# jiny2001/dcscn-super-resolution

Measured on AMD Instinct MI355X. Metric: LR Mpixels/sec at 48x48 patches, L12_F196to48 x2, higher is better.
Workload: dtype f32-equivalent (3x3 stack, wide 1x1 convs and folded tail: f16 hi/lo split, 3 products per MAC, f32 accumulate -- error at the f32 kernels' level, same parity bars; everything else f32)

## Files before the change

dcscn-super-resolution_amd/build.py:

```python

import os
import shutil
import subprocess
import sys
from concurrent.futures import ThreadPoolExecutor

PKG_DIR = os.path.dirname(os.path.abspath(__file__))
CSRC = os.path.join(PKG_DIR, "csrc")
INCLUDE = os.path.join(os.path.dirname(PKG_DIR), "include")
LIB_NAME = "libdcscn_hip.so"
LIB_PATH = os.path.join(PKG_DIR, LIB_NAME)
HEADERS = [os.path.join(CSRC, h) for h in sorted(os.listdir(CSRC)) if h.endswith((".h", ".hpp"))] + [os.path.join(INCLUDE, "dcscn.h")]
ARCH = "gfx950"
NO_PK_F32 = ["-Xclang", "-target-feature", "-Xclang", "-packed-fp32-ops"]
FLAGS = ["--offload-arch=" + ARCH, "-O3", "-std=c++17", "-fPIC", "-Wall", "-Wno-unused-function"] + NO_PK_F32
NO_SLP = ["-fno-slp-vectorize"]
KERNEL = NO_SLP + ["-Rpass-analysis=kernel-resource-usage"]
NO_CONTRACT = ["-ffp-contract=off"]
SOURCE_TABLE = {
    "api.hip": ([], False), "graph.hip": ([], False), "pack.hip": ([], False), "exec.hip": ([], False), "kernels.hip": ([], False),
    "resample.hip": ([], False), "ensemble.hip": ([], False), "color.hip": (NO_CONTRACT, False), "metrics.hip": (NO_CONTRACT, False),
    "conv_k1.hip": ([], False), "conv_k3.hip": ([], False), "conv_k5.hip": ([], False), "conv_k7.hip": ([], False),
    "conv_wino2.hip": (KERNEL, True), "conv_nin.hip": (KERNEL, True), "feat_stream.hip": (KERNEL, True),
    "conv_nin_h.hip": (KERNEL, True), "conv_nin_h_w8.hip": (KERNEL, True), "conv3_h.hip": (KERNEL, True), "conv3_h8.hip": (KERNEL, True),
    "conv5_h.hip": (KERNEL, True), "conv3_h_p16.hip": (KERNEL, True), "conv3_h8_p16.hip": (KERNEL, True),
    "conv3_h_fast16.hip": (KERNEL, True), "conv3_h8_fast16.hip": (KERNEL, True), "conv_nin_h_fast16.hip": (KERNEL, True),
    "conv5_h_fast16.hip": (KERNEL, True), "feat_stream_redo.hip": (NO_SLP, False), "feat3_stream.hip": (KERNEL, True),
    "feat3_stream_fast16.hip": (KERNEL, True),
    "train.hip": ([], False), "train_data.hip": ([], False), "train_h.hip": (KERNEL, True),
    "train_wgrad_h.hip": (KERNEL, True),
}
SOURCES = list(SOURCE_TABLE)
EXTRA_FLAGS = {src: flags for src, (flags, _) in SOURCE_TABLE.items()}
NO_SCRATCH = tuple(src for src, (_, no_spill) in SOURCE_TABLE.items() if no_spill)


def hipcc_path():
    for cand in (shutil.which("hipcc"), "/opt/rocm/bin/hipcc"):
        if cand and os.path.isfile(cand):
            return cand
    raise RuntimeError("hipcc not found; the DCSCN HIP extension cannot be built")


def _stale(target, deps):
    if not os.path.isfile(target):
        return True
    t = os.path.getmtime(target)
    return any(os.path.getmtime(d) > t for d in deps)


def _run(cmd):
    proc = subprocess.run(cmd, stdout=subprocess.PIPE, stderr=subprocess.STDOUT, text=True)
    proc.stdout = "\n".join(ln for ln in proc.stdout.splitlines() if "'-packed-fp32-ops' is not a recognized feature" not in ln)
    if proc.returncode != 0:
        raise RuntimeError("command failed (%d): %s\n%s" % (proc.returncode, " ".join(cmd), proc.stdout))
    if any(cmd[-3].endswith(n) for n in NO_SCRATCH if len(cmd) >= 3):
        import re
        bad = [ln for ln in proc.stdout.splitlines() if re.search(r"(ScratchSize \[bytes/lane\]|VGPRs Spill): [1-9]", ln)]
        if bad:
            os.remove(cmd[-1])
            raise RuntimeError("register spill in a kernel that must not spill (%s):\n%s" % (cmd[-3], "\n".join(bad[:6])))
        return ""
    return proc.stdout


def build(force=False, verbose=False):
    hipcc = hipcc_path()
    obj_dir = os.path.join(PKG_DIR, "build")
    os.makedirs(obj_dir, exist_ok=True)
    jobs = []
    objs = []
    for src in SOURCES:
        src_path = os.path.join(CSRC, src)
        obj = os.path.join(obj_dir, os.path.splitext(src)[0] + ".o")
        objs.append(obj)
        if force or _stale(obj, [src_path, os.path.abspath(__file__)] + HEADERS):
            jobs.append([hipcc] + FLAGS + EXTRA_FLAGS.get(src, []) + ["-I", INCLUDE, "-c", src_path, "-o", obj])
    if jobs:
        with ThreadPoolExecutor(max_workers=len(jobs)) as pool:
            for out in pool.map(_run, jobs):
                if verbose and out.strip():
                    print(out, file=sys.stderr)
    if jobs or force or _stale(LIB_PATH, objs):
        out = _run([hipcc, "--offload-arch=" + ARCH, "-shared", "-fPIC"] + objs + ["-o", LIB_PATH])
        if verbose and out.strip():
            print(out, file=sys.stderr)
    return LIB_PATH


if __name__ == "__main__":
    print(build(force="--force" in sys.argv, verbose=True))
```

dcscn-super-resolution_amd/csrc/api.hip:

```cpp
#include "plan.h"

#pragma clang fp contract(off)

namespace dcscn_impl {

thread_local std::string g_global_error;

void set_global_error(const char* fmt, ...) {
    char buf[512];
    va_list ap;
    va_start(ap, fmt);
    vsnprintf(buf, sizeof buf, fmt, ap);
    va_end(ap);
    g_global_error = buf;
}

int fail(dcscn_ctx* h, int code, const char* fmt, ...) {
    char buf[512];
    va_list ap;
    va_start(ap, fmt);
    vsnprintf(buf, sizeof buf, fmt, ap);
    va_end(ap);
    if (h) h->error = buf;
    g_global_error = buf;
    return code;
}

}

extern "C" {

int dcscn_abi_version(void) { return DCSCN_ABI_VERSION; }

const char* dcscn_last_global_error(void) { return g_global_error.c_str(); }

int dcscn_device_count(void) {
    int n = 0;
    hipError_t e = hipGetDeviceCount(&n);
    if (e != hipSuccess) {
        set_global_error("hipGetDeviceCount: %s", hipGetErrorString(e));
        return -DCSCN_ERR_HIP;
    }
    return n;
}

int dcscn_filter_schedule(int layers, int filters, int min_filters, double gamma, int32_t* out) {
    if (!out || layers <= 0 || gamma <= 0.0) {
        set_global_error("dcscn_filter_schedule: bad arguments");
        return DCSCN_ERR_INVALID_ARG;
    }
    std::vector<int> s;
    filter_schedule(layers, filters, std::min(filters, min_filters), gamma, s);
    for (int i = 0; i < layers; ++i) out[i] = s[i];
    return DCSCN_OK;
}

int dcscn_create(const dcscn_config* cfg, int device, dcscn_handle* out) {
    if (!cfg || !out) return fail(nullptr, DCSCN_ERR_INVALID_ARG, "dcscn_create: null argument");
    *out = nullptr;
    if (cfg->struct_size != (int32_t)sizeof(dcscn_config))
        return fail(nullptr, DCSCN_ERR_INVALID_ARG, "dcscn_create: struct_size %d != %zu", cfg->struct_size, sizeof(dcscn_config));
    dcscn_config c = *cfg;
    c.min_filters = std::min(c.filters, c.min_filters);
    c.reconstruct_layers = std::max(c.reconstruct_layers, 1);
    if (c.scale < 2 || c.scale > 4) return fail(nullptr, DCSCN_ERR_UNSUPPORTED, "scale %d (supported: 2, 3, 4)", c.scale);
    if (c.layers < 1 || c.layers > 256 || c.filters < 1) return fail(nullptr, DCSCN_ERR_INVALID_ARG, "bad layers/filters");
    if (c.layers > 1 && !(c.filters_decay_gamma > 0.0)) return fail(nullptr, DCSCN_ERR_INVALID_ARG, "filters_decay_gamma must be > 0");
    if (c.cnn_size != 1 && c.cnn_size != 3 && c.cnn_size != 5 && c.cnn_size != 7)
        return fail(nullptr, DCSCN_ERR_UNSUPPORTED, "cnn_size %d (supported: 1, 3, 5, 7)", c.cnn_size);
    if (c.channels != 1) return fail(nullptr, DCSCN_ERR_UNSUPPORTED, "channels %d (the reference itself only supports 1)", c.channels);
    if (c.batch_norm) return fail(nullptr, DCSCN_ERR_UNSUPPORTED, "batch_norm is not implemented");
    float dummy;
    if (kernel_act(c.activator, &dummy) < 0) return fail(nullptr, DCSCN_ERR_INVALID_ARG, "Not implemented activator:%d", c.activator);
    if (c.legacy_no_c && c.use_nin) return fail(nullptr, DCSCN_ERR_INVALID_ARG, "legacy_no_c requires use_nin = 0");
    if (c.reconstruct_layers > 1 && c.reconstruct_filters < 1) return fail(nullptr, DCSCN_ERR_INVALID_ARG, "reconstruct_filters must be positive");

    int ndev = 0;
    hipError_t e = hipGetDeviceCount(&ndev);
    if (e != hipSuccess || ndev <= 0)
        return fail(nullptr, DCSCN_ERR_HIP, "no HIP device available (%s); this library has no CPU fallback",
                    e != hipSuccess ? hipGetErrorString(e) : "device count 0");
    if (device < 0 || device >= ndev) return fail(nullptr, DCSCN_ERR_INVALID_ARG, "device %d out of range [0, %d)", device, ndev);

    dcscn_ctx* h = new (std::nothrow) dcscn_ctx();
    if (!h) return fail(nullptr, DCSCN_ERR_NOMEM, "out of host memory");
    h->cfg = c;
    h->device = device;
    int rc = DCSCN_OK;
    do {
        if ((e = hipSetDevice(device)) != hipSuccess) { rc = fail(h, DCSCN_ERR_HIP, "hipSetDevice: %s", hipGetErrorString(e)); break; }
        hipDeviceProp_t prop;
        if ((e = hipGetDeviceProperties(&prop, device)) != hipSuccess) { rc = fail(h, DCSCN_ERR_HIP, "hipGetDeviceProperties: %s", hipGetErrorString(e)); break; }
        if (strncmp(prop.gcnArchName, "gfx950", 6) != 0) {
            rc = fail(h, DCSCN_ERR_HIP, "device %d is %s; this library is built for gfx950 (MI355X) only", device, prop.gcnArchName);
            break;
        }
        h->n_cus = prop.multiProcessorCount > 0 ? prop.multiProcessorCount : 256;
        if ((e = hipStreamCreateWithFlags(&h->stream, hipStreamNonBlocking)) != hipSuccess) { rc = fail(h, DCSCN_ERR_HIP, "hipStreamCreate: %s", hipGetErrorString(e)); break; }
        if ((e = hipEventCreateWithFlags(&h->done_ev, hipEventDisableTiming)) != hipSuccess) { rc = fail(h, DCSCN_ERR_HIP, "hipEventCreate: %s", hipGetErrorString(e)); break; }
        if ((e = conv_init_kernels()) != hipSuccess) { rc = fail(h, DCSCN_ERR_HIP, "kernel attribute setup: %s", hipGetErrorString(e)); break; }
        {
            size_t free_b = 0, total_b = 0;
            if (hipMemGetInfo(&free_b, &total_b) == hipSuccess && free_b > 0)
                h->workspace_budget = std::min<int64_t>(h->workspace_budget, std::max<int64_t>((int64_t)(free_b / 10 * 6), (int64_t)256 << 20));
        }
        rc = build_graph(h);
    } while (0);
    if (rc != DCSCN_OK) {
        g_global_error = h->error;
        dcscn_destroy(h);
        return rc;
    }
    *out = h;
    return DCSCN_OK;
}

int dcscn_num_tensors(dcscn_handle h) { return h ? (int)h->tensors.size() : -DCSCN_ERR_INVALID_ARG; }

int dcscn_tensor_info(dcscn_handle h, int index, char* name, int name_capacity, int64_t* shape, int* rank) {
    if (!h) return DCSCN_ERR_INVALID_ARG;
    if (index < 0 || index >= (int)h->tensors.size() || !name || name_capacity <= 0 || !shape || !rank)
        return fail(h, DCSCN_ERR_INVALID_ARG, "dcscn_tensor_info: bad argument");
    const TensorSpec& t = h->tensors[index];
    snprintf(name, (size_t)name_capacity, "%s", t.name.c_str());
    *rank = (int)t.shape.size();
    for (int i = 0; i < 4; ++i) shape[i] = i < *rank ? t.shape[i] : 1;
    return DCSCN_OK;
}

int dcscn_set_tensor(dcscn_handle h, const char* name, const float* data, const int64_t* shape, int rank) {
    if (!h) return DCSCN_ERR_INVALID_ARG;
    if (!name || !data || !shape) return fail(h, DCSCN_ERR_INVALID_ARG, "dcscn_set_tensor: null argument");
    if (h->finalized) return fail(h, DCSCN_ERR_STATE, "dcscn_set_tensor after dcscn_finalize");
    auto it = h->tensor_index.find(name);
    if (it == h->tensor_index.end()) return fail(h, DCSCN_ERR_SHAPE, "variable '%s' is not part of this graph", name);
    TensorSpec& t = h->tensors[it->second];
    bool same = rank == (int)t.shape.size();
    for (int i = 0; same && i < rank; ++i) same = shape[i] == t.shape[i];
    if (!same) {
        std::string want, got;
        for (int64_t d : t.shape) want += std::to_string(d) + ",";
        for (int i = 0; i < rank && i < 8; ++i) got += std::to_string(shape[i]) + ",";
        return fail(h, DCSCN_ERR_SHAPE, "variable '%s': shape [%s] does not match graph shape [%s]", name, got.c_str(), want.c_str());
    }
    size_t count = 1;
    for (int64_t d : t.shape) count *= (size_t)d;
    for (size_t i = 0; i < count; ++i)
        if (!std::isfinite(data[i])) return fail(h, DCSCN_ERR_INVALID_ARG, "variable '%s' holds a non-finite value", name);
    t.data.assign(data, data + count);
    t.set = true;
    return DCSCN_OK;
}

static int pack_ops(dcscn_ctx* h) {
    const size_t first = h->device_allocs.size();
    int rc = DCSCN_OK;
    for (Op& op : h->ops) {
        rc = finalize_op(h, op);
        if (rc) break;
    }
    h->pack_allocs.insert(h->pack_allocs.end(), h->device_allocs.begin() + first, h->device_allocs.end());
    h->device_allocs.resize(first);
    return rc;
}

}

namespace dcscn_impl {
int repack_weights(dcscn_ctx* h) {
    HIP_TRY(h, hipDeviceSynchronize());
    if (h->graph_exec) {
        (void)hipGraphExecDestroy(h->graph_exec);
        h->graph_exec = nullptr;
        h->graph_key = dcscn_ctx::GraphKey();
    }
    h->graph_seen = dcscn_ctx::GraphKey();
    for (void* p : h->pack_allocs) (void)hipFree(p);
    h->pack_allocs.clear();
    return pack_ops(h);
}
}

extern "C" {

int dcscn_finalize(dcscn_handle h) {
    if (!h) return DCSCN_ERR_INVALID_ARG;
    if (h->finalized) return DCSCN_OK;
    for (const TensorSpec& t : h->tensors)
        if (!t.set) return fail(h, DCSCN_ERR_MISSING_TENSOR, "variable '%s' was never set", t.name.c_str());
    HIP_TRY(h, hipSetDevice(h->device));
    if (h->fold_tail) fold_linear_tail(h);
    fuse_tail_stream(h);
    fuse_feat_stream(h);
    densify_features(h);
    fuse_feat3_stream(h);
    fold_whole_tail(h);
    int rc0 = pack_ops(h);
    if (rc0) return rc0;
    plan_p16(h);
    for (Op& op : h->ops) {
        int rc = DCSCN_OK;
        if (op.kind == OP_CONV && op.shape.nin && op.h16.on && op.h16.in16_ok) {
            op.h16.h_tab16.assign((size_t)4 * op.h16.n_chunks, NinSrcQuad{0, 0, 0});
            rc = upload_vec(h, op.h16.h_tab16, &op.h16.d_tab16);
            if (rc) return rc;
        }
        auto alloc_srctab = [&](Op& o) {
            if (o.multi.empty()) return (int)DCSCN_OK;
            o.h_srctab.assign(std::max<size_t>((size_t)4 * o.n_chunks, (size_t)8 * ((o.cin_phys + kNinHKC - 1) / kNinHKC)), NinSrcQuad{0, 0, 0});
            return upload_vec(h, o.h_srctab, &o.d_srctab);
        };
        rc = alloc_srctab(op);
        if (rc) return rc;
        for (Op& sub : op.fused) {
            rc = alloc_srctab(sub);
            if (rc) return rc;
        }
    }
    h->finalized = true;
    return DCSCN_OK;
}

int dcscn_num_layers(dcscn_handle h) { return h ? (int)h->layers.size() : -DCSCN_ERR_INVALID_ARG; }

int dcscn_layer_info_get(dcscn_handle h, int index, dcscn_layer_info* out) {
    if (!h) return DCSCN_ERR_INVALID_ARG;
    if (!out || index < 0 || index >= (int)h->layers.size()) return fail(h, DCSCN_ERR_INVALID_ARG, "dcscn_layer_info_get: bad argument");
    *out = h->layers[index];
    return DCSCN_OK;
}

int dcscn_num_ops(dcscn_handle h) { return h ? (int)h->ops.size() : -DCSCN_ERR_INVALID_ARG; }

int dcscn_op_info_get(dcscn_handle h, int index, dcscn_op_info* out) {
    if (!h) return DCSCN_ERR_INVALID_ARG;
    if (!out || index < 0 || index >= (int)h->ops.size()) return fail(h, DCSCN_ERR_INVALID_ARG, "dcscn_op_info_get: bad argument");
    const Op& op = h->ops[index];
    memset(out, 0, sizeof *out);
    snprintf(out->name, sizeof out->name, "%s", op.name.c_str());
    const bool s16 = op_on_split16(h, op);
    snprintf(out->kernel, sizeof out->kernel, "%s", kernel_name(op_kernel(h, op)));
    out->kernel_size = op.ks;
    out->in_channels = op.cin;
    out->out_channels = op.cout;
    out->resolution = op.res;
    out->macs_per_lr_pixel = op.macs;
    out->bytes_per_lr_pixel = op.bytes;
    out->executed_macs_per_lr_pixel = op.macs;
    if (op.kind == OP_FOLDX && h->finalized && s16) {
        out->nt = 1; out->kc = 32; out->n_tiles = 1;
        out->executed_macs_per_lr_pixel = (h->fast16 ? 1 : 3) * 25 * (int64_t)op.h16.n_chunks * 32 * 16;
    }
    if (op.kind == OP_CONV && h->finalized) {
        out->mt = op.shape.mt; out->nt = op.shape.nt; out->kc = op.shape.kc; out->n_tiles = op.n_tiles;
        const int64_t r2 = (int64_t)op.res * op.res;
        const int64_t k_exec = (int64_t)op.n_chunks * op.shape.kc;
        if (s16) {
            const int64_t tiles = (int64_t)op.h16.n_tiles * (op.h16.nt - 1) + op.h16.n_full;
            out->nt = op.h16.nt; out->kc = 32; out->n_tiles = op.h16.n_tiles;
            const int64_t ksteps = op.shape.nin ? op.h16.n_chunks : op.fold_s > 0 ? 25 * (int64_t)op.h16.n_chunks
                                                : 9 * (int64_t)(op.h16.n_chunks - (op.h16.tail_octs ? 1 : 0)) + (op.h16.tail_octs ? c3h_tail_steps(op.h16.tail_octs) : 0);
            out->executed_macs_per_lr_pixel = r2 * (h->fast16 ? 1 : 3) * ksteps * 32 * tiles * 16;
        } else if (op.shape.nin) {
            const int64_t tiles = (int64_t)op.n_tiles * (op.shape.nt - 1) + op.n_full;
            out->executed_macs_per_lr_pixel = r2 * k_exec * tiles * 16;
        } else if (op.shape.wino) {
            const int64_t tiles = (int64_t)op.n_tiles * (op.shape.nt - 1) + op.n_full;
            out->executed_macs_per_lr_pixel = r2 * 4 * k_exec * tiles * 16;
        } else {
            out->executed_macs_per_lr_pixel = r2 * op.ks * op.ks * k_exec * (int64_t)op.n_tiles * op.shape.nt * 16;
        }
    }
    return DCSCN_OK;
}

int dcscn_set_option(dcscn_handle h, const char* key, int64_t value) {
    if (!h) return DCSCN_ERR_INVALID_ARG;
    if (!key) return fail(h, DCSCN_ERR_INVALID_ARG, "dcscn_set_option: null key");
    if (!strcmp(key, "sub_batch_pixels")) {
        if (value < 1) return fail(h, DCSCN_ERR_INVALID_ARG, "sub_batch_pixels must be >= 1");
        h->sub_batch_pixels = value;
        return DCSCN_OK;
    }
    if (!strcmp(key, "workspace_budget_bytes")) {
        if (value < 1) return fail(h, DCSCN_ERR_INVALID_ARG, "workspace_budget_bytes must be >= 1");
        h->workspace_budget = value;
        return DCSCN_OK;
    }
    if (!strcmp(key, "spatial_tiling")) {
        h->spatial_tiling = value != 0;
        return DCSCN_OK;
    }
    if (!strcmp(key, "fold_whole_tail")) {
        if (h->finalized) return fail(h, DCSCN_ERR_STATE, "the fold_whole_tail option must be set before dcscn_finalize");
        h->fold_whole = value != 0;
        return DCSCN_OK;
    }
    if (!strcmp(key, "fold_linear_tail")) {
        if (h->finalized) return fail(h, DCSCN_ERR_STATE, "the fold_linear_tail option must be set before dcscn_finalize");
        h->fold_tail = value != 0;
        h->fold_force = value == 2;
        return DCSCN_OK;
    }
    if (!strcmp(key, "stream_tail")) {
        if (h->finalized) return fail(h, DCSCN_ERR_STATE, "the stream_tail option must be set before dcscn_finalize");
        h->stream_tail = value != 0;
        return DCSCN_OK;
    }
    if (!strcmp(key, "stream_features")) {
        if (h->finalized) return fail(h, DCSCN_ERR_STATE, "the stream_features option must be set before dcscn_finalize");
        h->stream_features = value != 0;
        return DCSCN_OK;
    }
    if (!strcmp(key, "stream_nin")) {
        if (h->finalized) return fail(h, DCSCN_ERR_STATE, "the stream_nin option must be set before dcscn_finalize");
        h->stream_nin = value != 0;
        return DCSCN_OK;
    }
    if (!strcmp(key, "stream_dense")) {
        if (h->finalized) return fail(h, DCSCN_ERR_STATE, "the stream_dense option must be set before dcscn_finalize");
        h->stream_dense = value != 0;
        return DCSCN_OK;
    }
    if (!strcmp(key, "dense_features")) {
        if (h->finalized) return fail(h, DCSCN_ERR_STATE, "the dense_features option must be set before dcscn_finalize");
        h->dense_features = value != 0;
        return DCSCN_OK;
    }
    if (!strcmp(key, "nin_gemm")) {
        if (h->finalized) return fail(h, DCSCN_ERR_STATE, "the nin_gemm option must be set before dcscn_finalize");
        h->nin = value != 0;
        return DCSCN_OK;
    }
    if (!strcmp(key, "winograd")) {
        if (h->finalized) return fail(h, DCSCN_ERR_STATE, "the winograd option must be set before dcscn_finalize");
        h->winograd = value != 0;
        return DCSCN_OK;
    }
    if (!strcmp(key, "split16")) {
        h->split16 = value != 0;
        h->split16_mask = value == 2 ? 1 : value == 3 ? 2 : 3;
        return DCSCN_OK;
    }
    if (!strcmp(key, "fast16")) {
        h->fast16 = value != 0;
        return DCSCN_OK;
    }
    if (!strcmp(key, "fast16_stream")) {
        h->fast16_stream = value != 0;
        return DCSCN_OK;
    }
    if (!strcmp(key, "train_split16")) {
        h->train_split16 = value != 0;
        return DCSCN_OK;
    }
    if (!strcmp(key, "train_split16_wgrad")) {
        h->train_split16_wgrad = value != 0;
        return DCSCN_OK;
    }
    if (!strcmp(key, "p16")) {
        h->p16 = value != 0;
        return DCSCN_OK;
    }
    if (!strcmp(key, "conv3_h8")) {
        h->conv3_h8 = value != 0;
        return DCSCN_OK;
    }
    if (!strcmp(key, "nin_h8")) {
        h->nin_h8 = value != 0;
        return DCSCN_OK;
    }
    if (!strcmp(key, "debug_digest")) {
        if ((int)h->ops.size() + 1 > 1024) return fail(h, DCSCN_ERR_UNSUPPORTED, "debug_digest: more than 1023 launches");
        h->debug_digest = value != 0;
        return DCSCN_OK;
    }
    if (!strcmp(key, "debug_poison")) {
        h->debug_poison = (int)value;
        return DCSCN_OK;
    }
    if (!strcmp(key, "profile")) {
        h->profile = value != 0;
        return DCSCN_OK;
    }
    if (!strcmp(key, "graph_replay")) {
        h->graph_replay = value != 0;
        if (!h->graph_replay && h->graph_exec) {
            (void)hipGraphExecDestroy(h->graph_exec);
            h->graph_exec = nullptr;
        }
        h->graph_seen = dcscn_ctx::GraphKey{};
        return DCSCN_OK;
    }
    return fail(h, DCSCN_ERR_INVALID_ARG, "unknown option '%s'", key);
}

int dcscn_forward_device(dcscn_handle h, const float* x, const float* x2, float* y, int n, int height, int width, void* stream) {
    if (!h) return DCSCN_ERR_INVALID_ARG;
    if (h->finalized)
        if (int rc_ = train_sync_inference(h)) return rc_;
    return run_forward(h, x, x2, y, n, height, width, stream ? (hipStream_t)stream : h->stream);
}

static int ensure_io(dcscn_ctx* h, size_t lr_floats, size_t hr_floats) {
    int rc = grow(h, &h->io_x, &h->io_x_cap, lr_floats, h->stream, DCSCN_ERR_HIP);
    if (!rc) rc = grow(h, &h->io_x2, &h->io_x2_cap, hr_floats, h->stream, DCSCN_ERR_HIP);
    if (!rc) rc = grow(h, &h->io_y, &h->io_y_cap, hr_floats, h->stream, DCSCN_ERR_HIP);
    return rc;
}

static int forward_host_chunked(dcscn_ctx* h, const float* x, const float* x2, float* y, int n, int height, int width) {
    const int s = h->cfg.scale;
    const size_t lr1 = (size_t)height * width, hr1 = lr1 * s * s;
    int rc = ensure_io(h, lr1 * n, hr1 * n);
    if (rc) return rc;
    const int chunks = (hr1 * n * sizeof(float) >= ((size_t)8 << 20) && n >= 8) ? 4 : 1;
    while ((int)h->host_ev.size() < chunks) {
        hipEvent_t e;
        HIP_TRY(h, hipEventCreateWithFlags(&e, hipEventDisableTiming));
        h->host_ev.push_back(e);
    }
    int begin[5];
    for (int i = 0; i <= chunks; ++i) begin[i] = (int)((int64_t)n * i / chunks);
    auto span = [&](int i, int* b, int* cnt) { *b = begin[chunks - 1 - i] ; *cnt = begin[chunks - i] - begin[chunks - 1 - i]; };
    auto download = [&](int i) -> int {
        int b, cnt;
        span(i, &b, &cnt);
        HIP_TRY(h, hipEventSynchronize(h->host_ev[i]));
        HIP_TRY(h, hipMemcpy(y + (size_t)b * hr1, h->io_y + (size_t)b * hr1, (size_t)cnt * hr1 * sizeof(float), hipMemcpyDeviceToHost));
        return DCSCN_OK;
    };
    for (int i = 0; i < chunks; ++i) {
        int b, cnt;
        span(i, &b, &cnt);
        if (cnt > 0) {
            HIP_TRY(h, hipMemcpy(h->io_x + (size_t)b * lr1, x + (size_t)b * lr1, (size_t)cnt * lr1 * sizeof(float), hipMemcpyHostToDevice));
            if (x2) HIP_TRY(h, hipMemcpy(h->io_x2 + (size_t)b * hr1, x2 + (size_t)b * hr1, (size_t)cnt * hr1 * sizeof(float), hipMemcpyHostToDevice));
            else rc = resize_device(h, h->io_x + (size_t)b * lr1, h->io_x2 + (size_t)b * hr1, cnt, height, width, height * s, width * s, h->stream);
            if (!rc) rc = run_forward(h, h->io_x + (size_t)b * lr1, h->io_x2 + (size_t)b * hr1, h->io_y + (size_t)b * hr1, cnt, height, width, h->stream);
            if (rc) return rc;
        }
        HIP_TRY(h, hipEventRecord(h->host_ev[i], h->stream));
        if (i > 0 && (rc = download(i - 1))) return rc;
    }
    if ((rc = download(chunks - 1))) return rc;
    return DCSCN_OK;
}

int dcscn_forward(dcscn_handle h, const float* x, const float* x2, float* y, int n, int height, int width) {
    if (!h) return DCSCN_ERR_INVALID_ARG;
    if (!h->finalized) return fail(h, DCSCN_ERR_STATE, "dcscn_forward before dcscn_finalize");
    if (int rc_ = train_sync_inference(h)) return rc_;
    if (n < 0 || height <= 0 || width <= 0) return fail(h, DCSCN_ERR_INVALID_ARG, "bad shape n=%d h=%d w=%d", n, height, width);
    if (n == 0) return DCSCN_OK;
    if (!x || !x2 || !y) return fail(h, DCSCN_ERR_INVALID_ARG, "null image pointer");
    HIP_TRY(h, hipSetDevice(h->device));
    return forward_host_chunked(h, x, x2, y, n, height, width);
}

int dcscn_resample_table(int in_size, int out_size, int* ksize, int* bounds, double* weights, int capacity) {
    if (in_size <= 0 || out_size <= 0 || !ksize) return DCSCN_ERR_INVALID_ARG;
    std::vector<int> b;
    std::vector<double> k;
    *ksize = resample_coeffs(in_size, out_size, &b, &k);
    if (!bounds && !weights) return DCSCN_OK;
    if (!bounds || !weights || capacity < (int)k.size()) return DCSCN_ERR_INVALID_ARG;
    std::copy(b.begin(), b.end(), bounds);
    std::copy(k.begin(), k.end(), weights);
    return DCSCN_OK;
}

int dcscn_resize_bicubic(dcscn_handle h, const float* in, float* out, int n, int height, int width, int out_height, int out_width) {
    if (!h) return DCSCN_ERR_INVALID_ARG;
    if (n < 0 || height <= 0 || width <= 0 || out_height <= 0 || out_width <= 0)
        return fail(h, DCSCN_ERR_INVALID_ARG, "bad shape n=%d %dx%d -> %dx%d", n, height, width, out_height, out_width);
    if (n == 0) return DCSCN_OK;
    if (!in || !out) return fail(h, DCSCN_ERR_INVALID_ARG, "null image pointer");
    HIP_TRY(h, hipSetDevice(h->device));
    const size_t ni = (size_t)n * height * width, no = (size_t)n * out_height * out_width;
    int rc = grow(h, &h->rs_in, &h->rs_in_cap, ni, h->stream);
    if (!rc) rc = grow(h, &h->rs_out, &h->rs_out_cap, no, h->stream);
    if (rc) return rc;
    HIP_TRY(h, hipMemcpy(h->rs_in, in, ni * sizeof(float), hipMemcpyHostToDevice));
    rc = resize_device(h, h->rs_in, h->rs_out, n, height, width, out_height, out_width, h->stream);
    if (rc) return rc;
    HIP_TRY(h, hipStreamSynchronize(h->stream));
    HIP_TRY(h, hipMemcpy(out, h->rs_out, no * sizeof(float), hipMemcpyDeviceToHost));
    return DCSCN_OK;
}

int dcscn_resize_bicubic_device(dcscn_handle h, const float* in, float* out, int n, int height, int width, int out_height,
                                int out_width, void* stream) {
    if (!h) return DCSCN_ERR_INVALID_ARG;
    if (n < 0 || height <= 0 || width <= 0 || out_height <= 0 || out_width <= 0)
        return fail(h, DCSCN_ERR_INVALID_ARG, "bad shape n=%d %dx%d -> %dx%d", n, height, width, out_height, out_width);
    if (n == 0) return DCSCN_OK;
    if (!in || !out) return fail(h, DCSCN_ERR_INVALID_ARG, "null image pointer");
    HIP_TRY(h, hipSetDevice(h->device));
    hipStream_t st = stream ? (hipStream_t)stream : h->stream;
    if (h->has_last && h->last_stream != st) HIP_TRY(h, hipStreamWaitEvent(st, h->done_ev, 0));
    const int rc = resize_device(h, in, out, n, height, width, out_height, out_width, st);
    if (rc) return rc;
    return forward_done(h, st);
}

int dcscn_resample_table_bytes(int in_size, int out_size, int* ksize, int* bounds, int32_t* coeffs, int capacity) {
    if (in_size <= 0 || out_size <= 0 || !ksize) return DCSCN_ERR_INVALID_ARG;
    std::vector<int> b, k;
    *ksize = resample_coeffs8(in_size, out_size, &b, &k);
    if (!bounds && !coeffs) return DCSCN_OK;
    if (!bounds || !coeffs || capacity < (int)k.size()) return DCSCN_ERR_INVALID_ARG;
    std::copy(b.begin(), b.end(), bounds);
    std::copy(k.begin(), k.end(), coeffs);
    return DCSCN_OK;
}

static int resize_bytes_args(dcscn_handle h, const uint8_t* in, uint8_t* out, int n, int height, int width, int channels, int out_height,
                             int out_width, bool* run) {
    *run = false;
    if (n < 0 || height <= 0 || width <= 0 || out_height <= 0 || out_width <= 0)
        return fail(h, DCSCN_ERR_INVALID_ARG, "bad shape n=%d %dx%d -> %dx%d", n, height, width, out_height, out_width);
    if (channels != 1 && channels != 3)
        return fail(h, DCSCN_ERR_INVALID_ARG, "%d channels (uint8 images have 1 (mode L) or 3 (RGB))", channels);
    if (n == 0) return DCSCN_OK;
    if (!in || !out) return fail(h, DCSCN_ERR_INVALID_ARG, "null image pointer");
    *run = true;
    return DCSCN_OK;
}

int dcscn_resize_bicubic_bytes(dcscn_handle h, const uint8_t* in, uint8_t* out, int n, int height, int width, int channels, int out_height,
                               int out_width) {
    if (!h) return DCSCN_ERR_INVALID_ARG;
    bool run;
    int rc = resize_bytes_args(h, in, out, n, height, width, channels, out_height, out_width, &run);
    if (rc || !run) return rc;
    HIP_TRY(h, hipSetDevice(h->device));
    const size_t ni = (size_t)n * height * width * channels, no = (size_t)n * out_height * out_width * channels;
    rc = grow(h, &h->rs_in, &h->rs_in_cap, (ni + 3) / 4, h->stream);
    if (!rc) rc = grow(h, &h->rs_out, &h->rs_out_cap, (no + 3) / 4, h->stream);
    if (rc) return rc;
    HIP_TRY(h, hipMemcpy(h->rs_in, in, ni, hipMemcpyHostToDevice));
    rc = resize_device_bytes(h, reinterpret_cast<const uint8_t*>(h->rs_in), reinterpret_cast<uint8_t*>(h->rs_out), n, height, width, channels,
                             out_height, out_width, h->stream);
    if (rc) return rc;
    HIP_TRY(h, hipStreamSynchronize(h->stream));
    HIP_TRY(h, hipMemcpy(out, h->rs_out, no, hipMemcpyDeviceToHost));
    return DCSCN_OK;
}

int dcscn_resize_bicubic_bytes_device(dcscn_handle h, const uint8_t* in, uint8_t* out, int n, int height, int width, int channels,
                                      int out_height, int out_width, void* stream) {
    if (!h) return DCSCN_ERR_INVALID_ARG;
    bool run;
    int rc = resize_bytes_args(h, in, out, n, height, width, channels, out_height, out_width, &run);
    if (rc || !run) return rc;
    HIP_TRY(h, hipSetDevice(h->device));
    hipStream_t st = stream ? (hipStream_t)stream : h->stream;
    if (h->has_last && h->last_stream != st) HIP_TRY(h, hipStreamWaitEvent(st, h->done_ev, 0));
    rc = resize_device_bytes(h, in, out, n, height, width, channels, out_height, out_width, st);
    if (rc) return rc;
    return forward_done(h, st);
}

int dcscn_forward_lr(dcscn_handle h, const float* x, float* y, int n, int height, int width) {
    if (!h) return DCSCN_ERR_INVALID_ARG;
    if (!h->finalized) return fail(h, DCSCN_ERR_STATE, "dcscn_forward_lr before dcscn_finalize");
    if (int rc_ = train_sync_inference(h)) return rc_;
    if (n < 0 || height <= 0 || width <= 0) return fail(h, DCSCN_ERR_INVALID_ARG, "bad shape n=%d h=%d w=%d", n, height, width);
    if (n == 0) return DCSCN_OK;
    if (!x || !y) return fail(h, DCSCN_ERR_INVALID_ARG, "null image pointer");
    HIP_TRY(h, hipSetDevice(h->device));
    return forward_host_chunked(h, x, nullptr, y, n, height, width);
}

static int ensemble_on_device(dcscn_ctx* h, int height, int width, int n) {
    const int s = h->cfg.scale;
    const size_t lr = (size_t)height * width, hr = lr * s * s;
    const int na = std::min(n, 4), nb = n - na;
    int rc = grow(h, &h->ens_x, &h->ens_x_cap, n * lr, h->stream);
    if (!rc) rc = grow(h, &h->ens_x2, &h->ens_x2_cap, n * hr, h->stream);
    if (!rc) rc = grow(h, &h->ens_y, &h->ens_y_cap, n * hr, h->stream);
    if (!rc) rc = grow(h, &h->ens_out, &h->ens_out_cap, 2 * hr, h->stream);
    if (rc) return rc;
    HIP_TRY(h, ensemble_gather_launch(h->io_x, h->ens_x, height, width, n, h->stream));
    HIP_TRY(h, ensemble_gather_launch(h->io_x2, h->ens_x2, height * s, width * s, n, h->stream));
    rc = run_forward(h, h->ens_x, h->ens_x2, h->ens_y, na, height, width, h->stream);
    if (!rc && nb > 0)
        rc = run_forward(h, h->ens_x + (size_t)na * lr, h->ens_x2 + (size_t)na * hr, h->ens_y + (size_t)na * hr, nb, width, height, h->stream);
    if (rc) return rc;
    HIP_TRY(h, ensemble_reduce_launch(h->ens_y, reinterpret_cast<double*>(h->ens_out), height * s, width * s, n, h->stream));
    return DCSCN_OK;
}

int dcscn_forward_ensemble(dcscn_handle h, const float* x, const float* x2, double* y, int height, int width, int n_ensemble) {
    if (!h) return DCSCN_ERR_INVALID_ARG;
    if (!h->finalized) return fail(h, DCSCN_ERR_STATE, "dcscn_forward_ensemble before dcscn_finalize");
    if (int rc_ = train_sync_inference(h)) return rc_;
    if (!x || !x2 || !y) return fail(h, DCSCN_ERR_INVALID_ARG, "null image pointer");
    if (n_ensemble < 1 || n_ensemble > 8) return fail(h, DCSCN_ERR_INVALID_ARG, "n_ensemble %d outside [1, 8]", n_ensemble);
    if (height <= 0 || width <= 0) return fail(h, DCSCN_ERR_INVALID_ARG, "bad shape h=%d w=%d", height, width);
    HIP_TRY(h, hipSetDevice(h->device));
    const int s = h->cfg.scale;
    const size_t lr = (size_t)height * width, hr = lr * s * s;
    int rc = ensure_io(h, lr, hr);
    if (rc) return rc;
    HIP_TRY(h, hipMemcpy(h->io_x, x, lr * sizeof(float), hipMemcpyHostToDevice));
    HIP_TRY(h, hipMemcpy(h->io_x2, x2, hr * sizeof(float), hipMemcpyHostToDevice));
    rc = ensemble_on_device(h, height, width, n_ensemble);
    if (rc) return rc;
    HIP_TRY(h, hipStreamSynchronize(h->stream));
    HIP_TRY(h, hipMemcpy(y, h->ens_out, hr * sizeof(double), hipMemcpyDeviceToHost));
    return DCSCN_OK;
}


static int color_args(dcscn_handle h, const void* a, const void* b, int64_t n, const char* what) {
    if (!a || !b) return fail(h, DCSCN_ERR_INVALID_ARG, "%s: null pointer", what);
    if (n < 0) return fail(h, DCSCN_ERR_INVALID_ARG, "%s: negative pixel count", what);
    return DCSCN_OK;
}

int dcscn_convert_rgb_to_y(dcscn_handle h, const uint8_t* rgb, double* y, int64_t n_pixels) {
    if (!h) return DCSCN_ERR_INVALID_ARG;
    int rc = color_args(h, rgb, y, n_pixels, "dcscn_convert_rgb_to_y");
    if (rc || n_pixels == 0) return rc;
    HIP_TRY(h, hipSetDevice(h->device));
    rc = grow(h, &h->col_rgb, &h->col_rgb_cap, (size_t)(3 * n_pixels + 3) / 4, h->stream);
    if (!rc) rc = grow(h, &h->col_d, &h->col_d_cap, (size_t)2 * n_pixels, h->stream);
    if (rc) return rc;
    HIP_TRY(h, hipMemcpy(h->col_rgb, rgb, (size_t)3 * n_pixels, hipMemcpyHostToDevice));
    HIP_TRY(h, rgb_to_y_launch(reinterpret_cast<const uint8_t*>(h->col_rgb), reinterpret_cast<double*>(h->col_d), nullptr, n_pixels, h->stream));
    HIP_TRY(h, hipStreamSynchronize(h->stream));
    HIP_TRY(h, hipMemcpy(y, h->col_d, (size_t)n_pixels * sizeof(double), hipMemcpyDeviceToHost));
    return DCSCN_OK;
}

int dcscn_convert_rgb_to_ycbcr(dcscn_handle h, const uint8_t* rgb, double* ycbcr, int64_t n_pixels) {
    if (!h) return DCSCN_ERR_INVALID_ARG;
    int rc = color_args(h, rgb, ycbcr, n_pixels, "dcscn_convert_rgb_to_ycbcr");
    if (rc || n_pixels == 0) return rc;
    HIP_TRY(h, hipSetDevice(h->device));
    rc = grow(h, &h->col_rgb, &h->col_rgb_cap, (size_t)(3 * n_pixels + 3) / 4, h->stream);
    if (!rc) rc = grow(h, &h->col_d, &h->col_d_cap, (size_t)6 * n_pixels, h->stream);
    if (rc) return rc;
    HIP_TRY(h, hipMemcpy(h->col_rgb, rgb, (size_t)3 * n_pixels, hipMemcpyHostToDevice));
    HIP_TRY(h, rgb_to_ycbcr_launch(reinterpret_cast<const uint8_t*>(h->col_rgb), reinterpret_cast<double*>(h->col_d), n_pixels, h->stream));
    HIP_TRY(h, hipStreamSynchronize(h->stream));
    HIP_TRY(h, hipMemcpy(ycbcr, h->col_d, (size_t)3 * n_pixels * sizeof(double), hipMemcpyDeviceToHost));
    return DCSCN_OK;
}

int dcscn_convert_y_and_cbcr_to_rgb(dcscn_handle h, const double* y, const double* cbcr, double* rgb, int64_t n_pixels) {
    if (!h) return DCSCN_ERR_INVALID_ARG;
    int rc = color_args(h, y, cbcr, n_pixels, "dcscn_convert_y_and_cbcr_to_rgb");
    if (!rc && !rgb) rc = fail(h, DCSCN_ERR_INVALID_ARG, "dcscn_convert_y_and_cbcr_to_rgb: null pointer");
    if (rc || n_pixels == 0) return rc;
    HIP_TRY(h, hipSetDevice(h->device));
    rc = grow(h, &h->col_d, &h->col_d_cap, (size_t)6 * n_pixels, h->stream);
    if (!rc) rc = grow(h, &h->col_d2, &h->col_d2_cap, (size_t)6 * n_pixels, h->stream);
    if (rc) return rc;
    double* dy = reinterpret_cast<double*>(h->col_d);
    double* dc = dy + n_pixels;
    HIP_TRY(h, hipMemcpy(dy, y, (size_t)n_pixels * sizeof(double), hipMemcpyHostToDevice));
    HIP_TRY(h, hipMemcpy(dc, cbcr, (size_t)2 * n_pixels * sizeof(double), hipMemcpyHostToDevice));
    HIP_TRY(h, y_cbcr_to_rgb_launch(dy, nullptr, dc, nullptr, reinterpret_cast<double*>(h->col_d2), n_pixels, h->stream));
    HIP_TRY(h, hipStreamSynchronize(h->stream));
    HIP_TRY(h, hipMemcpy(rgb, h->col_d2, (size_t)3 * n_pixels * sizeof(double), hipMemcpyDeviceToHost));
    return DCSCN_OK;
}

static int sr_from_lr_on_device(dcscn_ctx* h, int lh, int lw, int n_ensemble) {
    const int s = h->cfg.scale;
    int rc = resize_device(h, h->io_x, h->io_x2, 1, lh, lw, lh * s, lw * s, h->stream);
    if (rc) return rc;
    if (n_ensemble > 1) return ensemble_on_device(h, lh, lw, n_ensemble);
    return run_forward(h, h->io_x, h->io_x2, h->io_y, 1, lh, lw, h->stream);
}

static int download_sr(dcscn_ctx* h, size_t hr, int n_ensemble, double* y) {
    HIP_TRY(h, hipStreamSynchronize(h->stream));
    if (n_ensemble > 1) {
        HIP_TRY(h, hipMemcpy(y, h->ens_out, hr * sizeof(double), hipMemcpyDeviceToHost));
    } else {
        std::vector<float> tmp(hr);
        HIP_TRY(h, hipMemcpy(tmp.data(), h->io_y, hr * sizeof(float), hipMemcpyDeviceToHost));
        for (size_t i = 0; i < hr; ++i) y[i] = (double)tmp[i];
    }
    return DCSCN_OK;
}

static int evaluate_rgb_on_device(dcscn_ctx* h, const uint8_t* rgb, int height, int width, int n_ensemble, const char* what) {
    if (!h->finalized) return fail(h, DCSCN_ERR_STATE, "%s before dcscn_finalize", what);
    if (int rc_ = train_sync_inference(h)) return rc_;
    if (!rgb) return fail(h, DCSCN_ERR_INVALID_ARG, "%s: null pointer", what);
    if (n_ensemble < 1 || n_ensemble > 8) return fail(h, DCSCN_ERR_INVALID_ARG, "n_ensemble %d outside [1, 8]", n_ensemble);
    const int s = h->cfg.scale;
    if (height <= 0 || width <= 0 || height % s || width % s)
        return fail(h, DCSCN_ERR_INVALID_ARG, "image %dx%d is not aligned to the scale %d (set_image_alignment, utilty.py:196-208)", height, width, s);
    HIP_TRY(h, hipSetDevice(h->device));
    const int lh = height / s, lw = width / s;
    const size_t hr = (size_t)height * width, lrn = (size_t)lh * lw;
    int rc = ensure_io(h, lrn, hr);
    if (!rc) rc = grow(h, &h->col_rgb, &h->col_rgb_cap, (3 * hr + 3) / 4, h->stream);
    if (!rc) rc = grow(h, &h->col_d, &h->col_d_cap, 2 * hr, h->stream);
    if (!rc) rc = grow(h, &h->col_y32, &h->col_y32_cap, hr, h->stream);
    if (rc) return rc;
    HIP_TRY(h, hipMemcpy(h->col_rgb, rgb, 3 * hr, hipMemcpyHostToDevice));
    HIP_TRY(h, rgb_to_y_launch(reinterpret_cast<const uint8_t*>(h->col_rgb), reinterpret_cast<double*>(h->col_d), h->col_y32, (long long)hr, h->stream));
    rc = resize_device(h, h->col_y32, h->io_x, 1, height, width, lh, lw, h->stream);
    if (!rc) rc = sr_from_lr_on_device(h, lh, lw, n_ensemble);
    return rc;
}

int dcscn_evaluate_rgb(dcscn_handle h, const uint8_t* rgb, int height, int width, int n_ensemble, double* true_y, float* lr, double* y) {
    if (!h) return DCSCN_ERR_INVALID_ARG;
    int rc = evaluate_rgb_on_device(h, y ? rgb : nullptr, height, width, n_ensemble, "dcscn_evaluate_rgb");
    const size_t hr = (size_t)height * width, lrn = hr / ((size_t)h->cfg.scale * h->cfg.scale);
    if (!rc) rc = download_sr(h, hr, n_ensemble, y);
    if (rc) return rc;
    if (true_y) HIP_TRY(h, hipMemcpy(true_y, h->col_d, hr * sizeof(double), hipMemcpyDeviceToHost));
    if (lr) HIP_TRY(h, hipMemcpy(lr, h->io_x, lrn * sizeof(float), hipMemcpyDeviceToHost));
    return DCSCN_OK;
}


static const MetricWeights& metric_weights() {
    static const MetricWeights wt = [] {
        MetricWeights m;
        const double sigma2 = 1.5 * 1.5;
        for (int k = 0; k < kMetricTaps; ++k) {
            const double x = (double)(k - kMetricTaps / 2);
            m.w[k] = exp(-0.5 / sigma2 * (x * x));
        }
        double sum = ((m.w[0] + m.w[1]) + (m.w[2] + m.w[3])) + ((m.w[4] + m.w[5]) + (m.w[6] + m.w[7]));
        for (int k = 8; k < kMetricTaps; ++k) sum += m.w[k];
        for (int k = 0; k < kMetricTaps; ++k) m.w[k] = m.w[k] / sum;
        return m;
    }();
    return wt;
}

static int metric_shape(dcscn_ctx* h, int height, int width, int border, const char* what, int* sh, int* sw) {
    if (height <= 0 || width <= 0) return fail(h, DCSCN_ERR_INVALID_ARG, "%s: bad shape h=%d w=%d", what, height, width);
    if (border < 0) return fail(h, DCSCN_ERR_INVALID_ARG, "%s: negative border_size %d (win_size cannot be placed)", what, border);
    *sh = height - 2 * border;
    *sw = width - 2 * border;
    if (*sh < kMetricTaps || *sw < 1)
        return fail(h, DCSCN_ERR_INVALID_ARG, "%s: win_size exceeds image extent (%d x %d after shaving %d: needs %d rows and 1 column)", what,
                    *sh, *sw, border, kMetricTaps);
    return DCSCN_OK;
}

static int metric_buffers(dcscn_ctx* h, int sh, int sw) {
    return grow(h, &h->met_buf, &h->met_buf_cap, (size_t)8 + 2 * (size_t)metric_segments(sh) * sw, h->stream);
}

static int metric_enqueue(dcscn_ctx* h, int slot, const double* a64, const float* a32, const double* b64, const float* b32, int width, int border,
                          int sh, int sw) {
    double* part_s = h->met_buf + 8;
    long long* part_e = reinterpret_cast<long long*>(part_s + (size_t)metric_segments(sh) * sw);
    HIP_TRY(h, metrics_launch(a64, a32, b64, b32, width, border, sh, sw, metric_weights(), part_s, part_e,
                              reinterpret_cast<long long*>(h->met_buf) + 4 * slot, h->stream));
    return DCSCN_OK;
}

static int metric_download(dcscn_ctx* h, dcscn_metrics* first, dcscn_metrics* second) {
    long long words[8];
    HIP_TRY(h, hipStreamSynchronize(h->stream));
    HIP_TRY(h, hipMemcpy(words, h->met_buf, sizeof words, hipMemcpyDeviceToHost));
    dcscn_metrics* outs[2] = {first, second};
    for (int i = 0; i < 2; ++i) {
        if (!outs[i]) continue;
        dcscn_metrics& m = *outs[i];
        m.sq_err_sum = words[4 * i];
        m.n_pixels = words[4 * i + 1];
        memcpy(&m.ssim, &words[4 * i + 2], sizeof(double));
        const double err = (double)m.sq_err_sum / (double)m.n_pixels;
        m.psnr = m.sq_err_sum == 0 ? (double)INFINITY : 10.0 * log10((255.0 * 255.0) / err);
    }
    return DCSCN_OK;
}

int dcscn_psnr_ssim(dcscn_handle h, const double* a, const double* b, int height, int width, int border_size, dcscn_metrics* out) {
    if (!h) return DCSCN_ERR_INVALID_ARG;
    if (!a || !b || !out) return fail(h, DCSCN_ERR_INVALID_ARG, "dcscn_psnr_ssim: null pointer");
    int sh, sw;
    int rc = metric_shape(h, height, width, border_size, "dcscn_psnr_ssim", &sh, &sw);
    if (rc) return rc;
    HIP_TRY(h, hipSetDevice(h->device));
    const size_t n = (size_t)height * width;
    rc = grow(h, &h->col_d, &h->col_d_cap, 2 * n, h->stream);
    if (!rc) rc = grow(h, &h->col_d2, &h->col_d2_cap, 2 * n, h->stream);
    if (!rc) rc = metric_buffers(h, sh, sw);
    if (rc) return rc;
    const double* da = reinterpret_cast<const double*>(h->col_d);
    const double* db = reinterpret_cast<const double*>(h->col_d2);
    HIP_TRY(h, hipMemcpy(h->col_d, a, n * sizeof(double), hipMemcpyHostToDevice));
    HIP_TRY(h, hipMemcpy(h->col_d2, b, n * sizeof(double), hipMemcpyHostToDevice));
    rc = metric_enqueue(h, 0, da, nullptr, db, nullptr, width, border_size, sh, sw);
    if (!rc) rc = metric_download(h, out, nullptr);
    return rc;
}

int dcscn_evaluate_rgb_metrics(dcscn_handle h, const uint8_t* rgb, int height, int width, int n_ensemble, int border_size, dcscn_metrics* model,
                               dcscn_metrics* bicubic, double* y) {
    if (!h) return DCSCN_ERR_INVALID_ARG;
    if (!h->finalized) return fail(h, DCSCN_ERR_STATE, "dcscn_evaluate_rgb_metrics before dcscn_finalize");
    if (!rgb || !model) return fail(h, DCSCN_ERR_INVALID_ARG, "dcscn_evaluate_rgb_metrics: null pointer");
    int sh, sw;
    int rc = metric_shape(h, height, width, border_size, "dcscn_evaluate_rgb_metrics", &sh, &sw);
    if (!rc) rc = evaluate_rgb_on_device(h, rgb, height, width, n_ensemble, "dcscn_evaluate_rgb_metrics");
    if (!rc) rc = metric_buffers(h, sh, sw);
    if (rc) return rc;
    const double* true_y = reinterpret_cast<const double*>(h->col_d);
    rc = metric_enqueue(h, 0, true_y, nullptr, n_ensemble > 1 ? reinterpret_cast<const double*>(h->ens_out) : nullptr,
                        n_ensemble > 1 ? nullptr : h->io_y, width, border_size, sh, sw);
    if (!rc && bicubic) rc = metric_enqueue(h, 1, true_y, nullptr, nullptr, h->io_x2, width, border_size, sh, sw);
    if (!rc) rc = metric_download(h, model, bicubic);
    if (!rc && y) rc = download_sr(h, (size_t)height * width, n_ensemble, y);
    return rc;
}

int dcscn_sr_rgb(dcscn_handle h, const uint8_t* rgb, const uint8_t* rgb_upscaled, int height, int width, int n_ensemble, double* y, double* rgb_out) {
    if (!h) return DCSCN_ERR_INVALID_ARG;
    if (!h->finalized) return fail(h, DCSCN_ERR_STATE, "dcscn_sr_rgb before dcscn_finalize");
    if (int rc_ = train_sync_inference(h)) return rc_;
    if (!rgb || !rgb_upscaled || !rgb_out) return fail(h, DCSCN_ERR_INVALID_ARG, "dcscn_sr_rgb: null pointer");
    if (n_ensemble < 1 || n_ensemble > 8) return fail(h, DCSCN_ERR_INVALID_ARG, "n_ensemble %d outside [1, 8]", n_ensemble);
    if (height <= 0 || width <= 0) return fail(h, DCSCN_ERR_INVALID_ARG, "bad shape h=%d w=%d", height, width);
    HIP_TRY(h, hipSetDevice(h->device));
    const int s = h->cfg.scale;
    const size_t lrn = (size_t)height * width, hr = lrn * s * s;
    int rc = ensure_io(h, lrn, hr);
    if (!rc) rc = grow(h, &h->col_rgb, &h->col_rgb_cap, (3 * hr + 3) / 4 + (3 * lrn + 3) / 4 + 4, h->stream);
    if (!rc) rc = grow(h, &h->col_d2, &h->col_d2_cap, 6 * hr, h->stream);
    if (rc) return rc;
    uint8_t* d_up = reinterpret_cast<uint8_t*>(h->col_rgb);
    uint8_t* d_lr = d_up + ((3 * hr + 15) & ~(size_t)15);
    HIP_TRY(h, hipMemcpy(d_lr, rgb, 3 * lrn, hipMemcpyHostToDevice));
    HIP_TRY(h, hipMemcpy(d_up, rgb_upscaled, 3 * hr, hipMemcpyHostToDevice));
    HIP_TRY(h, rgb_to_y_launch(d_lr, nullptr, h->io_x, (long long)lrn, h->stream));
    rc = sr_from_lr_on_device(h, height, width, n_ensemble);
    if (rc) return rc;
    HIP_TRY(h, y_cbcr_to_rgb_launch(n_ensemble > 1 ? reinterpret_cast<const double*>(h->ens_out) : nullptr, n_ensemble > 1 ? nullptr : h->io_y,
                                    nullptr, d_up, reinterpret_cast<double*>(h->col_d2), (long long)hr, h->stream));
    if (y) rc = download_sr(h, hr, n_ensemble, y);
    else HIP_TRY(h, hipStreamSynchronize(h->stream));
    if (rc) return rc;
    HIP_TRY(h, hipMemcpy(rgb_out, h->col_d2, 3 * hr * sizeof(double), hipMemcpyDeviceToHost));
    return DCSCN_OK;
}

int dcscn_sr_rgb_bytes(dcscn_handle h, const uint8_t* rgb, int height, int width, int n_ensemble, uint8_t* rgb_bicubic, uint8_t* y_bicubic,
                       uint8_t* y_out, uint8_t* rgb_out) {
    if (!h) return DCSCN_ERR_INVALID_ARG;
    if (!h->finalized) return fail(h, DCSCN_ERR_STATE, "dcscn_sr_rgb_bytes before dcscn_finalize");
    if (int rc_ = train_sync_inference(h)) return rc_;
    if (!rgb || (!rgb_bicubic && !y_bicubic && !y_out && !rgb_out)) return fail(h, DCSCN_ERR_INVALID_ARG, "dcscn_sr_rgb_bytes: null pointer");
    if (n_ensemble < 1 || n_ensemble > 8) return fail(h, DCSCN_ERR_INVALID_ARG, "n_ensemble %d outside [1, 8]", n_ensemble);
    if (height <= 0 || width <= 0) return fail(h, DCSCN_ERR_INVALID_ARG, "bad shape h=%d w=%d", height, width);
    HIP_TRY(h, hipSetDevice(h->device));
    const int s = h->cfg.scale;
    const size_t lrn = (size_t)height * width, hr = lrn * s * s;
    const bool net = y_out || rgb_out, luma = net || y_bicubic, colour = rgb_bicubic || rgb_out;
    const size_t plane = (hr + 15) & ~(size_t)15;
    int rc = ensure_io(h, lrn, hr);
    if (!rc) rc = grow(h, &h->col_rgb, &h->col_rgb_cap, (3 * hr + 3) / 4 + (3 * lrn + 3) / 4 + 4, h->stream);
    if (!rc) rc = grow(h, &h->col_d2, &h->col_d2_cap, (2 * plane + 3 * hr + 3) / 4, h->stream);
    if (rc) return rc;
    uint8_t* d_up = reinterpret_cast<uint8_t*>(h->col_rgb);
    uint8_t* d_lr = d_up + ((3 * hr + 15) & ~(size_t)15);
    uint8_t* d_yb = reinterpret_cast<uint8_t*>(h->col_d2);
    uint8_t *d_yo = d_yb + plane, *d_ro = d_yo + plane;
    HIP_TRY(h, hipMemcpy(d_lr, rgb, 3 * lrn, hipMemcpyHostToDevice));
    if (colour && (rc = resize_device_bytes(h, d_lr, d_up, 1, height, width, 3, height * s, width * s, h->stream))) return rc;
    if (luma) {
        HIP_TRY(h, rgb_to_y_launch(d_lr, nullptr, h->io_x, (long long)lrn, h->stream));
        rc = net ? sr_from_lr_on_device(h, height, width, n_ensemble)
                 : resize_device(h, h->io_x, h->io_x2, 1, height, width, height * s, width * s, h->stream);
        if (rc) return rc;
    }
    const double* y64 = n_ensemble > 1 ? reinterpret_cast<const double*>(h->ens_out) : nullptr;
    const float* y32 = n_ensemble > 1 ? nullptr : h->io_y;
    if (y_bicubic) HIP_TRY(h, cast_bytes_launch(nullptr, h->io_x2, d_yb, (long long)hr, h->stream));
    if (y_out) HIP_TRY(h, cast_bytes_launch(y64, y32, d_yo, (long long)hr, h->stream));
    if (rgb_out) HIP_TRY(h, y_cbcr_to_rgb_bytes_launch(y64, y32, d_up, d_ro, (long long)hr, h->stream));
    HIP_TRY(h, hipStreamSynchronize(h->stream));
    if (rgb_bicubic) HIP_TRY(h, hipMemcpy(rgb_bicubic, d_up, 3 * hr, hipMemcpyDeviceToHost));
    if (y_bicubic) HIP_TRY(h, hipMemcpy(y_bicubic, d_yb, hr, hipMemcpyDeviceToHost));
    if (y_out) HIP_TRY(h, hipMemcpy(y_out, d_yo, hr, hipMemcpyDeviceToHost));
    if (rgb_out) HIP_TRY(h, hipMemcpy(rgb_out, d_ro, 3 * hr, hipMemcpyDeviceToHost));
    return DCSCN_OK;
}

int dcscn_get_profile(dcscn_handle h, double* ms, int capacity) {
    if (!h) return DCSCN_ERR_INVALID_ARG;
    if (!ms || capacity < 0) return fail(h, DCSCN_ERR_INVALID_ARG, "dcscn_get_profile: bad argument");
    const int nops = (int)h->ops.size();
    std::vector<double> acc(nops + 1, 0.0);
    const int forwards = h->ev_forwards;
    if (h->ev_used > 0) {
        HIP_TRY(h, hipDeviceSynchronize());
        const size_t launches = h->ev_used / 2;
        for (size_t l = 0; l < launches && l < h->ev_op.size(); ++l) {
            float t = 0.0f;
            HIP_TRY(h, hipEventElapsedTime(&t, h->ev[2 * l], h->ev[2 * l + 1]));
            acc[std::min(std::max(h->ev_op[l], 0), nops)] += t;
        }
    }
    h->ev_used = 0;
    h->ev_forwards = 0;
    h->ev_op.clear();
    if (forwards > 1)
        for (double& v : acc) v /= forwards;
    for (int i = 0; i < std::min(capacity, nops + 1); ++i) ms[i] = acc[i];
    return DCSCN_OK;
}

int dcscn_debug_digests(dcscn_handle h, uint64_t* out, int capacity) {
    if (!h) return DCSCN_ERR_INVALID_ARG;
    if (!out || capacity < 0) return fail(h, DCSCN_ERR_INVALID_ARG, "dcscn_debug_digests: bad argument");
    if (!h->d_digest) return fail(h, DCSCN_ERR_STATE, "dcscn_debug_digests: no forward has run with the debug_digest option on");
    HIP_TRY(h, hipDeviceSynchronize());
    const int n = std::min(capacity, (int)h->ops.size() + 1);
    HIP_TRY(h, hipMemcpy(out, h->d_digest, (size_t)n * sizeof(uint64_t), hipMemcpyDeviceToHost));
    return DCSCN_OK;
}

int64_t dcscn_workspace_bytes(dcscn_handle h) { return h ? (int64_t)h->arena_bytes : -1; }

int dcscn_num_presplit_tensors(dcscn_handle h) {
    if (!h) return -DCSCN_ERR_INVALID_ARG;
    if (!h->finalized || !p16_active(h)) return 0;
    int n = 0;
    for (const WsBuf& b : h->bufs) n += b.p16_ok && b.stride > 0;
    return n;
}

const char* dcscn_last_error(dcscn_handle h) { return h ? h->error.c_str() : g_global_error.c_str(); }

int dcscn_get_stream(dcscn_handle h, void** stream) {
    if (!h) return DCSCN_ERR_INVALID_ARG;
    if (!stream) return fail(h, DCSCN_ERR_INVALID_ARG, "dcscn_get_stream: null pointer");
    *stream = (void*)h->stream;
    return DCSCN_OK;
}

int dcscn_synchronize(dcscn_handle h) {
    if (!h) return DCSCN_ERR_INVALID_ARG;
    HIP_TRY(h, hipSetDevice(h->device));
    if (h->has_last) HIP_TRY(h, hipStreamSynchronize(h->last_stream));
    HIP_TRY(h, hipStreamSynchronize(h->stream));
    return DCSCN_OK;
}

int dcscn_destroy(dcscn_handle h) {
    if (!h) return DCSCN_OK;
    (void)hipSetDevice(h->device);
    if (h->has_last) (void)hipStreamSynchronize(h->last_stream);
    if (h->stream) (void)hipStreamSynchronize(h->stream);
    if (h->graph_exec) (void)hipGraphExecDestroy(h->graph_exec);
    if (h->done_ev) (void)hipEventDestroy(h->done_ev);
    for (hipEvent_t e : h->host_ev) (void)hipEventDestroy(e);
    for (hipEvent_t e : h->ev) (void)hipEventDestroy(e);
    train_free(h);
    train_batches_free(h);
    for (void* p : h->device_allocs) (void)hipFree(p);
    for (void* p : h->pack_allocs) (void)hipFree(p);
    if (h->arena) (void)hipFree(h->arena);
    if (h->d_zrec) (void)hipFree(h->d_zrec);
    if (h->d_digest) (void)hipFree(h->d_digest);
    for (float* p : {h->io_x, h->io_x2, h->io_y, h->tile_x, h->tile_x2, h->tile_y, h->rs_tmp, h->rs_in, h->rs_out, h->ens_x, h->ens_x2, h->ens_y, h->ens_out, h->col_rgb, h->col_d,
                     h->col_d2, h->col_y32})
        if (p) (void)hipFree(p);
    if (h->met_buf) (void)hipFree(h->met_buf);
    if (h->stream) (void)hipStreamDestroy(h->stream);
    delete h;
    return DCSCN_OK;
}

}
```

dcscn-super-resolution_amd/csrc/conv3_h8.hip:

```cpp
#include "conv3_h8.hpp"

namespace dcscn {

using List = C3EVariants<false, 3>;

hipError_t c3e_init_kernels() {
    hipError_t e = c3e16_init_kernels();
    if (e == hipSuccess) e = c3e1_init_kernels();
    return e != hipSuccess ? e : List::set_attrs();
}

bool c3e_eligible(int nt, const ConvArgs& a, int n_groups) {
    return n_groups == 2 && nt >= 4 && nt <= 6 && a.n_full >= 1 && a.n_full <= 2 && a.ps == 1 && a.res == nullptr && (a.act == ACT_ALPHA || a.act == ACT_NONE) &&
           a.n_chunks >= 3;
}

hipError_t c3e_launch(int nt, const ConvArgs& args, int n_groups, int n_cus, hipStream_t stream, bool fast16) {
    if (!c3e_eligible(nt, args, n_groups) || !args.wpack16 || args.tiles_x != (args.W + 15) / 16 || args.tiles_y != (args.H + 15) / 16) return hipErrorInvalidValue;
    ConvArgs a = args;
    a.n_groups = n_groups;
    a.nt_pack = nt;
    const long long units = (long long)a.N * a.tiles_y * a.tiles_x;
    if (units > 0x7fffffffLL) return hipErrorInvalidValue;
    const int wgs = (int)(units < n_cus ? units : n_cus);
    const bool out16 = a.out0.p16.base != nullptr && (a.split >= (1 << 29) || a.out1.p16.base != nullptr);
    const bool p16 = a.in16.base && out16;
    if (!p16 && (a.in16.base || a.out0.p16.base || a.out1.p16.base)) return hipErrorInvalidValue;
    const int key = c3e_key(nt, a.n_full == 2 ? nt : nt - 1, p16);
    if (fast16) return c3e1_launch(key, a, wgs, stream);
    if (p16) return c3e16_launch(key, a, wgs, stream);
    return List::launch(key, a, wgs, stream);
}

}
```

dcscn-super-resolution_amd/csrc/conv3_h8.hpp:

```cpp
#pragma once
#include "conv3_h.hpp"
#include "p16.hpp"

namespace dcscn {

template <int N>
__device__ __forceinline__ void c3p_wait_vm() { asm volatile("s_waitcnt vmcnt(%0)" ::"n"(N) : "memory"); }
__device__ __forceinline__ void c3p_barrier() { asm volatile("s_waitcnt lgkmcnt(0)\n\ts_barrier" ::: "memory"); }

__device__ __forceinline__ void glds16c(const void* sbase, unsigned voff, unsigned lds_dst) {
    asm volatile("s_mov_b32 m0, %2\n\ts_nop 0\n\tglobal_load_lds_dwordx4 %0, %1" : : "v"(voff), "s"(sbase), "s"(lds_dst) : "memory", "m0");
}

template <int NT>
struct C3EGeom {
    static constexpr int THREADS = 512;
    static constexpr int KC = 32, TH = 16, TW = 16, HT = 18, HP = HT * HT;
    static constexpr int PIX_BYTES = 128, ROW_BYTES = HT * PIX_BYTES, IN_BYTES = HP * PIX_BYTES;
    static constexpr int IN_BUF = 41 * 1024;
    static constexpr int IN_ITEMS = HP * 8;
    static constexpr int IN_ROUNDS = (IN_ITEMS + THREADS - 1) / THREADS;
    static constexpr int F_TAP_BYTES = NT * 2048;
    static constexpr int F_ROUNDS = (2 * NT + 3) / 4;
    static constexpr int IMG = 0;
    static constexpr int F_BASE = 2 * IN_BUF;
    static constexpr int BA_BASE = F_BASE + 2 * 3 * F_TAP_BYTES;
    static constexpr int LDS_BYTES = BA_BASE + 4 * NT * 128;
};

template <int NT, int C1, int NTP = NT, bool P16 = false, int NP = 3>
__global__ __launch_bounds__(512, 2) void conv3_h8(const ConvArgs a) {
    static_assert(C1 == NT || C1 == NT - 1, "half 1 takes as many tiles as half 0 or one fewer");
    static_assert(NP == 1 || NP == 3, "one product (fast16) or three (split16)");
    constexpr int PFD = 2 < NT ? 2 : (NT > 1 ? NT - 1 : 1), NB = PFD + 1;
    using G = C3EGeom<NT>;
    extern __shared__ __attribute__((aligned(16))) char smem_c3e[];
    char* const smem = smem_c3e;
    constexpr int F = G::F_ROUNDS, L = G::IN_ROUNDS;

    const int tid = threadIdx.x;
    const int lane = tid & 63;
    const int wave = __builtin_amdgcn_readfirstlane(tid >> 6);
    const int half = wave >> 2, w4 = wave & 3;
    const int H = a.H, W = a.W;
    const int n_groups = a.n_groups, ntp = NTP ? NTP : a.nt_pack;
    const int n_pairs = (n_groups + 1) >> 1;
    const int n_units = a.N * a.tiles_y * a.tiles_x * n_pairs;
    const int n_chunks = a.n_chunks;
    const int octs = a.tail_octs;
    const int n_main = octs ? n_chunks - 1 : n_chunks;
    const int n_tail = (9 * octs + 3) >> 2;
    const int t_total = n_main * 9 + n_tail;
    const bool fastable = a.ps == 1 && a.res == nullptr && (a.act == ACT_ALPHA || a.act == ACT_NONE) && (a.split & 15) == 0;
    const unsigned lds0 = (unsigned)(uintptr_t)(__attribute__((address_space(3))) char*)smem;
    const unsigned f_off = (unsigned)(lane * 16);
    const int cq = tid & 7;
    const int tap_stride = ntp * 2048;

    struct Unit {
        int valid, tile_id, img, y0, x0, g, o;
        int pix0;
        bool all_in, full;
        const char* a_base;
        const char* f_base;
        unsigned ok_mask;
    };
    auto decode = [&](int id, Unit& u) DCSCN_INL {
        u.valid = id < n_units;
        const int idc = u.valid ? id : 0;
        const int tile_id = idc / n_pairs, p = idc - tile_id * n_pairs;
        const int g0 = 2 * p;
        if (g0 + 1 < n_groups) {
            u.g = g0 + half; u.o = 0;
        } else {
            u.g = g0; u.o = half ? NT : 0;
        }
        int bid = tile_id;
        const int tx = bid % a.tiles_x;
        bid /= a.tiles_x;
        const int ty = bid % a.tiles_y;
        u.tile_id = tile_id;
        u.img = bid / a.tiles_y;
        u.y0 = ty * G::TH; u.x0 = tx * G::TW;
        u.all_in = u.y0 >= 1 && u.x0 >= 1 && u.y0 + G::TH + 1 <= H && u.x0 + G::TW + 1 <= W;
        u.full = u.y0 + G::TH <= H && u.x0 + G::TW <= W;
        if constexpr (P16) { u.a_base = nullptr; u.pix0 = (u.img * H + u.y0 - 1) * W + u.x0 - 1; }
        else { u.pix0 = 0; u.a_base = reinterpret_cast<const char*>(a.in + (size_t)u.img * H * W * a.in_stride + a.in_off + ((ptrdiff_t)(u.y0 - 1) * W + (u.x0 - 1)) * a.in_stride); }
        u.f_base = reinterpret_cast<const char*>(a.wpack16) + (size_t)u.g * n_chunks * 9 * tap_stride + (size_t)u.o * 2048;
        unsigned m = 0;
        int hp0 = tid >> 3;
        asm volatile("" : "+v"(hp0));
        int hrow = hp0 / G::HT, hcol = hp0 - G::HT * hrow;
        static_for<0, L>([&](auto r_) DCSCN_INL {
            constexpr int r = decltype(r_)::value;
            const int gy = u.y0 - 1 + hrow, gx = u.x0 - 1 + hcol;
            bool ok = r * 64 + hp0 < G::HP && gy >= 0 && gy < H && gx >= 0 && gx < W;
            if constexpr (P16 && r == L - 1) {
                const int hp = 320 + (hp0 & 7), hr = hp / G::HT, hc = hp - G::HT * hr;
                const int qy = u.y0 - 1 + hr, qx = u.x0 - 1 + hc;
                ok = hp < G::HP && qy >= 0 && qy < H && qx >= 0 && qx < W;
            }
            m |= ok ? (1u << r) : 0u;
            hcol += 64 - 3 * G::HT; hrow += 3;
            if (hcol >= G::HT) { hcol -= G::HT; hrow += 1; }
        });
        u.ok_mask = m;
    };

    f32x4 gin[L];
    auto load_in = [&](const char* base, unsigned mask, int chunk) DCSCN_INL {
        const int c0 = chunk * G::KC + cq * 4;
        const unsigned coff = (unsigned)((c0 < a.cin_phys ? c0 : 0) * 4);
        int hp0 = tid >> 3;
        asm volatile("" : "+v"(hp0));
        int hrow = hp0 / G::HT, hcol = hp0 - G::HT * hrow;
        const int stride4 = a.in_stride * 4;
        static_for<0, L>([&](auto r_) DCSCN_INL {
            constexpr int r = decltype(r_)::value;
            const int pix = ((mask >> r) & 1u) ? hrow * W + hcol : W + 1;
            asm volatile("global_load_dwordx4 %0, %1, %2" : "=v"(gin[r]) : "v"((unsigned)(pix * stride4) + coff), "s"(base) : "memory");
            hcol += 64 - 3 * G::HT; hrow += 3;
            if (hcol >= G::HT) { hcol -= G::HT; hrow += 1; }
        });
    };
    const float m1 = opaque_minus_one();
    auto convert_store = [&](auto r_, bool all_in, unsigned mask, int chunk, int buf) DCSCN_INL {
        constexpr int r = decltype(r_)::value;
        asm volatile("" : "+v"(gin[r]));
        f32x4 x = gin[r];
        const bool whole = all_in && (chunk + 1) * G::KC <= a.cin_phys;
        if (!whole) {
            const bool ok = chunk * G::KC + cq * 4 < a.cin_phys && ((mask >> r) & 1u);
            x.x = ok ? x.x : 0.0f; x.y = ok ? x.y : 0.0f; x.z = ok ? x.z : 0.0f; x.w = ok ? x.w : 0.0f;
        }
        h4 hi, lo;
        split4(x, m1, hi, lo);
        const u32x2 hu = __builtin_bit_cast(u32x2, hi), lu = __builtin_bit_cast(u32x2, lo);
        int hp0 = tid >> 3;
        asm volatile("" : "+v"(hp0));
        const int hp = r * 64 + hp0;
        const int hcol = hp % G::HT;
        const int kq = cq >> 1;
        const int off = buf * G::IN_BUF + hp * G::PIX_BYTES + c3h_unit(hcol, kq, 0) * 16 + (cq & 1) * 8;
        if (r < L - 1 || hp < G::HP) {
            *reinterpret_cast<u32x2*>(smem + off) = hu;
            *reinterpret_cast<u32x2*>(smem + (off ^ 16)) = lu;
        }
    };
    auto img_piece = [&](auto r_, int pix0, unsigned mask, int chunk, int buf) DCSCN_INL {
        constexpr int r = decltype(r_)::value;
        const int rem = a.in16.octs - 4 * chunk;
        const int rec = rem >= 4 ? 128 : 32 * rem;
        const char* base = a.in16.base + (long long)chunk * a.in16.plane;
        int t8 = tid >> 3;
        asm volatile("" : "+v"(t8));
        const int hp = r < L - 1 ? r * 64 + t8 : 320 + (t8 & 7);
        const int hrow = hp / G::HT, hcol = hp - G::HT * hrow;
        const int s = lane & 7;
        const int kq = ((s >> 1) - (hcol >> 1)) & 3;
        const int part = (s ^ kq ^ hcol) & 1;
        const bool ok = ((mask >> r) & 1u) && kq < rem;
        const unsigned voff = ok ? 128u + (unsigned)(pix0 + hrow * W + hcol) * (unsigned)rec + (unsigned)((2 * kq + part) * 16) : (unsigned)(s * 16);
        const int piece = r < L - 1 ? wave + 8 * r : 40;
        glds16c(base, voff, lds0 + (unsigned)(buf * G::IN_BUF + piece * 1024));
    };
    auto dma_f = [&](const char* src, int slot , int cnt) DCSCN_INL {
        const int pieces = cnt > 0 ? 2 * cnt : 1;
        static_for<0, F>([&](auto r_) DCSCN_INL {
            constexpr int r = decltype(r_)::value;
            const int piece = (w4 + 4 * r) % pieces;
            glds16c(src + piece * 1024, f_off, lds0 + (unsigned)slot + (unsigned)piece * 1024u);
        });
    };
    auto tap_src = [&](const Unit& u, const Unit& un, int tt) DCSCN_INL -> const char* {
        const Unit& w = tt < t_total ? u : un;
        const int t = tt < t_total ? tt : tt - t_total;
        int idx;
        if (t < n_main * 9) { const int c = t / 9, s = t - 9 * c; idx = c * 9 + (s % 3) * 3 + s / 3; }
        else idx = t;
        return w.f_base + (size_t)idx * tap_stride;
    };

    auto run = [&](auto cnt_c, auto half_c) DCSCN_INL {
    constexpr int CNT = decltype(cnt_c)::value;
    constexpr int HALF = decltype(half_c)::value;
    constexpr bool BAR_L = HALF == 1, BAR_C = HALF == 0;
    constexpr bool DMA_LATE = HALF == 1;
    Unit cur, nxt;
    int id = blockIdx.x;
    decode(id, cur);
    if (!cur.valid) return;
    decode(id + (int)gridDim.x, nxt);
    int ibuf = 0;
    int sl0 = G::F_BASE + (half * 3 + 0) * G::F_TAP_BYTES, sl1 = G::F_BASE + (half * 3 + 1) * G::F_TAP_BYTES, sl2 = G::F_BASE + (half * 3 + 2) * G::F_TAP_BYTES;
    dma_f(tap_src(cur, nxt, 0), sl0, CNT);
    dma_f(tap_src(cur, nxt, 1), sl1, CNT);
    if constexpr (P16) {
        static_for<0, L>([&](auto r_) DCSCN_INL { img_piece(r_, cur.pix0, cur.ok_mask, 0, 0); });
        asm volatile("s_waitcnt vmcnt(0)" ::: "memory");
    } else {
        load_in(cur.a_base, cur.ok_mask, 0);
        asm volatile("s_waitcnt vmcnt(0)" ::: "memory");
        static_for<0, L>([&](auto r_) DCSCN_INL { convert_store(r_, cur.all_in, cur.ok_mask, 0, 0); });
    }
    c3p_barrier();
    if (half == 1) asm volatile("s_setprio 1");

    f32x4 acc[4][NT];
    [[maybe_unused]] h8 xh[4], xl[4], wa[NB], wb[NB];
    bool pending = false;
    int parity = 0;
    int e_tile = 0, e_img = 0, e_y0 = 0, e_x0 = 0, e_g = 0, e_o = 0;
    bool e_full = false;

    auto epilogue = [&]() DCSCN_INL {
        const int ba = G::BA_BASE + ((parity ^ 1) * 2 + half) * NT * 128;
        const int cb16 = e_g * ntp * 16 - 16 * (e_g > a.n_full ? e_g - a.n_full : 0) + e_o * 16;
        const float inv = a.inv_scale;
        const float zero = opaque_zero();
        float chk = 0.0f;
        int le = lane;
        asm volatile("" : "+v"(le));
        const int lje = le & 15, lke = le >> 4;
        if constexpr (P16) {
            const h2 zero2 = p16_opaque_zero2();
            auto finish = [&](auto act_c, auto mask_c) DCSCN_INL {
                constexpr int ACT_C = decltype(act_c)::value;
                constexpr bool MASK = decltype(mask_c)::value;
                const bool col_ok = !MASK || e_x0 + lje < W;
                static_for<0, CNT>([&](auto n_) DCSCN_INL {
                    constexpr int n = decltype(n_)::value;
                    const int c0 = cb16 + n * 16;
                    const bool first = c0 < a.split;
                    const P16Desc& od = first ? a.out0.p16 : a.out1.p16;
                    const int oct0 = ((first ? a.out0.off : a.out1.off) + (first ? c0 : c0 - a.split)) >> 3;
                    const int chunk = oct0 >> 2, rem = od.octs - 4 * chunk;
                    const int rec = rem >= 4 ? 128 : 32 * rem;
                    char* base = od.base + (long long)chunk * od.plane + 128 + (long long)((e_img * H + e_y0) * W + e_x0) * rec + (oct0 & 3) * 32;
                    const unsigned voff = (unsigned)((4 * w4 * W + lje) * rec + lke * 16);
                    const unsigned rowb = (unsigned)(W * rec);
                    const bool chan_ok = col_ok && oct0 + (lke >> 1) < od.octs;
                    const f32x4 bv = *reinterpret_cast<const f32x4*>(smem + ba + (n * 4 + lke) * 16);
                    f32x4 av = {0.0f, 0.0f, 0.0f, 0.0f};
                    if (ACT_C == ACT_ALPHA || (ACT_C < 0 && a.act == ACT_ALPHA)) av = *reinterpret_cast<const f32x4*>(smem + ba + NT * 64 + (n * 4 + lke) * 16);
                    static_for<0, 4>([&](auto m_) DCSCN_INL {
                        constexpr int m = decltype(m_)::value;
                        f32x4 v = acc[m][n] * inv + bv;
                        if constexpr (ACT_C == ACT_ALPHA) {
                            v.x = v.x > 0.0f ? v.x : av.x * v.x;
                            v.y = v.y > 0.0f ? v.y : av.y * v.y;
                            v.z = v.z > 0.0f ? v.z : av.z * v.z;
                            v.w = v.w > 0.0f ? v.w : av.w * v.w;
                        } else if constexpr (ACT_C < 0) {
                            if (chan_ok && (!MASK || e_y0 + 4 * w4 + m < H)) chk = nonfinite_acc(chk, acc[m][n], zero);
                            v.x = activate1(v.x, av.x, a.act);
                            v.y = activate1(v.y, av.y, a.act);
                            v.z = activate1(v.z, av.z, a.act);
                            v.w = activate1(v.w, av.w, a.act);
                        }
                        const u32x4 unit = p16_unit(v, m1, chk, zero2, chan_ok && (!MASK || e_y0 + 4 * w4 + m < H));
                        if (chan_ok && (!MASK || e_y0 + 4 * w4 + m < H)) *reinterpret_cast<u32x4*>(base + (size_t)(voff + m * rowb)) = unit;
                    });
                });
            };
            if (e_full) {
                if (a.act == ACT_ALPHA) finish(std::integral_constant<int, ACT_ALPHA>{}, std::false_type{});
                else if (a.act == ACT_NONE) finish(std::integral_constant<int, ACT_NONE>{}, std::false_type{});
                else finish(std::integral_constant<int, -1>{}, std::false_type{});
            } else {
                if (a.act == ACT_ALPHA) finish(std::integral_constant<int, ACT_ALPHA>{}, std::true_type{});
                else finish(std::integral_constant<int, -1>{}, std::true_type{});
            }
            if (chk != chk && a.redo) { a.redo[0] = 1; a.redo[1 + e_img] = 1; }
            pending = false;
            return;
        }
        if (fastable && e_full) {
            auto finish = [&](auto act_c) DCSCN_INL {
                constexpr int ACT_C = decltype(act_c)::value;
                static_for<0, CNT>([&](auto n_) DCSCN_INL {
                    constexpr int n = decltype(n_)::value;
                    const int c0 = cb16 + n * 16;
                    const bool first = c0 < a.split;
                    float* optr = first ? a.out0.ptr : a.out1.ptr;
                    const int ostride = first ? a.out0.stride : a.out1.stride;
                    const int ooff = first ? a.out0.off : a.out1.off;
                    const int owidth = first ? a.out0.width : a.out1.width;
                    const int cc0 = first ? c0 : c0 - a.split;
                    char* base = reinterpret_cast<char*>(optr + ((size_t)(e_img * H + e_y0) * W + e_x0) * ostride + ooff + cc0);
                    const unsigned voff = (unsigned)(((4 * w4 * W + lje) * ostride + 4 * lke) * 4);
                    const unsigned rowb = (unsigned)(W * ostride * 4);
                    const bool chan_ok = cc0 + 4 * lke < owidth;
                    const f32x4 bv = *reinterpret_cast<const f32x4*>(smem + ba + (n * 4 + lke) * 16);
                    f32x4 av = {0.0f, 0.0f, 0.0f, 0.0f};
                    if constexpr (ACT_C == ACT_ALPHA) av = *reinterpret_cast<const f32x4*>(smem + ba + NT * 64 + (n * 4 + lke) * 16);
                    static_for<0, 4>([&](auto m_) DCSCN_INL {
                        constexpr int m = decltype(m_)::value;
                        f32x4 v = acc[m][n] * inv + bv;
                        if constexpr (ACT_C == ACT_ALPHA) {
                            v.x = v.x > 0.0f ? v.x : av.x * v.x;
                            v.y = v.y > 0.0f ? v.y : av.y * v.y;
                            v.z = v.z > 0.0f ? v.z : av.z * v.z;
                            v.w = v.w > 0.0f ? v.w : av.w * v.w;
                        }
                        if (chan_ok) chk = nonfinite_acc(chk, acc[m][n], zero);
                        if (chan_ok) *reinterpret_cast<f32x4*>(base + (size_t)(voff + m * rowb)) = v;
                    });
                });
            };
            if (a.act == ACT_ALPHA) finish(std::integral_constant<int, ACT_ALPHA>{});
            else finish(std::integral_constant<int, ACT_NONE>{});
        } else {
            const int obase = cb16 + 4 * lke;
            const int act = a.act, ps = a.ps, orow = W * ps;
            const int gx = e_x0 + lje;
            static_for<0, CNT>([&](auto n_) DCSCN_INL {
                constexpr int n = decltype(n_)::value;
                const int c = obase + n * 16;
                const f32x4 bv = *reinterpret_cast<const f32x4*>(smem + ba + (n * 4 + lke) * 16);
                f32x4 av = {0.0f, 0.0f, 0.0f, 0.0f};
                if (act == ACT_ALPHA) av = *reinterpret_cast<const f32x4*>(smem + ba + NT * 64 + (n * 4 + lke) * 16);
                const bool first = c < a.split;
                float* optr = first ? a.out0.ptr : a.out1.ptr;
                const int ostride = first ? a.out0.stride : a.out1.stride;
                const int ooff = first ? a.out0.off : a.out1.off;
                const int owidth = first ? a.out0.width : a.out1.width;
                const int cc = first ? c : c - a.split;
                int ch = cc, ay = 0, bx = 0;
                if (ps != 1) {
                    const int sub = cc / a.ps_c;
                    ch = cc - sub * a.ps_c;
                    ay = sub / ps;
                    bx = sub - ay * ps;
                }
                const bool live = gx < W && cc < owidth;
                static_for<0, 4>([&](auto m_) DCSCN_INL {
                    constexpr int m = decltype(m_)::value;
                    const int gy = e_y0 + 4 * w4 + m;
                    f32x4 v = acc[m][n] * inv + bv;
                    v.x = activate1(v.x, av.x, act);
                    v.y = activate1(v.y, av.y, act);
                    v.z = activate1(v.z, av.z, act);
                    v.w = activate1(v.w, av.w, act);
                    if (live && gy < H) {
                        chk = nonfinite_acc(chk, acc[m][n], zero);
                        const size_t pix = (size_t)((e_img * H + gy) * ps + ay) * orow + (size_t)(gx * ps + bx);
                        if (a.res) v += *reinterpret_cast<const f32x4*>(a.res + pix * a.res_stride + ch);
                        *reinterpret_cast<f32x4*>(optr + pix * ostride + ooff + ch) = v;
                    }
                });
            });
        }
        if (chk != chk && a.redo) { a.redo[0] = 1; a.redo[1 + e_img] = 1; }
        pending = false;
    };
    auto phase_barrier = [&](auto on_c) DCSCN_INL {
        __builtin_amdgcn_sched_barrier(0);
        if constexpr (decltype(on_c)::value) {
            c3p_barrier();
            __builtin_amdgcn_sched_barrier(0);
        }
    };
    constexpr std::integral_constant<bool, BAR_L> bar_l{};
    constexpr std::integral_constant<bool, BAR_C> bar_c{};

    while (true) {
        {
            const int ba = G::BA_BASE + (parity * 2 + half) * NT * 128;
            const int t4 = tid & 255;
            const int boff = cur.g * ntp * 16 + cur.o * 16;
            if (t4 < NT * 4) {
                if (t4 < CNT * 4) *reinterpret_cast<f32x4*>(smem + ba + t4 * 16) = reinterpret_cast<const f32x4*>(a.bias + boff)[t4];
            } else if (t4 >= 64 && t4 < 64 + NT * 4 && a.act == ACT_ALPHA) {
                if (t4 - 64 < CNT * 4) *reinterpret_cast<f32x4*>(smem + ba + NT * 64 + (t4 - 64) * 16) = reinterpret_cast<const f32x4*>(a.alpha + boff)[t4 - 64];
            }
        }
        int b_hi = 0;
        const int a_lane = lane * 16;
        int tt = 0;
        for (int chunk = 0; chunk < n_main; ++chunk) {
            const bool last_main = chunk + 1 == n_main;
            const bool ends = last_main && octs == 0;
            const char* li_base = ends ? nxt.a_base : cur.a_base;
            const unsigned li_ok = ends ? nxt.ok_mask : cur.ok_mask;
            const bool li_all_in = ends ? nxt.all_in : cur.all_in;
            const int li_pix0 = ends ? nxt.pix0 : cur.pix0;
            const int lchunk = ends ? 0 : chunk + 1;
            const int img_off = ibuf * G::IN_BUF;
            static_for<0, 9>([&](auto s_) DCSCN_INL {
                constexpr int step = decltype(s_)::value;
                constexpr int kx = step / 3, ky = step % 3;
                if constexpr (ky == 0) {
                    int l = lane;
                    asm volatile("" : "+v"(l));
                    const int hx = (l & 15) + kx;
                    b_hi = img_off + (4 * w4 * G::HT + hx) * G::PIX_BYTES + c3h_unit(hx, l >> 4, 0) * 16;
                }
                static_for<(ky == 0 ? 0 : 3), 4>([&](auto m_) DCSCN_INL {
                    constexpr int row = ky + decltype(m_)::value;
                    xh[row & 3] = *reinterpret_cast<const h8*>(smem + b_hi + row * G::ROW_BYTES);
                    if constexpr (NP == 3) xl[row & 3] = *reinterpret_cast<const h8*>(smem + (b_hi ^ 16) + row * G::ROW_BYTES);
                });
                const char* fs = smem + (step % 3 == 0 ? sl0 : step % 3 == 1 ? sl1 : sl2) + a_lane;
                static_for<0, PFD>([&](auto p_) DCSCN_INL {
                    constexpr int p = decltype(p_)::value;
                    wb[p] = *reinterpret_cast<const h8*>(fs + (2 * p) * 1024);
                    if constexpr (NP == 3) wa[p] = *reinterpret_cast<const h8*>(fs + (2 * p + 1) * 1024);
                });
                auto dma_ahead = [&]() DCSCN_INL {
                    constexpr int step2 = (step + 2) % 9;
                    constexpr int ptap2 = (step2 % 3) * 3 + step2 / 3;
                    const char* src;
                    if constexpr (step + 2 < 9) src = cur.f_base + (size_t)(chunk * 9 + ptap2) * tap_stride;
                    else src = !last_main ? cur.f_base + (size_t)((chunk + 1) * 9 + ptap2) * tap_stride
                             : octs      ? cur.f_base + (size_t)(n_main * 9 + step2) * tap_stride
                                         : nxt.f_base + (size_t)ptap2 * tap_stride;
                    dma_f(src, (step + 2) % 3 == 0 ? sl0 : (step + 2) % 3 == 1 ? sl1 : sl2, CNT);
                };
                if constexpr (!DMA_LATE) dma_ahead();
                constexpr int IMG = P16 && step >= 1 && step <= L ? 1 : 0, IMG_PREV = P16 && step >= 2 && step <= L + 1 ? 1 : 0;
                if constexpr (P16) { if constexpr (IMG) img_piece(std::integral_constant<int, step - 1>{}, li_pix0, li_ok, lchunk, ibuf ^ 1); }
                else {
                    if constexpr (step == 0) load_in(li_base, li_ok, lchunk);
                    if constexpr (step >= 3) convert_store(std::integral_constant<int, step - 3>{}, li_all_in, li_ok, lchunk, ibuf ^ 1);
                }
                if constexpr (step == 0) { if (chunk == 0 && pending) epilogue(); }
                if constexpr (DMA_LATE) { if constexpr (P16) c3p_wait_vm<IMG>(); else if constexpr (step == 0) c3p_wait_vm<L>(); else c3p_wait_vm<0>(); }
                phase_barrier(bar_l);
                if constexpr (DMA_LATE) { dma_ahead(); __builtin_amdgcn_sched_barrier(0); }
                if constexpr (step == 0) {
                    if (chunk == 0)
                        static_for<0, 4>([&](auto m_) DCSCN_INL {
                            static_for<0, NT>([&](auto n_) DCSCN_INL { acc[decltype(m_)::value][decltype(n_)::value] = f32x4{0.0f, 0.0f, 0.0f, 0.0f}; });
                        });
                }
                auto mfmas = [&](auto cnt_c) DCSCN_INL {
                    constexpr int CNT = decltype(cnt_c)::value;
                    static_for<0, CNT>([&](auto n_) DCSCN_INL {
                        constexpr int n = decltype(n_)::value;
                        if constexpr (n + PFD < CNT) {
                            wb[(n + PFD) % NB] = *reinterpret_cast<const h8*>(fs + (2 * (n + PFD)) * 1024);
                            if constexpr (NP == 3) wa[(n + PFD) % NB] = *reinterpret_cast<const h8*>(fs + (2 * (n + PFD) + 1) * 1024);
                        }
                        if constexpr (NP == 3) {
                        static_for<0, 4>([&](auto m_) DCSCN_INL { constexpr int m = decltype(m_)::value; acc[m][n] = __builtin_amdgcn_mfma_f32_16x16x32_f16(wa[n % NB], xh[(ky + m) & 3], acc[m][n], 0, 0, 0); });
                        static_for<0, 4>([&](auto m_) DCSCN_INL { constexpr int m = decltype(m_)::value; acc[m][n] = __builtin_amdgcn_mfma_f32_16x16x32_f16(wb[n % NB], xl[(ky + m) & 3], acc[m][n], 0, 0, 0); });
                        }
                        static_for<0, 4>([&](auto m_) DCSCN_INL { constexpr int m = decltype(m_)::value; acc[m][n] = __builtin_amdgcn_mfma_f32_16x16x32_f16(wb[n % NB], xh[(ky + m) & 3], acc[m][n], 0, 0, 0); });
                        __builtin_amdgcn_sched_barrier(0);
                    });
                };
                mfmas(std::integral_constant<int, CNT>{});
                if constexpr (HALF == 0) { if constexpr (P16) c3p_wait_vm<F + IMG + IMG_PREV>(); else if constexpr (step <= 1) c3p_wait_vm<F + L>(); else c3p_wait_vm<F>(); }
                phase_barrier(bar_c);
                ++tt;
            });
            ibuf ^= 1;
        }
        if (octs) {
            const int img_off = ibuf * G::IN_BUF;
            int l = lane;
            asm volatile("" : "+v"(l));
            auto tail_step = [&](int step, auto first_c) DCSCN_INL {
                constexpr bool FIRST = decltype(first_c)::value;
                if constexpr (!P16)
                if (!FIRST && step == 2) {
                    if constexpr (HALF == 0) c3p_wait_vm<F>();
                    static_for<0, L>([&](auto r_) DCSCN_INL { convert_store(r_, nxt.all_in, nxt.ok_mask, 0, ibuf ^ 1); });
                }
                if constexpr (!DMA_LATE) dma_f(tap_src(cur, nxt, tt + 2), sl2, CNT);
                if constexpr (P16) {
                    if constexpr (!FIRST) { if (step == 1) static_for<0, L>([&](auto r_) DCSCN_INL { img_piece(r_, nxt.pix0, nxt.ok_mask, 0, ibuf ^ 1); }); }
                } else if constexpr (FIRST) load_in(nxt.a_base, nxt.ok_mask, 0);
                const int pair = 4 * step + (l >> 4);
                int tap = octs == 1 ? pair : octs == 2 ? pair >> 1 : (pair * 11) >> 5;
                const int oct = pair - tap * octs;
                tap = tap < 8 ? tap : 8;
                const int ky = (tap * 11) >> 5, kx = tap - 3 * ky;
                const int hx = (l & 15) + kx;
                const int b = img_off + ((4 * w4 + ky) * G::HT + hx) * G::PIX_BYTES + c3h_unit(hx, oct, 0) * 16;
                static_for<0, 4>([&](auto m_) DCSCN_INL {
                    constexpr int m = decltype(m_)::value;
                    xh[m] = *reinterpret_cast<const h8*>(smem + b + m * G::ROW_BYTES);
                    if constexpr (NP == 3) xl[m] = *reinterpret_cast<const h8*>(smem + (b ^ 16) + m * G::ROW_BYTES);
                });
                const char* fs = smem + sl0 + a_lane;
                static_for<0, PFD>([&](auto p_) DCSCN_INL {
                    constexpr int p = decltype(p_)::value;
                    wb[p] = *reinterpret_cast<const h8*>(fs + (2 * p) * 1024);
                    if constexpr (NP == 3) wa[p] = *reinterpret_cast<const h8*>(fs + (2 * p + 1) * 1024);
                });
                if constexpr (DMA_LATE) {
                    if constexpr (P16) { if (!FIRST && step == 1) c3p_wait_vm<L>(); else c3p_wait_vm<0>(); }
                    else if constexpr (FIRST) c3p_wait_vm<L>(); else c3p_wait_vm<0>();
                }
                phase_barrier(bar_l);
                if constexpr (DMA_LATE) { dma_f(tap_src(cur, nxt, tt + 2), sl2, CNT); __builtin_amdgcn_sched_barrier(0); }
                auto mfmas = [&](auto cnt_c) DCSCN_INL {
                    constexpr int CNT = decltype(cnt_c)::value;
                    static_for<0, CNT>([&](auto n_) DCSCN_INL {
                        constexpr int n = decltype(n_)::value;
                        if constexpr (n + PFD < CNT) {
                            wb[(n + PFD) % NB] = *reinterpret_cast<const h8*>(fs + (2 * (n + PFD)) * 1024);
                            if constexpr (NP == 3) wa[(n + PFD) % NB] = *reinterpret_cast<const h8*>(fs + (2 * (n + PFD) + 1) * 1024);
                        }
                        if constexpr (NP == 3) {
                        static_for<0, 4>([&](auto m_) DCSCN_INL { constexpr int m = decltype(m_)::value; acc[m][n] = __builtin_amdgcn_mfma_f32_16x16x32_f16(wa[n % NB], xh[m], acc[m][n], 0, 0, 0); });
                        static_for<0, 4>([&](auto m_) DCSCN_INL { constexpr int m = decltype(m_)::value; acc[m][n] = __builtin_amdgcn_mfma_f32_16x16x32_f16(wb[n % NB], xl[m], acc[m][n], 0, 0, 0); });
                        }
                        static_for<0, 4>([&](auto m_) DCSCN_INL { constexpr int m = decltype(m_)::value; acc[m][n] = __builtin_amdgcn_mfma_f32_16x16x32_f16(wb[n % NB], xh[m], acc[m][n], 0, 0, 0); });
                        __builtin_amdgcn_sched_barrier(0);
                    });
                };
                mfmas(std::integral_constant<int, CNT>{});
                if constexpr (HALF == 0) {
                    if constexpr (P16) { if (!FIRST && step == 1) c3p_wait_vm<F + L>(); else c3p_wait_vm<F>(); }
                    else if (FIRST || step == 1) c3p_wait_vm<F + L>(); else c3p_wait_vm<F>();
                }
                phase_barrier(bar_c);
                ++tt;
                { const int t = sl0; sl0 = sl1; sl1 = sl2; sl2 = t; }
            };
            tail_step(0, std::true_type{});
            for (int step = 1; step < n_tail; ++step) tail_step(step, std::false_type{});
            ibuf ^= 1;
        }
        pending = true;
        e_tile = cur.tile_id; e_img = cur.img; e_y0 = cur.y0; e_x0 = cur.x0; e_g = cur.g; e_o = cur.o; e_full = cur.full;
        parity ^= 1;
        if (!nxt.valid) break;
        id += (int)gridDim.x;
        decode(id, cur);
        decode(id + (int)gridDim.x, nxt);
    }
    epilogue();
    };
    if (half == 0) run(std::integral_constant<int, NT>{}, std::integral_constant<int, 0>{});
    else run(std::integral_constant<int, C1>{}, std::integral_constant<int, 1>{});
    asm volatile("s_waitcnt vmcnt(0)" ::: "memory");
}

constexpr int c3e_key(int nt, int c1, bool p16) { return (8 * nt + c1) * 2 + p16; }

template <int NT, int C1, bool P16, int NP>
struct C3EVariant {
    static constexpr int KEY = c3e_key(NT, C1, P16);
    static constexpr auto kernel = &conv3_h8<NT, C1, NT, P16, NP>;
    static constexpr int THREADS = C3EGeom<NT>::THREADS, LDS = C3EGeom<NT>::LDS_BYTES;
    static hipError_t set_attr() { return allow_lds(kernel, LDS); }
    static hipError_t launch(const ConvArgs& a, int wgs, hipStream_t stream) {
        if (P16 && (long long)a.N * a.H * a.W > kP16MaxPixels) return hipErrorInvalidValue;
        hipLaunchKernelGGL(kernel, dim3((unsigned)wgs), dim3(THREADS), LDS, stream, a);
        return hipGetLastError();
    }
};
template <bool P16, int NP>
using C3EVariants = Variants<C3EVariant<6, 6, P16, NP>, C3EVariant<6, 5, P16, NP>, C3EVariant<5, 5, P16, NP>, C3EVariant<5, 4, P16, NP>, C3EVariant<4, 4, P16, NP>,
                             C3EVariant<4, 3, P16, NP>>;

hipError_t c3e16_init_kernels();
hipError_t c3e16_launch(int key, const ConvArgs& a, int wgs, hipStream_t stream);
hipError_t c3e1_init_kernels();
hipError_t c3e1_launch(int key, const ConvArgs& a, int wgs, hipStream_t stream);

}
```

dcscn-super-resolution_amd/csrc/exec.hip:

```cpp
#include "plan.h"

#pragma clang fp contract(off)

namespace dcscn_impl {


static int ensure_workspace(dcscn_ctx* h, int nb, int H, int W, hipStream_t stream) {
    const bool want16 = p16_active(h);
    if (h->arena && nb <= h->lay_n && H == h->lay_h && W == h->lay_w && want16 == h->p16_now) return DCSCN_OK;
    std::vector<size_t> offsets(h->bufs.size()), sizes(h->bufs.size());
    size_t total = 0;
    for (size_t i = 0; i < h->bufs.size(); ++i) {
        const WsBuf& b = h->bufs[i];
        offsets[i] = total;
        sizes[i] = ws_tensor_bytes(b, (long long)nb * H * b.res * W * b.res, want16);
        total += ws_granules(sizes[i]);
    }
    const size_t redo_ints = 1 + (size_t)nb;
    h->redo_off = total;
    h->redo_ints = redo_ints;
    total += ws_granules(redo_ints * sizeof(int32_t));
    total = std::max<size_t>(total, 256);
    if (total > h->arena_bytes) {
        if (h->has_last) HIP_TRY(h, hipStreamSynchronize(h->last_stream));
        HIP_TRY(h, hipStreamSynchronize(h->stream));
        if (h->arena) HIP_TRY(h, hipFree(h->arena));
        h->arena = nullptr;
        h->arena_bytes = 0;
        h->lay_n = h->lay_h = h->lay_w = 0;
        hipError_t e = hipMalloc(&h->arena, total);
        if (e != hipSuccess) {
            (void)hipGetLastError();
            return fail(h, DCSCN_ERR_NOMEM, "workspace of %zu bytes: %s", total, hipGetErrorString(e));
        }
        h->arena_bytes = total;
    } else if (h->has_last && h->last_stream != stream) {
        HIP_TRY(h, hipStreamWaitEvent(stream, h->done_ev, 0));
    }
    for (size_t i = 0; i < h->bufs.size(); ++i) {
        WsBuf& b = h->bufs[i];
        b.offset = offsets[i];
        b.bytes = sizes[i];
        b.p16 = want16 && b.p16_ok && b.stride > 0;
        b.plane = p16_plane_bytes((long long)nb * H * b.res * W * b.res);
    }
    h->p16_now = want16;
    HIP_TRY(h, hipMemsetAsync(h->arena, 0, total, stream));
    h->carve_gen += 1;
    h->lay_n = nb;
    h->lay_h = H;
    h->lay_w = W;
    return DCSCN_OK;
}

static P16Desc p16_desc(const dcscn_ctx* h, int id) {
    const WsBuf& b = h->bufs[id];
    return P16Desc{static_cast<char*>(h->arena) + b.offset, b.plane, b.octs, 0};
}

bool op_on_split16(const dcscn_ctx* h, const Op& op) {
    if (op.kind == OP_STREAM || op.kind == OP_TAIL || op.kind == OP_STREAM3 || op.kind == OP_FOLDX) return h->split16 && op.h16.on && (h->split16_mask & 1);
    return op.kind == OP_CONV && h->split16 && op.h16.on && (h->split16_mask & (op.shape.nin ? 2 : 1));
}

static bool op_takes_h8(const dcscn_ctx* h, const Op& op) {
    if (!op_on_split16(h, op) || !h->conv3_h8 || op.shape.nin || op.fold_s > 0) return false;
    ConvArgs a{};
    a.n_full = op.h16.n_full; a.ps = op.ps; a.res = op.residual ? reinterpret_cast<const float*>(1) : nullptr; a.act = op.act; a.n_chunks = op.h16.n_chunks;
    if (!c3e_eligible(op.h16.nt, a, op.h16.n_tiles)) return false;
    const bool on16 = p16_active(h);
    const bool in16 = on16 && op.h16.in16_ok;
    bool all16 = true, any16 = false;
    for_each_dst(op, [&](int buf, int) {
        const bool o = on16 && buf >= 0 && h->bufs[buf].p16_ok && h->bufs[buf].stride > 0;
        all16 = all16 && o; any16 = any16 || o;
    });
    return in16 ? all16 : !any16;
}


Kernel op_kernel(const dcscn_ctx* h, const Op& op, bool redo) {
    const bool s16 = !redo && op_on_split16(h, op);
    switch (op.kind) {
        case OP_CONV:
            if (s16) return op.shape.nin ? K_CONV_NIN_H : op.fold_s > 0 ? K_CONV5_H : op_takes_h8(h, op) ? K_CONV3_H8 : K_CONV3_H;
            return op.shape.nin ? K_CONV_NIN : op.shape.wino ? K_CONV_WINO2 : K_CONV_IGEMM;
        case OP_CIN1: return K_CONV_CIN1;
        case OP_COUT1: return K_CONV_COUT1;
        case OP_DW: return K_DEPTHWISE;
        case OP_STREAM: return K_FEAT_STREAM;
        case OP_TAIL: return K_TAIL_STREAM;
        case OP_STREAM3: return s16 ? K_FEAT3_STREAM : K_LAYER_BY_LAYER;
        case OP_FOLDX: return s16 ? K_CONV5_H : K_LAYER_BY_LAYER;
    }
    return K_CONV_IGEMM;
}

const char* kernel_name(Kernel k) {
    static const char* const names[] = {"conv_igemm", "conv_wino2", "conv_nin", "conv_nin_h", "conv5_h", "conv3_h8", "conv3_h", "conv_cin1", "conv_cout1",
                                        "depthwise", "feat_stream", "tail_stream", "feat3_stream", "layer by layer"};
    static_assert(sizeof names / sizeof names[0] == K_LAYER_BY_LAYER + 1, "one name per Kernel");
    return names[k];
}

static bool op_any_split16(const dcscn_ctx* h, const Op& op) {
    if (op_on_split16(h, op)) return true;
    if (op_kernel(h, op, false) != K_LAYER_BY_LAYER) return false;
    for (const Op& sub : op.fused)
        if (op_any_split16(h, sub)) return true;
    return false;
}

struct Pass {
    int nb, H, W;
    const float* x; const float* x2; float* y;
    hipStream_t stream;
    bool redo;
};

static int32_t* redo_flags(const dcscn_ctx* h) { return reinterpret_cast<int32_t*>(static_cast<char*>(h->arena) + h->redo_off); }

template <class Args>
static int stream_geometry(Args& a, const Pass& p, int halo, int workgroups) {
    a.N = p.nb; a.H = p.H; a.W = p.W;
    a.halo = halo;
    if (p.W <= kStreamPX) { a.n_strips = 1; a.useful_w = p.W; }
    else { a.useful_w = kStreamPX - 2 * a.halo; a.n_strips = (p.W + a.useful_w - 1) / a.useful_w; }
    const int64_t cols = (int64_t)p.nb * a.n_strips;
    const int want = (int)std::max<int64_t>(1, (512 + cols - 1) / cols);
    a.useful_h = std::max(32, (p.H + want - 1) / want);
    a.n_blocks = (p.H + a.useful_h - 1) / a.useful_h;
    a.rows_c = a.n_blocks == 1 ? p.H : a.useful_h + 2 * a.halo;
    a.n_jobs = (int)(cols * a.n_blocks);
    a.jobs_per_wg = (a.n_jobs + workgroups - 1) / workgroups;
    return (a.n_jobs + a.jobs_per_wg - 1) / a.jobs_per_wg;
}

static int launch_stream3(dcscn_ctx* h, const Op& op, const Pass& p) {
    Stream3Args a = op.stream3;
    a.x = p.x;
    a.blob = op.d_w;
    const int grid = stream_geometry(a, p, a.L + (a.nin.on ? 1 : 0), h->n_cus);
    auto out_desc = [&](int id, int lo, int hi) {
        S3Out o{};
        o.ptr = buf_ptr(h, id);
        o.stride = h->bufs[id].stride;
        o.width = h->bufs[id].stride;
        o.p16 = h->bufs[id].p16 ? p16_desc(h, id) : P16Desc{nullptr, 0, 0, 0};
        o.lo = lo; o.hi = hi < 0 ? o.width : hi;
        return o;
    };
    if (a.nin.on) {
        for (int i = 0; i < kS3MaxL; ++i) a.out[i] = S3Out{};
        a.out[a.L] = out_desc(op.extra_out[0], 0, 8);
        a.out2 = out_desc(op.extra_out[0], 8, 32);
    } else {
        for (size_t i = 0; i < op.extra_out.size(); ++i) a.out[i] = out_desc(op.extra_out[i], 0, -1);
    }
    a.redo = redo_flags(h);
    HIP_TRY(h, stream3_launch(a, grid, p.stream, h->split16 && h->fast16_stream));
    return DCSCN_OK;
}

static int launch_foldx(dcscn_ctx* h, const Op& op, const Pass& p) {
    ConvArgs b{};
    b.in = buf_ptr(h, op.in_buf);
    b.in_stride = h->bufs[op.in_buf].stride;
    b.in_off = op.in_off;
    b.cin_phys = op.cin_phys;
    if (h->p16_now && op.h16.in16_ok) {
        b.in16 = p16_desc(h, op.in_buf);
        b.in = nullptr;
    }
    b.n_chunks = op.h16.n_chunks;
    b.wpack16 = op.h16.d_w;
    b.bias = op.h16.d_bias;
    b.inv_scale = op.h16.inv_scale;
    b.act = ACT_NONE;
    b.N = p.nb; b.H = p.H; b.W = p.W;
    b.tiles_x = (p.W + 15) / 16;
    b.tiles_y = (p.H + 15) / 16;
    b.out0.ptr = p.y; b.out0.stride = 1; b.out0.width = 1;
    b.out1 = b.out0;
    b.split = kNoSplit;
    b.ps = op.fold_s; b.ps_c = 1;
    b.res = p.x2; b.res_stride = 1;
    b.fold = 2;
    b.redo = redo_flags(h);
    HIP_TRY(h, c5h_launch(1, b, p.stream, h->fast16));
    HIP_TRY(h, c5h_border_launch(b, p.stream, h->fast16));
    return DCSCN_OK;
}

static int launch_tail(dcscn_ctx* h, const Op& op, const Pass& p, bool stream16) {
    TailArgs a = op.tail;
    a.c2 = buf_ptr(h, op.in_buf);
    a.c2_stride = h->bufs[op.in_buf].stride;
    a.x2 = p.x2;
    a.y = p.y;
    a.blob = stream16 ? static_cast<const float*>(op.h16.d_w) : op.d_w;
    a.redo = redo_flags(h); a.redo_check = p.redo ? 1 : 0;
    const int grid = stream_geometry(a, p, 2, 256);
    HIP_TRY(h, tail_launch(a, grid, stream16, p.stream));
    return DCSCN_OK;
}

static int launch_stream(dcscn_ctx* h, const Op& op, const Pass& p, bool stream16) {
    StreamArgs a = op.stream;
    a.x = p.x;
    a.out = buf_ptr(h, op.out_buf[0]);
    a.out_stride = h->bufs[op.out_buf[0]].stride;
    a.blob = stream16 ? static_cast<const float*>(op.h16.d_w) : op.d_w;
    a.redo = redo_flags(h); a.redo_check = p.redo ? 1 : 0;
    const int grid = stream_geometry(a, p, a.L + 1, 256);
    HIP_TRY(h, stream_launch(a, grid, stream16, p.stream));
    return DCSCN_OK;
}

static int launch_dw(dcscn_ctx* h, const Op& op, const Pass& p) {
    DwArgs a{};
    a.in = op.in_buf == EXT_X ? p.x : buf_ptr(h, op.in_buf);
    a.in_stride = op.in_buf == EXT_X ? 1 : h->bufs[op.in_buf].stride;
    a.in_off = op.in_off;
    a.chan_map = op.d_map;
    a.w = op.d_w;
    a.ks = op.ks;
    a.cin = op.cin;
    a.cout_phys = pad4(op.cin);
    a.N = p.nb; a.H = p.H * op.res; a.W = p.W * op.res;
    a.out = buf_ptr(h, op.out_buf[0]);
    a.out_stride = pad4(op.cin);
    a.redo = redo_flags(h); a.redo_check = p.redo ? 1 : 0;
    HIP_TRY(h, depthwise_launch(a, p.stream));
    return DCSCN_OK;
}

static int launch_cout1(dcscn_ctx* h, const Op& op, const Pass& p) {
    Cout1Args a{};
    a.in = buf_ptr(h, op.in_buf);
    a.in_stride = h->bufs[op.in_buf].stride;
    a.in_off = op.in_off;
    a.cin_phys = op.cin_phys;
    a.w = op.d_w;
    a.scale = op.out_scale;
    a.bias = 0.0f;
    a.ks = op.ks;
    a.N = p.nb; a.H = p.H * op.res; a.W = p.W * op.res;
    a.out = p.y;
    a.out_stride = 1;
    a.res = op.residual ? p.x2 : nullptr;
    a.res_stride = 1;
    a.redo = redo_flags(h); a.redo_check = p.redo ? 1 : 0;
    HIP_TRY(h, cout1_launch(a, p.stream));
    return DCSCN_OK;
}

static int launch_cin1(dcscn_ctx* h, const Op& op, const Pass& p) {
    Cin1Args a{};
    a.x = p.x;
    a.w = op.d_w; a.bias = op.d_bias; a.alpha = op.d_alpha;
    a.act = op.act;
    a.ks = op.ks;
    a.N = p.nb; a.H = p.H * op.res; a.W = p.W * op.res;
    a.cs = op.out_width[0];
    a.out.ptr = buf_ptr(h, op.out_buf[0]);
    a.out.stride = h->bufs[op.out_buf[0]].stride;
    a.out.off = op.out_off[0];
    a.out.width = op.out_width[0];
    if (!p.redo && h->bufs[op.out_buf[0]].p16) a.out.p16 = p16_desc(h, op.out_buf[0]);
    a.redo = redo_flags(h); a.redo_check = p.redo ? 1 : 0;
    HIP_TRY(h, cin1_launch(a, p.stream));
    return DCSCN_OK;
}

static int launch_conv(dcscn_ctx* h, const Op& op, const Pass& p, Kernel kernel) {
    const int Hr = p.H * op.res, Wr = p.W * op.res;
    ConvArgs a{};
    a.in = buf_ptr(h, op.in_buf);
    a.in_stride = op.in_stride_override > 0 ? op.in_stride_override : h->bufs[op.in_buf].stride;
    a.in_off = op.in_off;
    a.cin_phys = op.cin_phys;
    a.n_chunks = op.n_chunks;
    a.wpack = op.d_w; a.bias = op.d_bias; a.alpha = op.d_alpha;
    a.act = op.act;
    a.N = p.nb; a.H = Hr; a.W = Wr;
    a.tiles_x = (Wr + 15) / 16;
    a.tiles_y = (Hr + 4 * op.shape.mt - 1) / (4 * op.shape.mt);
    a.n_full = op.n_full;
    for (int i = 0; i < 2; ++i) {
        OutDesc& o = i == 0 ? a.out0 : a.out1;
        const int id = op.out_buf[i];
        o.ptr = id == EXT_Y ? p.y : buf_ptr(h, id);
        o.stride = id == EXT_Y ? 1 : h->bufs[id].stride;
        o.off = op.out_off[i];
        o.width = op.out_width[i];
    }
    a.split = op.split;
    a.ps = op.ps;
    a.ps_c = op.ps == 1 ? 1 : op.ps_c;
    a.vec4 = op.vec4 ? 1 : 0;
    a.res = op.residual ? p.x2 : nullptr;
    a.res_stride = 1;
    a.dww = op.d_dww;
    a.dwk = op.dwk;
    a.fold = op.fold_s > 0 ? 1 : 0;
    a.srctab = op.multi.empty() ? nullptr : op.d_srctab;
    a.redo = redo_flags(h);
    if (kernel == K_CONV_NIN || kernel == K_CONV_WINO2 || kernel == K_CONV_IGEMM) {
        a.redo_check = p.redo ? 1 : 0;
        if (kernel == K_CONV_NIN) HIP_TRY(h, nin_launch(op.shape.nt, a, op.n_tiles, p.stream));
        else if (kernel == K_CONV_WINO2) HIP_TRY(h, wino_launch(op.shape.nt, a, op.n_tiles, p.stream));
        else HIP_TRY(h, conv_launch(op.shape, a, op.n_tiles, p.stream));
        return DCSCN_OK;
    }
    ConvArgs b = a;
    b.wpack16 = op.h16.d_w;
    b.inv_scale = op.h16.inv_scale;
    b.n_chunks = op.h16.n_chunks;
    b.n_full = op.h16.n_full;
    if (h->p16_now && op.h16.in16_ok) {
        b.in16 = p16_desc(h, op.multi.empty() ? op.in_buf : op.multi[0].first);
        b.in = nullptr;
        if (op.shape.nin) b.srctab = op.h16.d_tab16;
    }
    if (op.out_buf[0] >= 0 && h->bufs[op.out_buf[0]].p16) b.out0.p16 = p16_desc(h, op.out_buf[0]);
    if (op.out_buf[1] >= 0 && h->bufs[op.out_buf[1]].p16) b.out1.p16 = p16_desc(h, op.out_buf[1]);
    if (kernel == K_CONV_NIN_H) {
        HIP_TRY(h, nin_h_launch(op.h16.nt, b, op.h16.n_tiles, h->nin_h8, p.stream, h->fast16));
    } else if (kernel == K_CONV5_H) {
        b.bias = op.h16.d_bias;
        HIP_TRY(h, c5h_launch(op.h16.nt, b, p.stream, h->fast16));
    } else {
        b.bias = op.h16.d_bias;
        b.tail_octs = op.h16.tail_octs;
        b.alpha = op.h16.d_alpha;
        b.tiles_y = (Hr + 15) / 16;
        if (kernel == K_CONV3_H8) HIP_TRY(h, c3e_launch(op.h16.nt, b, op.h16.n_tiles, h->n_cus, p.stream, h->fast16));
        else HIP_TRY(h, c3h_launch(op.h16.nt, b, op.h16.n_tiles, p.stream, h->fast16));
    }
    return DCSCN_OK;
}

static int launch_op(dcscn_ctx* h, const Op& op, const Pass& p) {
    const Kernel kernel = op_kernel(h, op, p.redo);
    if (kernel == K_LAYER_BY_LAYER) {
        for (const Op& sub : op.fused) {
            const int rc = launch_op(h, sub, p);
            if (rc) return rc;
        }
        return DCSCN_OK;
    }
    switch (op.kind) {
        case OP_STREAM3: return launch_stream3(h, op, p);
        case OP_FOLDX: return launch_foldx(h, op, p);
        case OP_TAIL: return launch_tail(h, op, p, !p.redo && op_on_split16(h, op));
        case OP_STREAM: return launch_stream(h, op, p, !p.redo && op_on_split16(h, op));
        case OP_DW: return launch_dw(h, op, p);
        case OP_COUT1: return launch_cout1(h, op, p);
        case OP_CIN1: return launch_cin1(h, op, p);
        case OP_CONV: return launch_conv(h, op, p, kernel);
    }
    return DCSCN_OK;
}

static int halo_lr_pixels(const dcscn_ctx* h) {
    double r = 0.0;
    for (const Op& op : h->ops) {
        const int k = op.kind == OP_CONV && op.dwk ? op.dwk : op.ks;
        r += (double)(op.halo >= 0 ? op.halo : k / 2) / op.res;
    }
    return (int)std::ceil(r - 1e-9);
}

static int run_tiled(dcscn_ctx* h, const float* x, const float* x2, float* y, int n, int H, int W, int64_t pass_pixels, hipStream_t stream) {
    const int R = halo_lr_pixels(h), s = h->cfg.scale;
    int Ht = (int)std::min<int64_t>(H, std::max<int64_t>(1, (int64_t)std::sqrt((double)pass_pixels)));
    int Wt = (int)std::min<int64_t>(W, std::max<int64_t>(1, pass_pixels / Ht));
    if (Wt == W) Ht = (int)std::min<int64_t>(H, pass_pixels / Wt);
    if ((Ht < H && Ht <= 2 * R) || (Wt < W && Wt <= 2 * R))
        return fail(h, DCSCN_ERR_NOMEM, "image %dx%d needs spatial tiling, but a pass of %lld LR pixels is too small for windows "
                    "with a %d-pixel halo; raise sub_batch_pixels / workspace_budget_bytes", H, W, (long long)pass_pixels, R);
    auto starts = [&](int full, int win) {
        std::vector<int> v;
        if (win >= full) { v.push_back(0); return v; }
        const int stride = win - 2 * R;
        for (int a = 0; a + win < full; a += stride) v.push_back(a);
        v.push_back(full - win);
        return v;
    };
    const std::vector<int> ys = starts(H, Ht), xs = starts(W, Wt);
    const size_t tiles = (size_t)n * ys.size() * xs.size();
    const size_t lr = tiles * Ht * Wt, hr = lr * s * s;
    if ((lr > h->tile_x_cap || hr > h->tile_x2_cap || hr > h->tile_y_cap) && h->has_last) HIP_TRY(h, hipStreamSynchronize(h->last_stream));
    int rc = grow(h, &h->tile_x, &h->tile_x_cap, lr, stream, DCSCN_ERR_HIP);
    if (!rc) rc = grow(h, &h->tile_x2, &h->tile_x2_cap, hr, stream, DCSCN_ERR_HIP);
    if (!rc) rc = grow(h, &h->tile_y, &h->tile_y_cap, hr, stream, DCSCN_ERR_HIP);
    if (rc) return rc;
    size_t t = 0;
    for (int img = 0; img < n; ++img)
        for (int wy : ys)
            for (int wx : xs) {
                HIP_TRY(h, hipMemcpy2DAsync(h->tile_x + t * Ht * Wt, (size_t)Wt * sizeof(float),
                                            x + ((size_t)img * H + wy) * W + wx, (size_t)W * sizeof(float),
                                            (size_t)Wt * sizeof(float), Ht, hipMemcpyDeviceToDevice, stream));
                HIP_TRY(h, hipMemcpy2DAsync(h->tile_x2 + t * Ht * Wt * s * s, (size_t)Wt * s * sizeof(float),
                                            x2 + ((size_t)img * H * s + (size_t)wy * s) * W * s + (size_t)wx * s, (size_t)W * s * sizeof(float),
                                            (size_t)Wt * s * sizeof(float), (size_t)Ht * s, hipMemcpyDeviceToDevice, stream));
                ++t;
            }
    if ((rc = run_forward(h, h->tile_x, h->tile_x2, h->tile_y, (int)tiles, Ht, Wt, stream))) return rc;
    auto owned = [&](const std::vector<int>& st, size_t i, int full, int* lo, int* hi) {
        *lo = st[i] + (st[i] > 0 ? R : 0);
        *hi = i + 1 < st.size() ? st[i + 1] + R : full;
    };
    t = 0;
    for (int img = 0; img < n; ++img)
        for (size_t iy = 0; iy < ys.size(); ++iy)
            for (size_t ix = 0; ix < xs.size(); ++ix) {
                int y0, y1, x0, x1;
                owned(ys, iy, H, &y0, &y1);
                owned(xs, ix, W, &x0, &x1);
                if (y1 > y0 && x1 > x0) {
                    const float* src = h->tile_y + t * Ht * Wt * s * s + ((size_t)(y0 - ys[iy]) * s) * Wt * s + (size_t)(x0 - xs[ix]) * s;
                    float* dst = y + ((size_t)img * H * s + (size_t)y0 * s) * W * s + (size_t)x0 * s;
                    HIP_TRY(h, hipMemcpy2DAsync(dst, (size_t)W * s * sizeof(float), src, (size_t)Wt * s * sizeof(float),
                                                (size_t)(x1 - x0) * s * sizeof(float), (size_t)(y1 - y0) * s,
                                                hipMemcpyDeviceToDevice, stream));
                }
                ++t;
            }
    return DCSCN_OK;
}


static void pass_pixels(const dcscn_ctx* h, int64_t* pass, int64_t* budget) {
    const bool want16 = p16_active(h);
    constexpr long long kRef = 1 << 20;
    int64_t ws_per_lr_pixel = 0;
    for (const WsBuf& b : h->bufs) ws_per_lr_pixel += (int64_t)b.res * b.res * (int64_t)(ws_tensor_bytes(b, kRef, want16) / kRef);
    ws_per_lr_pixel += (ws_per_lr_pixel + 63) / 64;
    *budget = h->workspace_budget / std::max<int64_t>(ws_per_lr_pixel, 1);
    if (want16) *budget = std::min<int64_t>(*budget, kP16MaxPixels / ((int64_t)h->p16_max_res * h->p16_max_res));
    *pass = std::min(h->sub_batch_pixels, *budget);
}

static int refill_tables(dcscn_ctx* h, hipStream_t stream) {
    std::vector<Op*> with_tables;
    for (Op& op : h->ops) {
        with_tables.push_back(&op);
        for (Op& sub : op.fused) with_tables.push_back(&sub);
    }
    for (Op* opp : with_tables) {
        Op& op = *opp;
        if (op.multi.empty() || !op.d_srctab) continue;
        const unsigned long long pad_ptr = (unsigned long long)(uintptr_t)buf_ptr(h, op.multi[0].first);
        size_t q = 0;
        for (const auto& sg : op.multi) {
            const char* base = reinterpret_cast<const char*>(buf_ptr(h, sg.first));
            const unsigned stride = (unsigned)(h->bufs[sg.first].stride * sizeof(float));
            for (int c4 = 0; c4 < ((sg.second + 7) & ~7) / 4 && q < op.h_srctab.size(); ++c4, ++q)
                op.h_srctab[q] = c4 < sg.second / 4 ? NinSrcQuad{(unsigned long long)(uintptr_t)(base + 16 * c4), stride, 1u} : NinSrcQuad{pad_ptr, 0, 0};
        }
        for (; q < op.h_srctab.size(); ++q) op.h_srctab[q] = NinSrcQuad{pad_ptr, 0, 0};
        HIP_TRY(h, hipMemcpyAsync(op.d_srctab, op.h_srctab.data(), op.h_srctab.size() * sizeof(NinSrcQuad), hipMemcpyHostToDevice, stream));
    }
    for (Op& op : h->ops) {
        if (!op.h16.d_tab16 || !h->p16_now || !op.h16.in16_ok) continue;
        std::vector<std::pair<int, int>> srcs = op.multi;
        if (srcs.empty()) srcs.push_back({op.in_buf, op.cin_phys});
        const unsigned long long zero_rec = (unsigned long long)(uintptr_t)buf_ptr(h, srcs[0].first);
        size_t q = 0;
        for (const auto& sg : srcs) {
            const WsBuf& wb = h->bufs[sg.first];
            const char* base = reinterpret_cast<const char*>(buf_ptr(h, sg.first));
            for (int o = 0; o < wb.octs && q < op.h16.h_tab16.size(); ++o, ++q)
                op.h16.h_tab16[q] = NinSrcQuad{(unsigned long long)(uintptr_t)(base + (long long)(o >> 2) * wb.plane + 128 + (o & 3) * 32),
                                               (unsigned)p16_rec_bytes(wb.octs, o >> 2), 1u};
        }
        for (; q < op.h16.h_tab16.size(); ++q) op.h16.h_tab16[q] = NinSrcQuad{zero_rec, 0, 0};
        HIP_TRY(h, hipMemcpyAsync(op.h16.d_tab16, op.h16.h_tab16.data(), op.h16.h_tab16.size() * sizeof(NinSrcQuad), hipMemcpyHostToDevice, stream));
    }
    h->h_zrec.clear();
    for (const WsBuf& wb : h->bufs)
        if (wb.p16)
            for (int c = 0; c < (wb.octs + 3) / 4; ++c) h->h_zrec.push_back((unsigned long long)(uintptr_t)(static_cast<char*>(h->arena) + wb.offset + (long long)c * wb.plane));
    if (!h->h_zrec.empty()) {
        if (h->h_zrec.size() > h->zrec_cap) {
            const int rc = grow(h, &h->d_zrec, &h->zrec_cap, h->h_zrec.size() * 2, stream, DCSCN_ERR_HIP);
            if (rc) return rc;
        }
        HIP_TRY(h, hipMemcpyAsync(h->d_zrec, h->h_zrec.data(), h->h_zrec.size() * sizeof(unsigned long long), hipMemcpyHostToDevice, stream));
    }
    h->tables_gen = h->carve_gen;
    return DCSCN_OK;
}

static int profile_begin(dcscn_ctx* h, int op_index, const Pass& p, size_t* evi) {
    *evi = h->ev_used;
    h->ev_used += 2;
    h->ev_op.push_back(op_index);
    HIP_TRY(h, hipEventRecord(h->ev[*evi], p.stream));
    return DCSCN_OK;
}

static int run_pass(dcscn_ctx* h, const Pass& p) {
    const int nops = (int)h->ops.size(), s = h->cfg.scale;
    const size_t y_floats = (size_t)p.nb * p.H * s * p.W * s;
    bool any_h16 = false;
    for (const Op& op : h->ops) any_h16 = any_h16 || op_any_split16(h, op);
    if (any_h16)
        HIP_TRY(h, pass_begin_launch(redo_flags(h), (int)h->redo_ints, h->p16_now ? h->d_zrec : nullptr, h->p16_now ? (int)h->h_zrec.size() : 0, p.stream));
    for (int i = 0; i < nops; ++i) {
        const Op& op = h->ops[i];
        size_t evi = 0;
        if (h->profile)
            if (int rc = profile_begin(h, i, p, &evi)) return rc;
        if (h->debug_poison) HIP_TRY(h, debug_poison_launch(h->debug_poison, p.stream));
        if (int rc = launch_op(h, op, p)) return rc;
        if (h->profile) HIP_TRY(h, hipEventRecord(h->ev[evi + 1], p.stream));
        if (h->debug_digest) {
            for (int k = 0; k < 2; ++k) {
                const int idx = op.out_buf[k];
                if (k == 1 && idx == op.out_buf[0]) break;
                if (idx >= 0) {
                    const WsBuf& wb = h->bufs[idx];
                    HIP_TRY(h, debug_digest_launch(static_cast<const char*>(h->arena) + wb.offset, wb.p16 ? wb.bytes / 4 : (size_t)p.nb * p.H * wb.res * p.W * wb.res * wb.stride, h->d_digest + i, p.stream));
                } else if (idx == EXT_Y) {
                    HIP_TRY(h, debug_digest_launch(p.y, y_floats, h->d_digest + i, p.stream));
                }
            }
        }
    }
    if (any_h16) {
        Pass redo = p;
        redo.redo = true;
        size_t evi = 0;
        if (h->profile)
            if (int rc = profile_begin(h, nops, p, &evi)) return rc;
        for (const Op& op : h->ops) {
            if (!op.h16.rerun) continue;
            if (int rc = launch_op(h, op, redo)) return rc;
        }
        if (h->profile) HIP_TRY(h, hipEventRecord(h->ev[evi + 1], p.stream));
    }
    if (h->debug_digest) HIP_TRY(h, debug_digest_launch(p.y, y_floats, h->d_digest + nops, p.stream));
    return DCSCN_OK;
}

struct CaptureGuard {
    hipStream_t stream;
    bool capturing = false;
    ~CaptureGuard() {
        if (!capturing) return;
        hipGraph_t g = nullptr;
        (void)hipStreamEndCapture(stream, &g);
        if (g) (void)hipGraphDestroy(g);
    }
};

int forward_done(dcscn_ctx* h, hipStream_t stream) {
    HIP_TRY(h, hipEventRecord(h->done_ev, stream));
    h->last_stream = stream;
    h->has_last = true;
    return DCSCN_OK;
}

int run_forward(dcscn_ctx* h, const float* x, const float* x2, float* y, int n, int H, int W, hipStream_t stream) {
    if (!h->finalized) return fail(h, DCSCN_ERR_STATE, "dcscn_forward before dcscn_finalize");
    if (n < 0 || H <= 0 || W <= 0) return fail(h, DCSCN_ERR_INVALID_ARG, "bad shape n=%d h=%d w=%d", n, H, W);
    if (n == 0) return DCSCN_OK;
    if (!x || !x2 || !y) return fail(h, DCSCN_ERR_INVALID_ARG, "null image pointer");
    HIP_TRY(h, hipSetDevice(h->device));
    const int64_t per_image = (int64_t)H * W;
    int64_t pass_px, budget_px;
    pass_pixels(h, &pass_px, &budget_px);
    if (h->has_last && h->last_stream != stream) HIP_TRY(h, hipStreamWaitEvent(stream, h->done_ev, 0));
    if (per_image > budget_px && h->spatial_tiling) return run_tiled(h, x, x2, y, n, H, W, budget_px, stream);
    int nb = (int)std::max<int64_t>(1, std::min<int64_t>(n, pass_px / per_image));
    int rc = ensure_workspace(h, nb, H, W, stream);
    while (rc == DCSCN_ERR_NOMEM && nb > 1) {
        nb = (nb + 1) / 2;
        rc = ensure_workspace(h, nb, H, W, stream);
    }
    if (rc) return rc;
    if (h->tables_gen != h->carve_gen)
        if ((rc = refill_tables(h, stream))) return rc;
    const int s = h->cfg.scale;
    const int batches = (n + nb - 1) / nb;
    const int nops = (int)h->ops.size();
    if (h->profile) {
        const size_t need = h->ev_used + (size_t)batches * (nops + 1) * 2;
        while (h->ev.size() < need) {
            hipEvent_t e;
            HIP_TRY(h, hipEventCreate(&e));
            h->ev.push_back(e);
        }
        h->ev_forwards += 1;
    }
    dcscn_ctx::GraphKey gkey;
    gkey.x = x; gkey.x2 = x2; gkey.y = y; gkey.stream = stream; gkey.n = n; gkey.H = H; gkey.W = W;
    gkey.split16 = h->split16 ? h->split16_mask : 0;
    gkey.fast16 = h->split16 && h->fast16 ? 1 : 0;
    gkey.fast16_stream = h->split16 && h->fast16_stream ? 1 : 0;
    gkey.nb = nb;
    gkey.h8 = h->conv3_h8 ? 1 : 0;
    gkey.nin_h8 = h->nin_h8 ? 1 : 0;
    gkey.p16 = h->p16_now ? 1 : 0;
    gkey.carve = (unsigned long long)h->carve_gen;
    const bool graphs = h->graph_replay && !h->profile && !h->debug_digest && !h->debug_poison;
    if (graphs && h->graph_exec && gkey == h->graph_key) {
        HIP_TRY(h, hipGraphLaunch(h->graph_exec, stream));
        return forward_done(h, stream);
    }
    CaptureGuard capture{stream};
    if (graphs && gkey == h->graph_seen) {
        if (hipStreamBeginCapture(stream, hipStreamCaptureModeThreadLocal) == hipSuccess) capture.capturing = true;
        else (void)hipGetLastError();
    }
    h->graph_seen = gkey;
    if (h->debug_digest) {
        if (nops + 1 > 1024) return fail(h, DCSCN_ERR_UNSUPPORTED, "debug_digest: more than 1023 launches");
        if (!h->d_digest) HIP_TRY(h, hipMalloc((void**)&h->d_digest, 1024 * sizeof(unsigned long long)));
        HIP_TRY(h, hipMemsetAsync(h->d_digest, 0, 1024 * sizeof(unsigned long long), stream));
    }
    for (int b = 0; b < batches; ++b) {
        const size_t b0 = (size_t)b * nb;
        const Pass pass{std::min(nb, n - b * nb), H, W, x + b0 * H * W, x2 + b0 * H * s * W * s, y + b0 * H * s * W * s, stream, false};
        if ((rc = run_pass(h, pass))) return rc;
    }
    if (capture.capturing) {
        capture.capturing = false;
        hipGraph_t g = nullptr;
        hipError_t ce = hipStreamEndCapture(stream, &g);
        if (h->graph_exec) {
            (void)hipGraphExecDestroy(h->graph_exec);
            h->graph_exec = nullptr;
        }
        if (ce == hipSuccess) ce = hipGraphInstantiate(&h->graph_exec, g, nullptr, nullptr, 0);
        if (g) (void)hipGraphDestroy(g);
        if (ce == hipSuccess) ce = hipGraphLaunch(h->graph_exec, stream);
        if (ce != hipSuccess) {
            (void)hipGetLastError();
            if (h->graph_exec) (void)hipGraphExecDestroy(h->graph_exec);
            h->graph_exec = nullptr;
            h->graph_seen = dcscn_ctx::GraphKey{};
            const bool was = h->graph_replay;
            h->graph_replay = false;
            const int rr = run_forward(h, x, x2, y, n, H, W, stream);
            h->graph_replay = was;
            return rr;
        }
        h->graph_key = gkey;
    }
    return forward_done(h, stream);
}

int resample_table(dcscn_ctx* h, int in_size, int out_size, const dcscn_ctx::ResampleTable** out) {
    auto key = std::make_pair(in_size, out_size);
    auto it = h->resample_tables.find(key);
    if (it == h->resample_tables.end()) {
        std::vector<int> bounds;
        std::vector<double> kk;
        dcscn_ctx::ResampleTable t;
        t.ksize = resample_coeffs(in_size, out_size, &bounds, &kk);
        int rc = upload_vec(h, bounds, &t.d_bounds);
        if (!rc) rc = upload_vec(h, kk, &t.d_kk);
        if (rc) return rc;
        it = h->resample_tables.emplace(key, t).first;
    }
    *out = &it->second;
    return DCSCN_OK;
}

int resize_device(dcscn_ctx* h, const float* in, float* out, int n, int H, int W, int OH, int OW, hipStream_t stream) {
    if (n <= 0) return DCSCN_OK;
    const float* src = in;
    if (OW != W) {
        const dcscn_ctx::ResampleTable* t;
        int rc = resample_table(h, W, OW, &t);
        if (rc) return rc;
        float* dst = out;
        if (OH != H) {
            rc = grow(h, &h->rs_tmp, &h->rs_tmp_cap, (size_t)n * H * OW, stream);
            if (rc) return rc;
            dst = h->rs_tmp;
        }
        HIP_TRY(h, resample_h_launch(src, dst, t->d_bounds, t->d_kk, t->ksize, (long long)n * H, W, OW, stream));
        src = dst;
    }
    if (OH != H) {
        const dcscn_ctx::ResampleTable* t;
        int rc = resample_table(h, H, OH, &t);
        if (rc) return rc;
        HIP_TRY(h, resample_v_launch(src, out, t->d_bounds, t->d_kk, t->ksize, n, H, OH, OW, stream));
    } else if (OW == W) {
        HIP_TRY(h, hipMemcpyAsync(out, in, (size_t)n * H * W * sizeof(float), hipMemcpyDeviceToDevice, stream));
    }
    return DCSCN_OK;
}

static int resample_table8(dcscn_ctx* h, int in_size, int out_size, const dcscn_ctx::ResampleTable** out) {
    const dcscn_ctx::ResampleTable* t;
    int rc = resample_table(h, in_size, out_size, &t);
    if (rc) return rc;
    dcscn_ctx::ResampleTable& e = h->resample_tables[std::make_pair(in_size, out_size)];
    if (!e.d_k8) {
        std::vector<int> bounds, k8;
        resample_coeffs8(in_size, out_size, &bounds, &k8);
        if ((rc = upload_vec(h, k8, &e.d_k8))) return rc;
    }
    *out = &e;
    return DCSCN_OK;
}

int resize_device_bytes(dcscn_ctx* h, const uint8_t* in, uint8_t* out, int n, int H, int W, int C, int OH, int OW, hipStream_t stream) {
    if (n <= 0) return DCSCN_OK;
    const uint8_t* src = in;
    const dcscn_ctx::ResampleTable* t;
    int rc;
    if (OW != W) {
        if ((rc = resample_table8(h, W, OW, &t))) return rc;
        uint8_t* dst = out;
        if (OH != H) {
            if ((rc = grow(h, &h->rs_tmp, &h->rs_tmp_cap, ((size_t)n * H * OW * C + 3) / 4, stream))) return rc;
            dst = reinterpret_cast<uint8_t*>(h->rs_tmp);
        }
        HIP_TRY(h, resample_h8_launch(src, dst, t->d_bounds, t->d_k8, t->ksize, (long long)n * H, W, OW, C, stream));
        src = dst;
    }
    if (OH != H) {
        if ((rc = resample_table8(h, H, OH, &t))) return rc;
        HIP_TRY(h, resample_v8_launch(src, out, t->d_bounds, t->d_k8, t->ksize, n, H, OH, OW * C, stream));
    } else if (OW == W) {
        HIP_TRY(h, hipMemcpyAsync(out, in, (size_t)n * H * W * C, hipMemcpyDeviceToDevice, stream));
    }
    return DCSCN_OK;
}

}
```

dcscn-super-resolution_amd/csrc/kernels.h:

```cpp
#pragma once
#include <hip/hip_runtime.h>
#include <stdint.h>

#include <vector>

namespace dcscn {

enum { ACT_NONE = 0, ACT_ALPHA = 1, ACT_SIGMOID = 2, ACT_TANH = 3, ACT_SELU = 4 };

struct P16Desc {
    char*     base;
    long long plane;
    int32_t   octs;
    int32_t   pad_;
};
__host__ __device__ constexpr int p16_rec_bytes(int octs, int chunk) { return octs - 4 * chunk >= 4 ? 128 : 32 * (octs - 4 * chunk); }
__host__ __device__ constexpr long long p16_plane_bytes(long long npix) { return ((npix + 1) * 128 + 255) & ~255LL; }
__host__ __device__ constexpr long long p16_tensor_bytes(long long npix, int octs) {
    return ((octs + 3) / 4 - 1) * p16_plane_bytes(npix) + ((128 + npix * p16_rec_bytes(octs, (octs + 3) / 4 - 1) + 255) & ~255LL);
}
constexpr long long kP16MaxPixels = (1LL << 25) - 2;

struct OutDesc {
    float*  ptr;
    int32_t stride;
    int32_t off;
    int32_t width;
    P16Desc p16;
};

struct NinSrcQuad {
    unsigned long long ptr;
    unsigned stride;
    unsigned valid;
};

struct ConvArgs {
    const float* in;
    P16Desc in16;
    int32_t in_stride;
    int32_t in_off;
    int32_t cin_phys;
    int32_t n_chunks;
    const float* wpack;
    const float* bias;
    const float* alpha;
    int32_t act;
    int32_t N, H, W;
    int32_t tiles_x, tiles_y;
    OutDesc out0, out1;
    int32_t split;
    int32_t ps;
    int32_t ps_c;
    int32_t vec4;
    const float* res;
    int32_t res_stride;
    const float* dww;
    int32_t dwk;
    int32_t n_full;
    int32_t n_groups;
    int32_t group_span;
    int32_t fold;
    const void* srctab;
    const void* wpack16;
    float inv_scale;
    int32_t* redo;
    int32_t tail_octs;
    int32_t redo_check;
    int32_t nt_pack;
};

struct ConvShape {
    int ks, mt, nt, kc;
    int dwk = 0;
    int nin = 0;
    int wino = 0;
};

__host__ __device__ constexpr int conv_ns(int nt) { return (nt & 1) ? nt * 16 : nt * 16 + 16; }
__host__ __device__ constexpr int conv_plane_stride(int halo_pixels) {
    return ((halo_pixels + 15) / 32) * 32 + 16;
}

ConvShape conv_pick_shape(int ks, int nt, int dwk = 0);
size_t conv_lds_bytes(const ConvShape& s);
hipError_t conv_init_kernels();
hipError_t conv_launch(const ConvShape& s, const ConvArgs& a, int n_tiles, hipStream_t stream);
constexpr int kWinoKC = 8;
constexpr int kWinoMaxNT = 3;
hipError_t wino_init_kernels();
hipError_t wino_launch(int nt, const ConvArgs& a, int n_groups, hipStream_t stream);
constexpr int kNinKC = 16;
constexpr int kNinMaxNT = 6;
hipError_t nin_init_kernels();
hipError_t nin_launch(int nt, const ConvArgs& a, int n_groups, hipStream_t stream);
constexpr int kNinHKC = 32;
hipError_t nin_h_init_kernels();
hipError_t nin_h_launch(int nt, const ConvArgs& a, int n_groups, bool w8, hipStream_t stream, bool fast16 = false);
constexpr int kC3hKC = 32;
constexpr int kC3hMaxNT = 6;
inline int c3h_tail_octs(int cin_phys) {
    const int n_chunks = (cin_phys + kC3hKC - 1) / kC3hKC, tail = cin_phys - (n_chunks - 1) * kC3hKC;
    return n_chunks < 2 || tail > 24 ? 0 : (tail + 7) / 8;
}
inline int c3h_tail_steps(int octs) { return (9 * octs + 3) / 4; }
inline long long xcd_grid_ids(ConvArgs& a, int n_groups) {
    a.n_groups = n_groups;
    a.group_span = n_groups < 3 ? n_groups : 3;
    const long long tiles = (long long)a.N * a.tiles_y * a.tiles_x;
    const int phases = (n_groups + a.group_span - 1) / a.group_span;
    return ((tiles + 7) / 8) * 8 * a.group_span * phases;
}
hipError_t c3h_init_kernels();
hipError_t c3h_launch(int nt, const ConvArgs& a, int n_groups, hipStream_t stream, bool fast16 = false);
hipError_t c3e_init_kernels();
bool c3e_eligible(int nt, const ConvArgs& a, int n_groups);
hipError_t c3e_launch(int nt, const ConvArgs& a, int n_groups, int n_cus, hipStream_t stream, bool fast16 = false);
hipError_t c5h_init_kernels();
hipError_t c5h_launch(int nt, const ConvArgs& args, hipStream_t stream, bool fast16 = false);
constexpr int kFoldVariants = 16;
hipError_t c5h_border_launch(const ConvArgs& args, hipStream_t stream, bool fast16 = false);

constexpr int kStreamPX = 48;
constexpr int kStreamRowPx = kStreamPX + 2;
constexpr int kStreamMaxL = 7;
constexpr int kStreamMT = kStreamPX / 16;

struct StreamRing {
    int32_t off;
    int32_t units;
    int32_t quads;
    int32_t slots;
};
struct StreamConv {
    StreamRing in, out;
    int32_t lag;
    int32_t dww;
    int32_t wp;
    int32_t ba;
    int32_t to_global;
    float inv;
};
struct StreamNinSrc {
    StreamRing ring;
    int32_t chunks;
    int32_t w;
    int32_t last_ql;
};
struct StreamArgs {
    const float* x;
    float* out;
    const float* blob;
    int32_t out_stride;
    int32_t N, H, W;
    int32_t n_strips, useful_w, halo;
    int32_t n_blocks, useful_h, rows_c;
    int32_t n_jobs, jobs_per_wg;
    int32_t L, n_conv, total_lag;
    alignas(16) int8_t role[16];
    int32_t ring_bytes, ldsw_bytes, ldsw_src;
    int32_t first_w;
    StreamRing first_out;
    StreamConv conv[kStreamMaxL];
    StreamNinSrc nin[kStreamMaxL];
    StreamRing b1;
    int32_t nin_ba;
    int32_t nb_quads;
    float nin_inv;
    int32_t* redo;
    int32_t redo_check;
};


struct TailArgs {
    const float* c2;
    const float* x2;
    float* y;
    const float* blob;
    int32_t c2_stride;
    int32_t N, H, W;
    int32_t n_strips, useful_w, halo;
    int32_t n_blocks, useful_h, rows_c;
    int32_t n_jobs, jobs_per_wg;
    StreamRing in, u;
    int32_t v_off;
    int32_t ring_bytes, ldsw_bytes;
    int32_t a_dww, a_wp, a_bias;
    int32_t b_dww, b_wp, b_bias;
    float c_w[9];
    float c_scale;
    float a_inv, b_inv;
    int32_t* redo;
    int32_t redo_check;
};
hipError_t tail_launch(const TailArgs& a, int grid, bool f16, hipStream_t stream);
void stream_init_kernels();
hipError_t stream_launch(const StreamArgs& a, int grid, bool f16, hipStream_t stream);

constexpr int kS3MaxL = 8;
constexpr int kS3MaxWaves = 8;
constexpr int kS3RolePair = 32, kS3RoleNin = 16;
struct S3Ring { int32_t off, px, octs; };
struct S3Out {
    P16Desc p16;
    float* ptr;
    int32_t stride, width;
    int32_t lo, hi;
};
struct S3Nin {
    int32_t on;
    int32_t w_off;
    int32_t ba_off;
    float inv;
    S3Ring b1;
};
struct S3Conv {
    S3Ring in, out;
    int32_t lag;
    int32_t w_off;
    int32_t ba_off;
    int32_t tiles;
    float inv;
};
struct Stream3Args {
    const float* x;
    const float* blob;
    int32_t N, H, W;
    int32_t n_strips, useful_w, halo, n_blocks, useful_h, rows_c, n_jobs, jobs_per_wg;
    int32_t L, total_lag, n_waves;
    int8_t role_conv[kS3MaxWaves];
    int32_t first_w;
    S3Ring first_out;
    S3Conv conv[kS3MaxL];
    S3Out out[kS3MaxL];
    S3Nin nin;
    S3Out out2;
    int32_t ring_bytes;
    int32_t* redo;
};
hipError_t stream3_launch(const Stream3Args& a, int grid, hipStream_t stream, bool fast16 = false);
hipError_t stream3_fast16_launch(const Stream3Args& a, int grid, hipStream_t stream);

int conv_max_fused_dw_nt();

hipError_t ensemble_gather_launch(const float* in, float* out, int h, int w, int n, hipStream_t stream);
hipError_t ensemble_reduce_launch(const float* y, double* out, int h, int w, int n, hipStream_t stream);

hipError_t rgb_to_y_launch(const uint8_t* rgb, double* y64, float* y32, long long n, hipStream_t stream);
hipError_t rgb_to_ycbcr_launch(const uint8_t* rgb, double* out, long long n, hipStream_t stream);
hipError_t y_cbcr_to_rgb_launch(const double* y64, const float* y32, const double* cbcr, const uint8_t* rgb8, double* out, long long n,
                                hipStream_t stream);
hipError_t y_cbcr_to_rgb_bytes_launch(const double* y64, const float* y32, const uint8_t* rgb8, uint8_t* out, long long n, hipStream_t stream);
hipError_t cast_bytes_launch(const double* v64, const float* v32, uint8_t* out, long long n, hipStream_t stream);

constexpr int kMetricTaps = 11;
struct MetricWeights { double w[kMetricTaps]; };
int metric_segments(int h);
hipError_t metrics_launch(const double* a64, const float* a32, const double* b64, const float* b32, int stride, int border, int h, int w,
                          const MetricWeights& wt, double* part_s, long long* part_e, long long* out, hipStream_t stream);

int resample_coeffs(int in_size, int out_size, std::vector<int>* bounds, std::vector<double>* kk);
hipError_t resample_h_launch(const float* in, float* out, const int* bounds, const double* kk, int ksize,
                             long long rows, int w, int ow, hipStream_t stream);
hipError_t resample_v_launch(const float* in, float* out, const int* bounds, const double* kk, int ksize,
                             int n_img, int h, int oh, int w, hipStream_t stream);
int resample_coeffs8(int in_size, int out_size, std::vector<int>* bounds, std::vector<int>* k8);
hipError_t resample_h8_launch(const uint8_t* in, uint8_t* out, const int* bounds, const int* k8, int ksize, long long rows, int w, int ow,
                              int c, hipStream_t stream);
hipError_t resample_v8_launch(const uint8_t* in, uint8_t* out, const int* bounds, const int* k8, int ksize, int n_img, int h, int oh,
                              int wc, hipStream_t stream);
int conv_max_nt(int ks);
inline size_t cin1_lds_bytes(int ks, int cs) { const int ht = 16 + 2 * (ks / 2); return (size_t)(((ht * ht + 3) & ~3) + (ks * ks + 2) * cs) * sizeof(float); }
inline size_t cout1_lds_bytes(int ks, int cin_phys) { const int ht = 16 + 2 * (ks / 2); return (size_t)(ks * ks * cin_phys + ks * ks * ((ht * ht + 3) & ~3)) * sizeof(float); }

struct Cin1Args {
    const float* x;
    const float* w;
    const float* bias;
    const float* alpha;
    int32_t act;
    int32_t ks;
    int32_t N, H, W;
    int32_t cs;
    OutDesc out;
    int32_t* redo;
    int32_t redo_check;
};
hipError_t cin1_launch(const Cin1Args& a, hipStream_t stream);

struct Cout1Args {
    const float* in; int32_t in_stride, in_off, cin_phys;
    const float* w;
    float scale;
    float bias;
    int32_t ks;
    int32_t N, H, W;
    float* out; int32_t out_stride;
    const float* res; int32_t res_stride;
    const int32_t* redo; int32_t redo_check;
};
hipError_t cout1_launch(const Cout1Args& a, hipStream_t stream);

struct DwArgs {
    const float* in; int32_t in_stride, in_off;
    const int32_t* chan_map;
    const float* w;
    int32_t ks, cin, cout_phys;
    int32_t N, H, W;
    float* out; int32_t out_stride;
    const int32_t* redo; int32_t redo_check;
};
hipError_t depthwise_launch(const DwArgs& a, hipStream_t stream);
hipError_t pass_begin_launch(int32_t* redo, int n, const unsigned long long* zrec, int nz, hipStream_t stream);
hipError_t debug_poison_launch(int what, hipStream_t stream);
hipError_t debug_digest_launch(const void* p, size_t n_words, unsigned long long* out, hipStream_t stream);

}
```

dcscn-super-resolution_amd/csrc/plan.h:

```cpp
#pragma once
#include <hip/hip_runtime.h>

#include <algorithm>
#include <cmath>
#include <cstdarg>
#include <cstdio>
#include <cstdlib>
#include <cstring>
#include <map>
#include <string>
#include <vector>

#include "../../include/dcscn.h"
#include "kernels.h"

namespace dcscn_impl {
using namespace dcscn;

inline int pad4(int c) { return (c + 3) & ~3; }
inline int pad16(int c) { return (c + 15) & ~15; }

enum { EXT_X = -1, EXT_X2 = -2, EXT_Y = -3 };
enum OpKind { OP_CONV = 0, OP_CIN1 = 1, OP_DW = 2, OP_COUT1 = 3, OP_STREAM = 4, OP_TAIL = 5, OP_STREAM3 = 6, OP_FOLDX = 7 };
enum Kernel { K_CONV_IGEMM, K_CONV_WINO2, K_CONV_NIN, K_CONV_NIN_H, K_CONV5_H, K_CONV3_H8, K_CONV3_H, K_CONV_CIN1, K_CONV_COUT1, K_DEPTHWISE,
              K_FEAT_STREAM, K_TAIL_STREAM, K_FEAT3_STREAM, K_LAYER_BY_LAYER };
constexpr int kNoSplit = 1 << 30;

struct TensorSpec {
    std::string name;
    std::vector<int64_t> shape;
    std::vector<float> data;
    bool set = false;
};

struct WsBuf {
    int stride = 0;
    int res = 1;
    size_t offset = 0;
    bool p16_ok = false, p16 = false;
    int octs = 0;
    long long plane = 0;
    size_t bytes = 0;
};

inline size_t ws_tensor_bytes(const WsBuf& b, long long npix, bool p16) {
    const size_t bytes = (size_t)npix * b.stride * sizeof(float);
    return p16 && b.p16_ok && b.stride > 0 ? std::max(bytes, (size_t)p16_tensor_bytes(npix, b.octs)) : bytes;
}
inline size_t ws_granules(size_t bytes) { return (bytes + 255) & ~(size_t)255; }

struct ColSeg {
    int w = -1, b = -1, alpha = -1;
    int cout = 0;
    int col0 = 0;
    int dst = 0;
    int dw1 = -1;
};

struct TrainState;
struct TrainBatches;

struct Op {
    OpKind kind = OP_CONV;
    std::string name;
    int ks = 3, cin = 0, cout = 0, res = 1;
    int act = ACT_NONE;
    float const_alpha = 0.0f;
    int in_buf = EXT_X, in_off = 0, cin_phys = 0;
    int in_stride_override = 0;
    std::vector<int> chan_map;
    std::vector<ColSeg> segs;
    int dw_w = -1;
    int dwk = 0;
    float out_scale = 1.0f;
    int tconv_s = 0;
    int fold_s = 0;
    int fold_c = 0;
    int fold_rw = -1;
    int out_buf[2] = {EXT_Y, EXT_Y}, out_off[2] = {0, 0}, out_width[2] = {0, 0};
    int split = kNoSplit;
    int ps = 1, ps_c = 0;
    bool residual = false;
    bool vec4 = true;
    ConvShape shape{3, 2, 1, 4};
    int n_tiles = 1, n_chunks = 0, ctot = 0;
    int n_full = 0;
    int64_t macs = 0, bytes = 0;
    float* d_w = nullptr;
    float* d_bias = nullptr;
    float* d_alpha = nullptr;
    int32_t* d_map = nullptr;
    float* d_dww = nullptr;
    std::vector<std::pair<int, int>> multi;
    std::vector<NinSrcQuad> h_srctab;
    NinSrcQuad* d_srctab = nullptr;
    std::vector<Op> fused;
    StreamArgs stream{};
    TailArgs tail{};
    Stream3Args stream3{};
    std::vector<int> extra_out;
    int halo = -1;
    struct Split16 {
        bool on = false;
        int nt = 0, n_tiles = 0, n_full = 0, n_chunks = 0;
        float inv_scale = 1.0f;
        void* d_w = nullptr;
        float* d_bias = nullptr;
        float* d_alpha = nullptr;
        int tail_octs = 0;
        bool rerun = false;
        bool in16_ok = false;
        std::vector<NinSrcQuad> h_tab16;
        NinSrcQuad* d_tab16 = nullptr;
    } h16;
};

inline bool has_second_dst(const Op& op) { return op.split < (1 << 29); }
template <class F>
inline void for_each_dst(const Op& op, F&& f) {
    f(op.out_buf[0], 0);
    if (has_second_dst(op)) f(op.out_buf[1], 1);
    for (int b : op.extra_out) f(b, 0);
}

}

using namespace dcscn_impl;

struct dcscn_ctx {
    dcscn_config cfg{};
    int device = 0;
    hipStream_t stream = nullptr;
    std::string error;
    bool finalized = false;

    std::vector<int> sched;
    std::vector<TensorSpec> tensors;
    std::map<std::string, int> tensor_index;
    std::vector<dcscn_layer_info> layers;
    std::vector<WsBuf> bufs;
    std::vector<Op> ops;

    void* arena = nullptr;
    size_t arena_bytes = 0;
    int lay_n = 0, lay_h = 0, lay_w = 0;
    float* io_x = nullptr; float* io_x2 = nullptr; float* io_y = nullptr;
    size_t io_x_cap = 0, io_x2_cap = 0, io_y_cap = 0;
    struct ResampleTable { int ksize = 0; int* d_bounds = nullptr; double* d_kk = nullptr; int* d_k8 = nullptr; };
    std::map<std::pair<int, int>, ResampleTable> resample_tables;
    float* rs_tmp = nullptr; size_t rs_tmp_cap = 0;
    float* ens_x = nullptr; float* ens_x2 = nullptr; float* ens_y = nullptr; float* ens_out = nullptr;
    size_t ens_x_cap = 0, ens_x2_cap = 0, ens_y_cap = 0, ens_out_cap = 0;
    float* rs_in = nullptr; float* rs_out = nullptr; size_t rs_in_cap = 0, rs_out_cap = 0;
    float* col_rgb = nullptr; float* col_d = nullptr; float* col_d2 = nullptr; float* col_y32 = nullptr;
    size_t col_rgb_cap = 0, col_d_cap = 0, col_d2_cap = 0, col_y32_cap = 0;
    double* met_buf = nullptr; size_t met_buf_cap = 0;
    float* tile_x = nullptr; float* tile_x2 = nullptr; float* tile_y = nullptr;
    size_t tile_x_cap = 0, tile_x2_cap = 0, tile_y_cap = 0;
    std::vector<void*> device_allocs;

    int64_t sub_batch_pixels = 4 << 20;
    int64_t workspace_budget = (int64_t)48 << 30;
    hipEvent_t done_ev = nullptr;
    std::vector<hipEvent_t> host_ev;
    hipStream_t last_stream = nullptr;
    bool has_last = false;
    bool profile = false;
    unsigned long long* d_digest = nullptr;
    int debug_digest = 0;
    bool conv3_h8 = true;
    bool nin_h8 = true;
    int n_cus = 256;
    int debug_poison = 0;
    bool graph_replay = false;
    struct GraphKey {
        const void *x = nullptr, *x2 = nullptr, *y = nullptr;
        void* stream = nullptr;
        int n = 0, H = 0, W = 0, split16 = 0, fast16 = 0, fast16_stream = 0, nb = 0, h8 = 0, nin_h8 = 0, p16 = 0;
        unsigned long long carve = 0;
        bool operator==(const GraphKey& o) const {
            return x == o.x && x2 == o.x2 && y == o.y && stream == o.stream && n == o.n && H == o.H && W == o.W && split16 == o.split16 && fast16 == o.fast16 &&
                   fast16_stream == o.fast16_stream && nb == o.nb &&
                   h8 == o.h8 && nin_h8 == o.nin_h8 && p16 == o.p16 && carve == o.carve;
        }
    };
    GraphKey graph_seen, graph_key;
    hipGraphExec_t graph_exec = nullptr;
    bool winograd = true;
    bool stream_tail = true;
    bool stream_nin = true;
    bool stream_dense = true;
    bool stream_features = true;
    int split16_mask = 3;
    bool split16 = true;
    bool fast16 = false;
    bool fast16_stream = false;
    size_t redo_off = 0, redo_ints = 0;
    bool p16 = true;
    bool p16_now = false;
    bool any_p16 = false;
    int p16_max_res = 1;
    bool dense_features = true;
    int concat_buf = -1;
    std::vector<std::pair<int, int>> concat_slices;
    uint64_t carve_gen = 0, tables_gen = 0;
    bool nin = true;
    bool fold_force = false;
    bool fold_tail = true;
    bool fold_whole = true;
    bool spatial_tiling = true;
    std::vector<unsigned long long> h_zrec;
    unsigned long long* d_zrec = nullptr;
    size_t zrec_cap = 0;
    std::vector<hipEvent_t> ev;
    size_t ev_used = 0;
    std::vector<int> ev_op;
    int ev_forwards = 0;
    std::vector<void*> pack_allocs;
    bool train_split16 = false;
    bool train_split16_wgrad = false;
    dcscn_impl::TrainState* train = nullptr;
    dcscn_impl::TrainBatches* batches = nullptr;
};

namespace dcscn_impl {

extern thread_local std::string g_global_error;
void set_global_error(const char* fmt, ...);
int fail(dcscn_ctx* h, int code, const char* fmt, ...);

#define HIP_TRY(h, expr)                                                                       \
    do {                                                                                       \
        hipError_t e_ = (expr);                                                                \
        if (e_ != hipSuccess)                                                                  \
            return fail(h, DCSCN_ERR_HIP, "%s failed: %s (%s:%d)", #expr, hipGetErrorString(e_), \
                        __FILE__, __LINE__);                                                   \
    } while (0)

inline float* buf_ptr(dcscn_ctx* h, int id) { return reinterpret_cast<float*>(static_cast<char*>(h->arena) + h->bufs[id].offset); }

void filter_schedule(int layers, int filters, int min_filters, double gamma, std::vector<int>& out);
int kernel_act(int activator, float* const_alpha);
int build_graph(dcscn_ctx* h);
bool nin_eligible(const dcscn_ctx* h, const Op& op);
bool wino_eligible(const dcscn_ctx* h, const Op& op);
bool h16_direct_eligible(const dcscn_ctx* h, const Op& op);
bool fold_linear_tail(dcscn_ctx* h);
bool fold_whole_tail(dcscn_ctx* h);
int stream_chunk_channel(int quads, int ch, int q, int s);
void fuse_feat_stream(dcscn_ctx* h);
void fuse_tail_stream(dcscn_ctx* h);
void fuse_feat3_stream(dcscn_ctx* h);
void densify_features(dcscn_ctx* h);
void plan_p16(dcscn_ctx* h);
inline bool p16_active(const dcscn_ctx* h) { return h->p16 && h->any_p16 && h->split16 && h->split16_mask == 3; }
int upload(dcscn_ctx* h, const void* host, size_t bytes, void** dev);
template <class T, class P>
inline int upload_vec(dcscn_ctx* h, const std::vector<T>& v, P** dev) { return upload(h, v.data(), v.size() * sizeof(T), (void**)dev); }
int finalize_op(dcscn_ctx* h, Op& op);
int pack_feat_stream(dcscn_ctx* h, Op& op);
int pack_tail_stream(dcscn_ctx* h, Op& op);
int pack_feat3_stream(dcscn_ctx* h, Op& op);
int pack_foldx(dcscn_ctx* h, Op& op);
int repack_weights(dcscn_ctx* h);
void train_free(dcscn_ctx* h);
int train_sync_inference(dcscn_ctx* h);
int check_patches(dcscn_ctx* h, const dcscn_patch* p, int n, int lr_size, double max_value);
int build_batch_device(dcscn_ctx* h, const dcscn_patch* p, int n, int lr_size, double max_value, float* x, float* x2, float* y_true,
                       hipStream_t stream);
void train_batches_free(dcscn_ctx* h);
bool op_on_split16(const dcscn_ctx* h, const Op& op);
Kernel op_kernel(const dcscn_ctx* h, const Op& op, bool redo = false);
const char* kernel_name(Kernel k);
int run_forward(dcscn_ctx* h, const float* x, const float* x2, float* y, int n, int H, int W, hipStream_t stream);
int forward_done(dcscn_ctx* h, hipStream_t stream);
int resample_table(dcscn_ctx* h, int in_size, int out_size, const dcscn_ctx::ResampleTable** out);
template <class T>
int grow(dcscn_ctx* h, T** p, size_t* cap, size_t count, hipStream_t stream, int nomem_code = DCSCN_ERR_NOMEM) {
    if (count <= *cap) return DCSCN_OK;
    HIP_TRY(h, hipStreamSynchronize(stream));
    if (*p) HIP_TRY(h, hipFree(*p));
    *p = nullptr;
    *cap = 0;
    hipError_t e = hipMalloc((void**)p, count * sizeof(T));
    if (e != hipSuccess) return fail(h, nomem_code, "buffer of %zu bytes: %s", count * sizeof(T), hipGetErrorString(e));
    *cap = count;
    return DCSCN_OK;
}
int resize_device(dcscn_ctx* h, const float* in, float* out, int n, int H, int W, int OH, int OW, hipStream_t stream);
int resize_device_bytes(dcscn_ctx* h, const uint8_t* in, uint8_t* out, int n, int H, int W, int C, int OH, int OW, hipStream_t stream);

}
```

Measured before the change: 123.4.

## Add six-row-per-wave conv3 h8 variant to tile 48-row images without padding waste

```diff
diff --git a/dcscn-super-resolution_amd/build.py b/dcscn-super-resolution_amd/build.py
--- a/dcscn-super-resolution_amd/build.py
+++ b/dcscn-super-resolution_amd/build.py
@@ -24,6 +24,7 @@
     "conv_wino2.hip": (KERNEL, True), "conv_nin.hip": (KERNEL, True), "feat_stream.hip": (KERNEL, True),
     "conv_nin_h.hip": (KERNEL, True), "conv_nin_h_w8.hip": (KERNEL, True), "conv3_h.hip": (KERNEL, True), "conv3_h8.hip": (KERNEL, True),
     "conv5_h.hip": (KERNEL, True), "conv3_h_p16.hip": (KERNEL, True), "conv3_h8_p16.hip": (KERNEL, True),
+    "conv3_h8_rows6.hip": (KERNEL, True),
     "conv3_h_fast16.hip": (KERNEL, True), "conv3_h8_fast16.hip": (KERNEL, True), "conv_nin_h_fast16.hip": (KERNEL, True),
     "conv5_h_fast16.hip": (KERNEL, True), "feat_stream_redo.hip": (NO_SLP, False), "feat3_stream.hip": (KERNEL, True),
     "feat3_stream_fast16.hip": (KERNEL, True),
diff --git a/dcscn-super-resolution_amd/csrc/api.hip b/dcscn-super-resolution_amd/csrc/api.hip
--- a/dcscn-super-resolution_amd/csrc/api.hip
+++ b/dcscn-super-resolution_amd/csrc/api.hip
@@ -258,6 +258,7 @@
         if (s16) {
             const int64_t tiles = (int64_t)op.h16.n_tiles * (op.h16.nt - 1) + op.h16.n_full;
             out->nt = op.h16.nt; out->kc = 32; out->n_tiles = op.h16.n_tiles;
+            if (op_kernel(h, op) == K_CONV3_H8) out->mt = op_h8_rows(h, op, h->lay_h * op.res);
             const int64_t ksteps = op.shape.nin ? op.h16.n_chunks : op.fold_s > 0 ? 25 * (int64_t)op.h16.n_chunks
                                                 : 9 * (int64_t)(op.h16.n_chunks - (op.h16.tail_octs ? 1 : 0)) + (op.h16.tail_octs ? c3h_tail_steps(op.h16.tail_octs) : 0);
             out->executed_macs_per_lr_pixel = r2 * (h->fast16 ? 1 : 3) * ksteps * 32 * tiles * 16;
@@ -364,6 +365,11 @@
     }
     if (!strcmp(key, "conv3_h8")) {
         h->conv3_h8 = value != 0;
+        return DCSCN_OK;
+    }
+    if (!strcmp(key, "conv3_h8_rows")) {
+        if (value != 0 && value != 4) return fail(h, DCSCN_ERR_INVALID_ARG, "conv3_h8_rows must be 0 (automatic) or 4");
+        h->conv3_h8_rows = (int)value;
         return DCSCN_OK;
     }
     if (!strcmp(key, "nin_h8")) {
diff --git a/dcscn-super-resolution_amd/csrc/conv3_h8.hip b/dcscn-super-resolution_amd/csrc/conv3_h8.hip
--- a/dcscn-super-resolution_amd/csrc/conv3_h8.hip
+++ b/dcscn-super-resolution_amd/csrc/conv3_h8.hip
@@ -6,6 +6,7 @@
 
 hipError_t c3e_init_kernels() {
     hipError_t e = c3e16_init_kernels();
+    if (e == hipSuccess) e = c3e6_init_kernels();
     if (e == hipSuccess) e = c3e1_init_kernels();
     return e != hipSuccess ? e : List::set_attrs();
 }
@@ -15,8 +16,13 @@
            a.n_chunks >= 3;
 }
 
-hipError_t c3e_launch(int nt, const ConvArgs& args, int n_groups, int n_cus, hipStream_t stream, bool fast16) {
-    if (!c3e_eligible(nt, args, n_groups) || !args.wpack16 || args.tiles_x != (args.W + 15) / 16 || args.tiles_y != (args.H + 15) / 16) return hipErrorInvalidValue;
+int c3e_rows(int nt, int H, bool p16, bool fast16) {
+    return nt <= 4 && p16 && !fast16 && H > 0 && (H + 23) / 24 * 24 <= (H + 15) / 16 * 16 ? 6 : 4;
+}
+
+hipError_t c3e_launch(int nt, const ConvArgs& args, int n_groups, int n_cus, hipStream_t stream, bool fast16, int rows) {
+    if (rows != 4 && rows != 6) return hipErrorInvalidValue;
+    if (!c3e_eligible(nt, args, n_groups) || !args.wpack16 || args.tiles_x != (args.W + 15) / 16 || args.tiles_y != (args.H + 4 * rows - 1) / (4 * rows)) return hipErrorInvalidValue;
     ConvArgs a = args;
     a.n_groups = n_groups;
     a.nt_pack = nt;
@@ -27,6 +33,7 @@
     const bool p16 = a.in16.base && out16;
     if (!p16 && (a.in16.base || a.out0.p16.base || a.out1.p16.base)) return hipErrorInvalidValue;
     const int key = c3e_key(nt, a.n_full == 2 ? nt : nt - 1, p16);
+    if (rows == 6) return c3e_rows(nt, a.H, p16, fast16) == 6 ? c3e6_launch(key, a, wgs, stream) : hipErrorInvalidValue;
     if (fast16) return c3e1_launch(key, a, wgs, stream);
     if (p16) return c3e16_launch(key, a, wgs, stream);
     return List::launch(key, a, wgs, stream);
diff --git a/dcscn-super-resolution_amd/csrc/conv3_h8.hpp b/dcscn-super-resolution_amd/csrc/conv3_h8.hpp
--- a/dcscn-super-resolution_amd/csrc/conv3_h8.hpp
+++ b/dcscn-super-resolution_amd/csrc/conv3_h8.hpp
@@ -12,28 +12,31 @@
     asm volatile("s_mov_b32 m0, %2\n\ts_nop 0\n\tglobal_load_lds_dwordx4 %0, %1" : : "v"(voff), "s"(sbase), "s"(lds_dst) : "memory", "m0");
 }
 
-template <int NT>
+template <int NT, int R = 4>
 struct C3EGeom {
     static constexpr int THREADS = 512;
-    static constexpr int KC = 32, TH = 16, TW = 16, HT = 18, HP = HT * HT;
+    static constexpr int KC = 32, TH = 4 * R, TW = 16, HT = 18, HR = TH + 2, HP = HT * HR;
     static constexpr int PIX_BYTES = 128, ROW_BYTES = HT * PIX_BYTES, IN_BYTES = HP * PIX_BYTES;
-    static constexpr int IN_BUF = 41 * 1024;
+    static constexpr int IN_BUF = R == 4 ? 41 * 1024 : IN_BYTES;
     static constexpr int IN_ITEMS = HP * 8;
     static constexpr int IN_ROUNDS = (IN_ITEMS + THREADS - 1) / THREADS;
     static constexpr int F_TAP_BYTES = NT * 2048;
     static constexpr int F_ROUNDS = (2 * NT + 3) / 4;
     static constexpr int IMG = 0;
+    static constexpr int SLOTS0 = R == 4 ? 3 : 2;
     static constexpr int F_BASE = 2 * IN_BUF;
-    static constexpr int BA_BASE = F_BASE + 2 * 3 * F_TAP_BYTES;
+    static constexpr int F1_BASE = F_BASE + SLOTS0 * F_TAP_BYTES;
+    static constexpr int BA_BASE = F1_BASE + 3 * F_TAP_BYTES;
     static constexpr int LDS_BYTES = BA_BASE + 4 * NT * 128;
 };
 
-template <int NT, int C1, int NTP = NT, bool P16 = false, int NP = 3>
+template <int NT, int C1, int NTP = NT, bool P16 = false, int NP = 3, int R = 4>
 __global__ __launch_bounds__(512, 2) void conv3_h8(const ConvArgs a) {
     static_assert(C1 == NT || C1 == NT - 1, "half 1 takes as many tiles as half 0 or one fewer");
+    static_assert(R == 4 || (R == 6 && NT <= 4 && P16), "six rows: 96 accumulators, image staged by LDS-DMA");
     static_assert(NP == 1 || NP == 3, "one product (fast16) or three (split16)");
-    constexpr int PFD = 2 < NT ? 2 : (NT > 1 ? NT - 1 : 1), NB = PFD + 1;
-    using G = C3EGeom<NT>;
+    constexpr int PFD = R == 6 ? 1 : 2 < NT ? 2 : (NT > 1 ? NT - 1 : 1), NB = PFD + 1;
+    using G = C3EGeom<NT, R>;
     extern __shared__ __attribute__((aligned(16))) char smem_c3e[];
     char* const smem = smem_c3e;
     constexpr int F = G::F_ROUNDS, L = G::IN_ROUNDS;
@@ -56,6 +59,7 @@
     const unsigned f_off = (unsigned)(lane * 16);
     const int cq = tid & 7;
     const int tap_stride = ntp * 2048;
+    const int last_off = R == 4 ? 40 * 1024 : wave < 2 ? (56 + wave) * 1024 : G::IN_BYTES - 1024;
 
     struct Unit {
         int valid, tile_id, img, y0, x0, g, o;
@@ -96,7 +100,7 @@
             const int gy = u.y0 - 1 + hrow, gx = u.x0 - 1 + hcol;
             bool ok = r * 64 + hp0 < G::HP && gy >= 0 && gy < H && gx >= 0 && gx < W;
             if constexpr (P16 && r == L - 1) {
-                const int hp = 320 + (hp0 & 7), hr = hp / G::HT, hc = hp - G::HT * hr;
+                const int hp = last_off / G::PIX_BYTES + (hp0 & 7), hr = hp / G::HT, hc = hp - G::HT * hr;
                 const int qy = u.y0 - 1 + hr, qx = u.x0 - 1 + hc;
                 ok = hp < G::HP && qy >= 0 && qy < H && qx >= 0 && qx < W;
             }
@@ -154,15 +158,15 @@
         const char* base = a.in16.base + (long long)chunk * a.in16.plane;
         int t8 = tid >> 3;
         asm volatile("" : "+v"(t8));
-        const int hp = r < L - 1 ? r * 64 + t8 : 320 + (t8 & 7);
+        const int hp = r < L - 1 ? r * 64 + t8 : last_off / G::PIX_BYTES + (t8 & 7);
         const int hrow = hp / G::HT, hcol = hp - G::HT * hrow;
         const int s = lane & 7;
         const int kq = ((s >> 1) - (hcol >> 1)) & 3;
         const int part = (s ^ kq ^ hcol) & 1;
         const bool ok = ((mask >> r) & 1u) && kq < rem;
         const unsigned voff = ok ? 128u + (unsigned)(pix0 + hrow * W + hcol) * (unsigned)rec + (unsigned)((2 * kq + part) * 16) : (unsigned)(s * 16);
-        const int piece = r < L - 1 ? wave + 8 * r : 40;
-        glds16c(base, voff, lds0 + (unsigned)(buf * G::IN_BUF + piece * 1024));
+        const int dst = r < L - 1 ? (wave + 8 * r) * 1024 : last_off;
+        glds16c(base, voff, lds0 + (unsigned)(buf * G::IN_BUF + dst));
     };
     auto dma_f = [&](const char* src, int slot , int cnt) DCSCN_INL {
         const int pieces = cnt > 0 ? 2 * cnt : 1;
@@ -186,15 +190,18 @@
     constexpr int HALF = decltype(half_c)::value;
     constexpr bool BAR_L = HALF == 1, BAR_C = HALF == 0;
     constexpr bool DMA_LATE = HALF == 1;
+    constexpr int NS = HALF == 0 ? G::SLOTS0 : 3, AHEAD = NS - 1;
     Unit cur, nxt;
     int id = blockIdx.x;
     decode(id, cur);
     if (!cur.valid) return;
     decode(id + (int)gridDim.x, nxt);
     int ibuf = 0;
-    int sl0 = G::F_BASE + (half * 3 + 0) * G::F_TAP_BYTES, sl1 = G::F_BASE + (half * 3 + 1) * G::F_TAP_BYTES, sl2 = G::F_BASE + (half * 3 + 2) * G::F_TAP_BYTES;
+    constexpr int F_HALF = HALF == 0 ? G::F_BASE : G::F1_BASE;
+    int sl0 = F_HALF, sl1 = F_HALF + G::F_TAP_BYTES;
+    [[maybe_unused]] int sl2 = F_HALF + (NS - 1) * G::F_TAP_BYTES;
     dma_f(tap_src(cur, nxt, 0), sl0, CNT);
-    dma_f(tap_src(cur, nxt, 1), sl1, CNT);
+    if constexpr (NS == 3) dma_f(tap_src(cur, nxt, 1), sl1, CNT);
     if constexpr (P16) {
         static_for<0, L>([&](auto r_) DCSCN_INL { img_piece(r_, cur.pix0, cur.ok_mask, 0, 0); });
         asm volatile("s_waitcnt vmcnt(0)" ::: "memory");
@@ -206,8 +213,8 @@
     c3p_barrier();
     if (half == 1) asm volatile("s_setprio 1");
 
-    f32x4 acc[4][NT];
-    [[maybe_unused]] h8 xh[4], xl[4], wa[NB], wb[NB];
+    f32x4 acc[R][NT];
+    [[maybe_unused]] h8 xh[R], xl[R], wa[NB], wb[NB];
     bool pending = false;
     int parity = 0;
     int e_tile = 0, e_img = 0, e_y0 = 0, e_x0 = 0, e_g = 0, e_o = 0;
@@ -237,13 +244,13 @@
                     const int chunk = oct0 >> 2, rem = od.octs - 4 * chunk;
                     const int rec = rem >= 4 ? 128 : 32 * rem;
                     char* base = od.base + (long long)chunk * od.plane + 128 + (long long)((e_img * H + e_y0) * W + e_x0) * rec + (oct0 & 3) * 32;
-                    const unsigned voff = (unsigned)((4 * w4 * W + lje) * rec + lke * 16);
+                    const unsigned voff = (unsigned)((R * w4 * W + lje) * rec + lke * 16);
                     const unsigned rowb = (unsigned)(W * rec);
                     const bool chan_ok = col_ok && oct0 + (lke >> 1) < od.octs;
                     const f32x4 bv = *reinterpret_cast<const f32x4*>(smem + ba + (n * 4 + lke) * 16);
                     f32x4 av = {0.0f, 0.0f, 0.0f, 0.0f};
                     if (ACT_C == ACT_ALPHA || (ACT_C < 0 && a.act == ACT_ALPHA)) av = *reinterpret_cast<const f32x4*>(smem + ba + NT * 64 + (n * 4 + lke) * 16);
-                    static_for<0, 4>([&](auto m_) DCSCN_INL {
+                    static_for<0, R>([&](auto m_) DCSCN_INL {
                         constexpr int m = decltype(m_)::value;
                         f32x4 v = acc[m][n] * inv + bv;
                         if constexpr (ACT_C == ACT_ALPHA) {
@@ -252,14 +259,14 @@
                             v.z = v.z > 0.0f ? v.z : av.z * v.z;
                             v.w = v.w > 0.0f ? v.w : av.w * v.w;
                         } else if constexpr (ACT_C < 0) {
-                            if (chan_ok && (!MASK || e_y0 + 4 * w4 + m < H)) chk = nonfinite_acc(chk, acc[m][n], zero);
+                            if (chan_ok && (!MASK || e_y0 + R * w4 + m < H)) chk = nonfinite_acc(chk, acc[m][n], zero);
                             v.x = activate1(v.x, av.x, a.act);
                             v.y = activate1(v.y, av.y, a.act);
                             v.z = activate1(v.z, av.z, a.act);
                             v.w = activate1(v.w, av.w, a.act);
                         }
-                        const u32x4 unit = p16_unit(v, m1, chk, zero2, chan_ok && (!MASK || e_y0 + 4 * w4 + m < H));
-                        if (chan_ok && (!MASK || e_y0 + 4 * w4 + m < H)) *reinterpret_cast<u32x4*>(base + (size_t)(voff + m * rowb)) = unit;
+                        const u32x4 unit = p16_unit(v, m1, chk, zero2, chan_ok && (!MASK || e_y0 + R * w4 + m < H));
+                        if (chan_ok && (!MASK || e_y0 + R * w4 + m < H)) *reinterpret_cast<u32x4*>(base + (size_t)(voff + m * rowb)) = unit;
                     });
                 });
             };
@@ -288,13 +295,13 @@
                     const int owidth = first ? a.out0.width : a.out1.width;
                     const int cc0 = first ? c0 : c0 - a.split;
                     char* base = reinterpret_cast<char*>(optr + ((size_t)(e_img * H + e_y0) * W + e_x0) * ostride + ooff + cc0);
-                    const unsigned voff = (unsigned)(((4 * w4 * W + lje) * ostride + 4 * lke) * 4);
+                    const unsigned voff = (unsigned)(((R * w4 * W + lje) * ostride + 4 * lke) * 4);
                     const unsigned rowb = (unsigned)(W * ostride * 4);
                     const bool chan_ok = cc0 + 4 * lke < owidth;
                     const f32x4 bv = *reinterpret_cast<const f32x4*>(smem + ba + (n * 4 + lke) * 16);
                     f32x4 av = {0.0f, 0.0f, 0.0f, 0.0f};
                     if constexpr (ACT_C == ACT_ALPHA) av = *reinterpret_cast<const f32x4*>(smem + ba + NT * 64 + (n * 4 + lke) * 16);
-                    static_for<0, 4>([&](auto m_) DCSCN_INL {
+                    static_for<0, R>([&](auto m_) DCSCN_INL {
                         constexpr int m = decltype(m_)::value;
                         f32x4 v = acc[m][n] * inv + bv;
                         if constexpr (ACT_C == ACT_ALPHA) {
@@ -334,9 +341,9 @@
                     bx = sub - ay * ps;
                 }
                 const bool live = gx < W && cc < owidth;
-                static_for<0, 4>([&](auto m_) DCSCN_INL {
+                static_for<0, R>([&](auto m_) DCSCN_INL {
                     constexpr int m = decltype(m_)::value;
-                    const int gy = e_y0 + 4 * w4 + m;
+                    const int gy = e_y0 + R * w4 + m;
                     f32x4 v = acc[m][n] * inv + bv;
                     v.x = activate1(v.x, av.x, act);
                     v.y = activate1(v.y, av.y, act);
@@ -394,32 +401,35 @@
                     int l = lane;
                     asm volatile("" : "+v"(l));
                     const int hx = (l & 15) + kx;
-                    b_hi = img_off + (4 * w4 * G::HT + hx) * G::PIX_BYTES + c3h_unit(hx, l >> 4, 0) * 16;
-                }
-                static_for<(ky == 0 ? 0 : 3), 4>([&](auto m_) DCSCN_INL {
+                    b_hi = img_off + (R * w4 * G::HT + hx) * G::PIX_BYTES + c3h_unit(hx, l >> 4, 0) * 16;
+                }
+                static_for<(ky == 0 ? 0 : R - 1), R>([&](auto m_) DCSCN_INL {
                     constexpr int row = ky + decltype(m_)::value;
-                    xh[row & 3] = *reinterpret_cast<const h8*>(smem + b_hi + row * G::ROW_BYTES);
-                    if constexpr (NP == 3) xl[row & 3] = *reinterpret_cast<const h8*>(smem + (b_hi ^ 16) + row * G::ROW_BYTES);
-                });
-                const char* fs = smem + (step % 3 == 0 ? sl0 : step % 3 == 1 ? sl1 : sl2) + a_lane;
+                    xh[row % R] = *reinterpret_cast<const h8*>(smem + b_hi + row * G::ROW_BYTES);
+                    if constexpr (NP == 3) xl[row % R] = *reinterpret_cast<const h8*>(smem + (b_hi ^ 16) + row * G::ROW_BYTES);
+                });
+                auto slot_of = [&](auto s_c) DCSCN_INL { constexpr int s = decltype(s_c)::value % NS; return s == 0 ? sl0 : s == 1 ? sl1 : sl2; };
+                const char* fs = smem + slot_of(std::integral_constant<int, step>{}) + a_lane;
                 static_for<0, PFD>([&](auto p_) DCSCN_INL {
                     constexpr int p = decltype(p_)::value;
                     wb[p] = *reinterpret_cast<const h8*>(fs + (2 * p) * 1024);
                     if constexpr (NP == 3) wa[p] = *reinterpret_cast<const h8*>(fs + (2 * p + 1) * 1024);
                 });
                 auto dma_ahead = [&]() DCSCN_INL {
-                    constexpr int step2 = (step + 2) % 9;
+                    constexpr int step2 = (step + AHEAD) % 9;
                     constexpr int ptap2 = (step2 % 3) * 3 + step2 / 3;
                     const char* src;
-                    if constexpr (step + 2 < 9) src = cur.f_base + (size_t)(chunk * 9 + ptap2) * tap_stride;
+                    if constexpr (step + AHEAD < 9) src = cur.f_base + (size_t)(chunk * 9 + ptap2) * tap_stride;
                     else src = !last_main ? cur.f_base + (size_t)((chunk + 1) * 9 + ptap2) * tap_stride
                              : octs      ? cur.f_base + (size_t)(n_main * 9 + step2) * tap_stride
                                          : nxt.f_base + (size_t)ptap2 * tap_stride;
-                    dma_f(src, (step + 2) % 3 == 0 ? sl0 : (step + 2) % 3 == 1 ? sl1 : sl2, CNT);
+                    dma_f(src, slot_of(std::integral_constant<int, step + AHEAD>{}), CNT);
                 };
                 if constexpr (!DMA_LATE) dma_ahead();
-                constexpr int IMG = P16 && step >= 1 && step <= L ? 1 : 0, IMG_PREV = P16 && step >= 2 && step <= L + 1 ? 1 : 0;
-                if constexpr (P16) { if constexpr (IMG) img_piece(std::integral_constant<int, step - 1>{}, li_pix0, li_ok, lchunk, ibuf ^ 1); }
+                constexpr int IMG = !P16 ? 0 : R == 4 ? (step >= 1 && step <= L ? 1 : 0) : step == 1 || step == 2 ? 2 : step >= 3 && step <= 6 ? 1 : 0;
+                constexpr int IMG0 = R == 4 ? step - 1 : step <= 2 ? 2 * (step - 1) : step + 1;
+                constexpr int IMG_PREV = P16 && step >= 2 && step <= L + 1 ? 1 : 0;
+                if constexpr (P16) static_for<0, IMG>([&](auto i_) DCSCN_INL { img_piece(std::integral_constant<int, IMG0 + decltype(i_)::value>{}, li_pix0, li_ok, lchunk, ibuf ^ 1); });
                 else {
                     if constexpr (step == 0) load_in(li_base, li_ok, lchunk);
                     if constexpr (step >= 3) convert_store(std::integral_constant<int, step - 3>{}, li_all_in, li_ok, lchunk, ibuf ^ 1);
@@ -430,7 +440,7 @@
                 if constexpr (DMA_LATE) { dma_ahead(); __builtin_amdgcn_sched_barrier(0); }
                 if constexpr (step == 0) {
                     if (chunk == 0)
-                        static_for<0, 4>([&](auto m_) DCSCN_INL {
+                        static_for<0, R>([&](auto m_) DCSCN_INL {
                             static_for<0, NT>([&](auto n_) DCSCN_INL { acc[decltype(m_)::value][decltype(n_)::value] = f32x4{0.0f, 0.0f, 0.0f, 0.0f}; });
                         });
                 }
@@ -443,19 +453,23 @@
                             if constexpr (NP == 3) wa[(n + PFD) % NB] = *reinterpret_cast<const h8*>(fs + (2 * (n + PFD) + 1) * 1024);
                         }
                         if constexpr (NP == 3) {
-                        static_for<0, 4>([&](auto m_) DCSCN_INL { constexpr int m = decltype(m_)::value; acc[m][n] = __builtin_amdgcn_mfma_f32_16x16x32_f16(wa[n % NB], xh[(ky + m) & 3], acc[m][n], 0, 0, 0); });
-                        static_for<0, 4>([&](auto m_) DCSCN_INL { constexpr int m = decltype(m_)::value; acc[m][n] = __builtin_amdgcn_mfma_f32_16x16x32_f16(wb[n % NB], xl[(ky + m) & 3], acc[m][n], 0, 0, 0); });
+                        static_for<0, R>([&](auto m_) DCSCN_INL { constexpr int m = decltype(m_)::value; acc[m][n] = __builtin_amdgcn_mfma_f32_16x16x32_f16(wa[n % NB], xh[(ky + m) % R], acc[m][n], 0, 0, 0); });
+                        static_for<0, R>([&](auto m_) DCSCN_INL { constexpr int m = decltype(m_)::value; acc[m][n] = __builtin_amdgcn_mfma_f32_16x16x32_f16(wb[n % NB], xl[(ky + m) % R], acc[m][n], 0, 0, 0); });
                         }
-                        static_for<0, 4>([&](auto m_) DCSCN_INL { constexpr int m = decltype(m_)::value; acc[m][n] = __builtin_amdgcn_mfma_f32_16x16x32_f16(wb[n % NB], xh[(ky + m) & 3], acc[m][n], 0, 0, 0); });
+                        static_for<0, R>([&](auto m_) DCSCN_INL { constexpr int m = decltype(m_)::value; acc[m][n] = __builtin_amdgcn_mfma_f32_16x16x32_f16(wb[n % NB], xh[(ky + m) % R], acc[m][n], 0, 0, 0); });
                         __builtin_amdgcn_sched_barrier(0);
                     });
                 };
                 mfmas(std::integral_constant<int, CNT>{});
-                if constexpr (HALF == 0) { if constexpr (P16) c3p_wait_vm<F + IMG + IMG_PREV>(); else if constexpr (step <= 1) c3p_wait_vm<F + L>(); else c3p_wait_vm<F>(); }
+                if constexpr (HALF == 0) {
+                    if constexpr (NS == 2) c3p_wait_vm<IMG>();
+                    else if constexpr (P16) c3p_wait_vm<F + IMG + IMG_PREV>(); else if constexpr (step <= 1) c3p_wait_vm<F + L>(); else c3p_wait_vm<F>();
+                }
                 phase_barrier(bar_c);
                 ++tt;
             });
             ibuf ^= 1;
+            if constexpr (NS == 2) { const int t = sl0; sl0 = sl1; sl1 = t; }
         }
         if (octs) {
             const int img_off = ibuf * G::IN_BUF;
@@ -468,7 +482,7 @@
                     if constexpr (HALF == 0) c3p_wait_vm<F>();
                     static_for<0, L>([&](auto r_) DCSCN_INL { convert_store(r_, nxt.all_in, nxt.ok_mask, 0, ibuf ^ 1); });
                 }
-                if constexpr (!DMA_LATE) dma_f(tap_src(cur, nxt, tt + 2), sl2, CNT);
+                if constexpr (!DMA_LATE) dma_f(tap_src(cur, nxt, tt + AHEAD), NS == 3 ? sl2 : sl1, CNT);
                 if constexpr (P16) {
                     if constexpr (!FIRST) { if (step == 1) static_for<0, L>([&](auto r_) DCSCN_INL { img_piece(r_, nxt.pix0, nxt.ok_mask, 0, ibuf ^ 1); }); }
                 } else if constexpr (FIRST) load_in(nxt.a_base, nxt.ok_mask, 0);
@@ -478,8 +492,8 @@
                 tap = tap < 8 ? tap : 8;
                 const int ky = (tap * 11) >> 5, kx = tap - 3 * ky;
                 const int hx = (l & 15) + kx;
-                const int b = img_off + ((4 * w4 + ky) * G::HT + hx) * G::PIX_BYTES + c3h_unit(hx, oct, 0) * 16;
-                static_for<0, 4>([&](auto m_) DCSCN_INL {
+                const int b = img_off + ((R * w4 + ky) * G::HT + hx) * G::PIX_BYTES + c3h_unit(hx, oct, 0) * 16;
+                static_for<0, R>([&](auto m_) DCSCN_INL {
                     constexpr int m = decltype(m_)::value;
                     xh[m] = *reinterpret_cast<const h8*>(smem + b + m * G::ROW_BYTES);
                     if constexpr (NP == 3) xl[m] = *reinterpret_cast<const h8*>(smem + (b ^ 16) + m * G::ROW_BYTES);
@@ -505,21 +519,23 @@
                             if constexpr (NP == 3) wa[(n + PFD) % NB] = *reinterpret_cast<const h8*>(fs + (2 * (n + PFD) + 1) * 1024);
                         }
                         if constexpr (NP == 3) {
-                        static_for<0, 4>([&](auto m_) DCSCN_INL { constexpr int m = decltype(m_)::value; acc[m][n] = __builtin_amdgcn_mfma_f32_16x16x32_f16(wa[n % NB], xh[m], acc[m][n], 0, 0, 0); });
-                        static_for<0, 4>([&](auto m_) DCSCN_INL { constexpr int m = decltype(m_)::value; acc[m][n] = __builtin_amdgcn_mfma_f32_16x16x32_f16(wb[n % NB], xl[m], acc[m][n], 0, 0, 0); });
+                        static_for<0, R>([&](auto m_) DCSCN_INL { constexpr int m = decltype(m_)::value; acc[m][n] = __builtin_amdgcn_mfma_f32_16x16x32_f16(wa[n % NB], xh[m], acc[m][n], 0, 0, 0); });
+                        static_for<0, R>([&](auto m_) DCSCN_INL { constexpr int m = decltype(m_)::value; acc[m][n] = __builtin_amdgcn_mfma_f32_16x16x32_f16(wb[n % NB], xl[m], acc[m][n], 0, 0, 0); });
                         }
-                        static_for<0, 4>([&](auto m_) DCSCN_INL { constexpr int m = decltype(m_)::value; acc[m][n] = __builtin_amdgcn_mfma_f32_16x16x32_f16(wb[n % NB], xh[m], acc[m][n], 0, 0, 0); });
+                        static_for<0, R>([&](auto m_) DCSCN_INL { constexpr int m = decltype(m_)::value; acc[m][n] = __builtin_amdgcn_mfma_f32_16x16x32_f16(wb[n % NB], xh[m], acc[m][n], 0, 0, 0); });
                         __builtin_amdgcn_sched_barrier(0);
                     });
                 };
                 mfmas(std::integral_constant<int, CNT>{});
                 if constexpr (HALF == 0) {
-                    if constexpr (P16) { if (!FIRST && step == 1) c3p_wait_vm<F + L>(); else c3p_wait_vm<F>(); }
+                    if constexpr (NS == 2) { if (!FIRST && step == 1) c3p_wait_vm<L>(); else c3p_wait_vm<0>(); }
+                    else if constexpr (P16) { if (!FIRST && step == 1) c3p_wait_vm<F + L>(); else c3p_wait_vm<F>(); }
                     else if (FIRST || step == 1) c3p_wait_vm<F + L>(); else c3p_wait_vm<F>();
                 }
                 phase_barrier(bar_c);
                 ++tt;
-                { const int t = sl0; sl0 = sl1; sl1 = sl2; sl2 = t; }
+                if constexpr (NS == 3) { const int t = sl0; sl0 = sl1; sl1 = sl2; sl2 = t; }
+                else { const int t = sl0; sl0 = sl1; sl1 = t; }
             };
             tail_step(0, std::true_type{});
             for (int step = 1; step < n_tail; ++step) tail_step(step, std::false_type{});
@@ -542,11 +558,12 @@
 
 constexpr int c3e_key(int nt, int c1, bool p16) { return (8 * nt + c1) * 2 + p16; }
 
-template <int NT, int C1, bool P16, int NP>
+template <int NT, int C1, bool P16, int NP, int R = 4>
 struct C3EVariant {
     static constexpr int KEY = c3e_key(NT, C1, P16);
-    static constexpr auto kernel = &conv3_h8<NT, C1, NT, P16, NP>;
-    static constexpr int THREADS = C3EGeom<NT>::THREADS, LDS = C3EGeom<NT>::LDS_BYTES;
+    static constexpr auto kernel = &conv3_h8<NT, C1, NT, P16, NP, R>;
+    static constexpr int THREADS = C3EGeom<NT, R>::THREADS, LDS = C3EGeom<NT, R>::LDS_BYTES;
+    static_assert(LDS <= 160 * 1024, "a workgroup's LDS");
     static hipError_t set_attr() { return allow_lds(kernel, LDS); }
     static hipError_t launch(const ConvArgs& a, int wgs, hipStream_t stream) {
         if (P16 && (long long)a.N * a.H * a.W > kP16MaxPixels) return hipErrorInvalidValue;
@@ -560,6 +577,8 @@
 
 hipError_t c3e16_init_kernels();
 hipError_t c3e16_launch(int key, const ConvArgs& a, int wgs, hipStream_t stream);
+hipError_t c3e6_init_kernels();
+hipError_t c3e6_launch(int key, const ConvArgs& a, int wgs, hipStream_t stream);
 hipError_t c3e1_init_kernels();
 hipError_t c3e1_launch(int key, const ConvArgs& a, int wgs, hipStream_t stream);
 
diff --git a/dcscn-super-resolution_amd/csrc/conv3_h8_rows6.hip b/dcscn-super-resolution_amd/csrc/conv3_h8_rows6.hip
--- /dev/null
+++ b/dcscn-super-resolution_amd/csrc/conv3_h8_rows6.hip
@@ -0,0 +1,10 @@
+#include "conv3_h8.hpp"
+
+namespace dcscn {
+
+using List = Variants<C3EVariant<4, 4, true, 3, 6>, C3EVariant<4, 3, true, 3, 6>>;
+
+hipError_t c3e6_init_kernels() { return List::set_attrs(); }
+hipError_t c3e6_launch(int key, const ConvArgs& a, int wgs, hipStream_t stream) { return List::launch(key, a, wgs, stream); }
+
+}
diff --git a/dcscn-super-resolution_amd/csrc/exec.hip b/dcscn-super-resolution_amd/csrc/exec.hip
--- a/dcscn-super-resolution_amd/csrc/exec.hip
+++ b/dcscn-super-resolution_amd/csrc/exec.hip
@@ -76,6 +76,11 @@
         all16 = all16 && o; any16 = any16 || o;
     });
     return in16 ? all16 : !any16;
+}
+
+int op_h8_rows(const dcscn_ctx* h, const Op& op, int H) {
+    if (h->conv3_h8_rows == 4) return 4;
+    return c3e_rows(op.h16.nt, H, h->p16_now && op.h16.in16_ok, h->fast16);
 }
 
 
@@ -335,7 +340,11 @@
         b.tail_octs = op.h16.tail_octs;
         b.alpha = op.h16.d_alpha;
         b.tiles_y = (Hr + 15) / 16;
-        if (kernel == K_CONV3_H8) HIP_TRY(h, c3e_launch(op.h16.nt, b, op.h16.n_tiles, h->n_cus, p.stream, h->fast16));
+        if (kernel == K_CONV3_H8) {
+            const int rows = op_h8_rows(h, op, Hr);
+            b.tiles_y = (Hr + 4 * rows - 1) / (4 * rows);
+            HIP_TRY(h, c3e_launch(op.h16.nt, b, op.h16.n_tiles, h->n_cus, p.stream, h->fast16, rows));
+        }
         else HIP_TRY(h, c3h_launch(op.h16.nt, b, op.h16.n_tiles, p.stream, h->fast16));
     }
     return DCSCN_OK;
@@ -604,6 +613,7 @@
     gkey.fast16_stream = h->split16 && h->fast16_stream ? 1 : 0;
     gkey.nb = nb;
     gkey.h8 = h->conv3_h8 ? 1 : 0;
+    gkey.h8_rows = h->conv3_h8_rows;
     gkey.nin_h8 = h->nin_h8 ? 1 : 0;
     gkey.p16 = h->p16_now ? 1 : 0;
     gkey.carve = (unsigned long long)h->carve_gen;
diff --git a/dcscn-super-resolution_amd/csrc/kernels.h b/dcscn-super-resolution_amd/csrc/kernels.h
--- a/dcscn-super-resolution_amd/csrc/kernels.h
+++ b/dcscn-super-resolution_amd/csrc/kernels.h
@@ -115,7 +115,8 @@
 hipError_t c3h_launch(int nt, const ConvArgs& a, int n_groups, hipStream_t stream, bool fast16 = false);
 hipError_t c3e_init_kernels();
 bool c3e_eligible(int nt, const ConvArgs& a, int n_groups);
-hipError_t c3e_launch(int nt, const ConvArgs& a, int n_groups, int n_cus, hipStream_t stream, bool fast16 = false);
+int c3e_rows(int nt, int H, bool p16, bool fast16);
+hipError_t c3e_launch(int nt, const ConvArgs& a, int n_groups, int n_cus, hipStream_t stream, bool fast16 = false, int rows = 4);
 hipError_t c5h_init_kernels();
 hipError_t c5h_launch(int nt, const ConvArgs& args, hipStream_t stream, bool fast16 = false);
 constexpr int kFoldVariants = 16;
diff --git a/dcscn-super-resolution_amd/csrc/plan.h b/dcscn-super-resolution_amd/csrc/plan.h
--- a/dcscn-super-resolution_amd/csrc/plan.h
+++ b/dcscn-super-resolution_amd/csrc/plan.h
@@ -169,6 +169,7 @@
     unsigned long long* d_digest = nullptr;
     int debug_digest = 0;
     bool conv3_h8 = true;
+    int conv3_h8_rows = 0;
     bool nin_h8 = true;
     int n_cus = 256;
     int debug_poison = 0;
@@ -176,12 +177,12 @@
     struct GraphKey {
         const void *x = nullptr, *x2 = nullptr, *y = nullptr;
         void* stream = nullptr;
-        int n = 0, H = 0, W = 0, split16 = 0, fast16 = 0, fast16_stream = 0, nb = 0, h8 = 0, nin_h8 = 0, p16 = 0;
+        int n = 0, H = 0, W = 0, split16 = 0, fast16 = 0, fast16_stream = 0, nb = 0, h8 = 0, h8_rows = 0, nin_h8 = 0, p16 = 0;
         unsigned long long carve = 0;
         bool operator==(const GraphKey& o) const {
             return x == o.x && x2 == o.x2 && y == o.y && stream == o.stream && n == o.n && H == o.H && W == o.W && split16 == o.split16 && fast16 == o.fast16 &&
                    fast16_stream == o.fast16_stream && nb == o.nb &&
-                   h8 == o.h8 && nin_h8 == o.nin_h8 && p16 == o.p16 && carve == o.carve;
+                   h8 == o.h8 && h8_rows == o.h8_rows && nin_h8 == o.nin_h8 && p16 == o.p16 && carve == o.carve;
         }
     };
     GraphKey graph_seen, graph_key;
@@ -271,6 +272,7 @@
 void train_batches_free(dcscn_ctx* h);
 bool op_on_split16(const dcscn_ctx* h, const Op& op);
 Kernel op_kernel(const dcscn_ctx* h, const Op& op, bool redo = false);
+int op_h8_rows(const dcscn_ctx* h, const Op& op, int H);
 const char* kernel_name(Kernel k);
 int run_forward(dcscn_ctx* h, const float* x, const float* x2, float* y, int n, int H, int W, hipStream_t stream);
 int forward_done(dcscn_ctx* h, hipStream_t stream);
```

Result: no change. 124.6 (median of 6 runs) (+1.0%).
